# zhang-tao-whu/DVIS_Plus

Hardware: AMD Instinct MI355X
Metric: frames/sec DVIS++ R50 offline, 720p T=30 synthetic (higher is better)
Workload: dtype f32 (storage, accumulation, results; the segmenter's dense layers - R50 convolutions from 128 channels on, pixel-decoder projections and FPN output convolution, the deformable encoder's projections and FFN, the decoder's key / value projections - multiply each fp32 operand as two f16 terms on the f1

## Files before the change

### dvis_plus_amd/csrc/conv1x1_x3.hip

```cpp
#include "dvis_common.h"
#include "x3_common.h"

DVIS_EXPORT int64_t dvis_conv_x3_image_bytes(int64_t N, int C, int H, int W);
DVIS_EXPORT int dvis_conv_x3_gn_fold_supported(int K, int G, int64_t HW);

namespace {

constexpr unsigned kOOB = 0x80000000u;

struct CxArgs {
  const float *x, *bias, *res;
  const void *wp;
  float *y;
  int N, C, K, relu, npass;
  int stride, W_in, OW, H_in;
  int taps;
  long long HW, HW_in, pixels;
  long long tiles;
  float xscale, inv;
  int *flag;
  int tag;
  const float *x2;
  int C2, stride2, W2_in;
  long long HW2_in;
// ... 193 lines not shown
              hi4[e] = a.in_relu ? fmaxf(t1, 0.f) : t1;
            }
            asm volatile("" : "+v"(lo4), "+v"(hi4));
            __builtin_amdgcn_sched_barrier(0);
          }
          split8(lo4, hi4, a.xscale, xh[s], xl[s]);
        }
        if constexpr (kAffine)
          if (kc + 1 == NC && more) load_tab(ntile);
        if (++cc == NCC) cc = 0, ++tap;
        const bool first = kc + 1 < NC1, sec = !first && kc + 1 < NC;
        const unsigned po = first ? cx_tap_offset(a, gm, tap) : (sec ? gm2 : cx_tap_offset(a, ngm, 0));
        load_raw(po, first ? cc : (sec ? kc + 1 - NC1 : 0), sec);
      }
#pragma unroll
      for (int part = 0; part < IPC; ++part) {
        const char *stage = ring.wait(false);
        ring.begin(ring.more() ? next_offset() : 0);
        mma_item<IK, NB, PW>(stage, lane, acc, xh + IK * part, xl + IK * part, [&](int i) { ring.piece(i); });
      }
    }
    float chk = 0.f;
    if constexpr (NB == 2 || IMGOUT) {
      if (a.img != nullptr) {
        const unsigned gs = (unsigned)(a.K / 64) * 8192u;
        const __amdgpu_buffer_rsrc_t ri = dvis_make_rsrc_uniform(a.img, (unsigned)((long long)a.N * a.OH * a.XG * gs));
        const __amdgpu_buffer_rsrc_t rb = dvis_make_rsrc_uniform(a.bias ? (const void *)a.bias : (const void *)a.img, a.bias ? (unsigned)a.K * 4u : 0u);
        unsigned ibase = kOOB;
        if (p < a.pixels) {
          const int pix = (int)(p - n * a.HW), oy = pix / a.OW, ox = pix - oy * a.OW;
          ibase = (unsigned)(((n * a.OH + oy) * a.XG + (ox >> 5)) * gs + (co0 / 64) * 8192 + g * 512 + (ox & 31) * 16);
        }
#pragma unroll
        for (int nb = 0; nb < NB; ++nb) {
          float v[16];
#pragma unroll
          for (int q = 0; q < 4; ++q) {
            const f4 b = __builtin_bit_cast(f4, __builtin_amdgcn_raw_buffer_load_b128(rb, (unsigned)(co0 + 32 * nb + 8 * q + 4 * g) * 4u, 0, 0));
#pragma unroll
            for (int i = 0; i < 4; ++i) {
              const float t = acc[nb][4 * q + i] * a.inv + b[i];
              chk = __builtin_fmaf(t, 0.f, chk);
              v[4 * q + i] = a.relu ? x3_relu(t) : t;
            }
          }
          h8 hi[2], lo[2];
#pragma unroll
          for (int u = 0; u < 2; ++u) {
            const f4 p0 = {v[8 * u], v[8 * u + 1], v[8 * u + 2], v[8 * u + 3]}, p1 = {v[8 * u + 4], v[8 * u + 5], v[8 * u + 6], v[8 * u + 7]};
            split8(p0, p1, a.oscale, hi[u], lo[u]);
          }
          const h8 ls = lo[0] + lo[1];
          chk = __builtin_fmaf((float)((ls[0] + ls[1]) + (ls[2] + ls[3]) + (ls[4] + ls[5]) + (ls[6] + ls[7])), 0.f, chk);
          store_fragments4(ri, ibase, hi[0], 4096 * nb, lo[0], 4096 * nb + 1024, hi[1], 4096 * nb + 2048, lo[1], 4096 * nb + 3072);
        }
        if (a.flag != nullptr && chk != chk && p < a.pixels) atomicCAS(a.flag, 0, a.tag);
        tile = ntile, pass = npass_, gm = ngm, gm2 = ngm2;
        continue;
      }
    }
    double gw[8], gw2[4], gw4[2], gtot = 0.0;
#pragma unroll
    for (int nb = 0; nb < NB; ++nb) {
      float rv[16];
      double gq[4];
#pragma unroll
      for (int r = 0; r < 16; ++r)
        rv[r] = a.res ? __builtin_bit_cast(float, __builtin_amdgcn_raw_buffer_load_b32(
                                                      rr, obase + (unsigned)(co0 + 32 * nb + 8 * (r >> 2) + 4 * g + (r & 3)) * ochan, 0, 0))
                      : 0.f;
#pragma unroll
      for (int q = 0; q < 4; ++q) {
        const int co = co0 + 32 * nb + 8 * q + 4 * g;
        f4 b = {0.f, 0.f, 0.f, 0.f};
        if (a.bias) b = *(const f4 *)(a.bias + co);
        double gsum = 0.0, gsq = 0.0;
#pragma unroll
        for (int i = 0; i < 4; ++i) {
          const unsigned o = obase + (unsigned)(co + i) * ochan;
          float v = acc[nb][4 * q + i] * a.inv + b[i] + rv[4 * q + i];
          chk = __builtin_fmaf(v, 0.f, chk);
          if (a.relu) v = x3_relu(v);
          __builtin_amdgcn_raw_buffer_store_b32(__builtin_bit_cast(unsigned, v), ry, o, 0, 0);
          if constexpr (kStats) {
            const double d = p < a.pixels ? (double)v : 0.0;
            gsum = i == 0 ? d : gsum + d;
            gsq = i == 0 ? d * d : __builtin_fma(d, d, gsq);
          }
        }
        if constexpr (kStats) gq[q] = cx_fold<5>(gsum, gsq, lane);
      }
      if constexpr (kStats) {
        gw[nb] = cx_fold<3>(cx_fold<4>(gq[0], gq[1], lane), cx_fold<4>(gq[2], gq[3], lane), lane);
        if (nb % 2 == 1) gw2[nb / 2] = cx_fold<2>(gw[nb - 1], gw[nb], lane);
        if (nb % 4 == 3) gw4[nb / 4] = cx_fold<1>(gw2[nb / 2 - 1], gw2[nb / 2], lane);
        if (nb == NB - 1) gtot = cx_fold<0>(gw4[0], gw4[1], lane);
      }
    }
    if constexpr (kStats) {
      const long long pw = tile * kTile + wave * 32;
      if (pw < a.pixels) {
        const long long nw = pw / a.HW, slot = (pw - nw * a.HW) >> 5;
        const int group = co0 / 8 + 4 * (((lane >> 2) & 1) + 2 * ((lane >> 1) & 1) + 4 * (lane & 1)) + ((lane >> 4) & 1) + 2 * ((lane >> 3) & 1);
        a.gn_part[((nw * (a.K / 8) + group) * a.slots + slot) * 2 + (lane >> 5)] = gtot;
      }
    }
    if (a.flag != nullptr && chk != chk && p < a.pixels) atomicCAS(a.flag, 0, a.tag);
    tile = ntile, pass = npass_, gm = ngm, gm2 = ngm2;
  }
}

__global__ __launch_bounds__(256) void upsample_add_image_kernel(const float *__restrict__ lateral, const float *__restrict__ top,
                                                                 void *__restrict__ img, int N, int C, int H, int W, int h, int w,
                                                                 const float *__restrict__ lat_scale, const float *__restrict__ lat_shift,
                                                                 float oscale) {
  const int NCC = C / 64, XG = (W + 31) / 32;
  const int cc = blockIdx.x, xg = blockIdx.y;
  const int x = threadIdx.x & 31, g = (threadIdx.x >> 5) & 1, S = threadIdx.x >> 6;
  const int px = 32 * xg + x;
  const float sy = (float)h / (float)H, sx = (float)w / (float)W;
  const int pxc = px < W ? px : W - 1;
  float fx = sx * ((float)pxc + 0.5f) - 0.5f;
  fx = fx < 0.f ? 0.f : fx;
  const int x0 = min((int)fx, w - 1), x1 = x0 + (x0 < w - 1 ? 1 : 0);
  const float lx1 = fx - (float)x0, lx0 = 1.f - lx1;
  const __amdgpu_buffer_rsrc_t ri = dvis_make_rsrc_uniform(img, (unsigned)((long long)N * H * XG * NCC * 8192));
  const unsigned rows = (unsigned)N * (unsigned)H;
  for (unsigned row = blockIdx.z * 16u; row < blockIdx.z * 16u + 16u && row < rows; ++row) {
    const unsigned n = row / (unsigned)H;
    const int y = (int)(row - n * (unsigned)H);
    float fy = sy * ((float)y + 0.5f) - 0.5f;
    fy = fy < 0.f ? 0.f : fy;
    const int y0 = min((int)fy, h - 1), y1 = y0 + (y0 < h - 1 ? 1 : 0);
    const float ly1 = fy - (float)y0, ly0 = 1.f - ly1;
    float v[8];
#pragma unroll
    for (int e = 0; e < 8; ++e) {
      const int c = 64 * cc + 32 * (S >> 1) + 16 * (S & 1) + 8 * (e >> 2) + 4 * g + (e & 3);
      const unsigned pl = n * (unsigned)C + (unsigned)c;
      const float *t0 = top + ((size_t)pl * h + y0) * (size_t)w, *t1 = top + ((size_t)pl * h + y1) * (size_t)w;
      float lat = lateral[((size_t)pl * H + y) * (size_t)W + pxc];
      if (lat_scale) lat = lat * lat_scale[pl] + lat_shift[pl];
      v[e] = lat + (ly0 * (lx0 * t0[x0] + lx1 * t0[x1]) + ly1 * (lx0 * t1[x0] + lx1 * t1[x1]));
    }
    const f4 p0 = {v[0], v[1], v[2], v[3]}, p1 = {v[4], v[5], v[6], v[7]};
    h8 hi, lo;
    split8(p0, p1, oscale, hi, lo);
    const unsigned G = row * (unsigned)XG + (unsigned)xg;
    const unsigned off = (G * (unsigned)NCC + (unsigned)cc) * 8192u + (unsigned)(S * 2048 + g * 512 + x * 16);
    store_fragments2(ri, off, hi, 0, lo, 1024);
  }
}

}

DVIS_EXPORT int dvis_upsample_add_image(const float *lateral, const float *lat_scale, const float *lat_shift, const float *top, void *image,
                                        int N, int C, int H, int W, int h, int w, int oexp, void *stream) {
  DVIS_REQUIRE(lateral && top && image, "dvis_upsample_add_image: null pointer");
  DVIS_REQUIRE((lat_scale == nullptr) == (lat_shift == nullptr), "dvis_upsample_add_image: scale and shift together");
  DVIS_REQUIRE(N > 0 && C > 0 && C % 64 == 0 && H > 0 && W > 0 && h > 0 && w > 0, "dvis_upsample_add_image: bad sizes");
  DVIS_REQUIRE((uintptr_t)image % 16 == 0 && dvis_conv_x3_image_bytes(N, C, H, W) < ((int64_t)1 << 31), "dvis_upsample_add_image: a 16-byte "
               "aligned image below 2 GiB");
  const int per = 16 * 65535 / H;
  DVIS_REQUIRE(per >= 1 && (W + 31) / 32 <= 65535, "dvis_upsample_add_image: map too large (%d x %d)", H, W);
  for (int i = 0; i < N; i += per) {
    const int n = N - i < per ? N - i : per;
    hipLaunchKernelGGL(upsample_add_image_kernel, dim3(C / 64, (W + 31) / 32, (n * H + 15) / 16), dim3(256), 0, (hipStream_t)stream,
                       lateral + (size_t)i * C * H * W, top + (size_t)i * C * h * w,
                       (char *)image + (size_t)i * H * ((W + 31) / 32) * (C / 64) * 8192, n, C, H, W, h, w,
                       lat_scale ? lat_scale + (size_t)i * C : nullptr, lat_shift ? lat_shift + (size_t)i * C : nullptr, ldexpf(1.f, oexp));
  }
  return dvis_check_launch("dvis_upsample_add_image");
}

DVIS_EXPORT int dvis_conv1x1_x3_supported(int C, int K, int64_t N, int64_t HW_in, int64_t HW_out) {
  if (C < 64 || C % 64 != 0 || C > 4096) return 0;
  if (!(K == 64 || K == 128 || (K > 0 && K % 256 == 0 && K <= 8192))) return 0;
  if (N <= 0 || HW_out <= 0 || HW_in < HW_out) return 0;
  if (N * C * HW_in * 4 >= ((int64_t)1 << 31) || N * K * HW_out * 4 >= ((int64_t)1 << 31)) return 0;
  return 1;
}

DVIS_EXPORT int64_t dvis_conv1x1_x3_packed_bytes(int C, int K) {
  if (!dvis_conv1x1_x3_supported(C, K, 1, 1, 1)) return -1;
  return (int64_t)(C / 16) * (K / 32) * 2 * kPiece;
}

DVIS_EXPORT int dvis_conv1x1_x3_pack(const float *w, int K, int C, int wexp, void *packed, void *stream) {
  DVIS_REQUIRE(w && packed, "dvis_conv1x1_x3_pack: null operand");
  DVIS_REQUIRE(dvis_conv1x1_x3_supported(C, K, 1, 1, 1), "dvis_conv1x1_x3_pack: (C, K) = (%d, %d) is not served", C, K);
  DVIS_REQUIRE(wexp >= -60 && wexp <= 60, "dvis_conv1x1_x3_pack: wexp = %d", wexp);
  const int NB = K == 64 ? 2 : K == 128 ? 4 : 8;
  const int64_t fragments = (int64_t)(C / 16) * (K / 32) * 64;
  hipLaunchKernelGGL(x3_pack_kernel, dim3((unsigned)((fragments + 255) / 256)), dim3(256), 0, (hipStream_t)stream, w, (int64_t)C, K, C,
                     NB, 0, ldexpf(1.f, wexp), (_Float16 *)packed, fragments);
  return dvis_check_launch("dvis_conv1x1_x3_pack");
}

struct CxFold {
  double *gn_part;
  const float *in_scale, *in_shift;
  int in_relu;
};

static int cx_launch(const float *x, const void *packed, const float *bias, const float *res, float *y, int N, int C, int K, int H, int W,
                     int stride, int taps, int xexp, int wexp, int relu, void *stream, const float *x2 = nullptr, int C2 = 0, int H2 = 0,
                     int W2 = 0, int stride2 = 1, void *image = nullptr, int oexp = 0, const void *ximg = nullptr,
                     const CxFold *fold = nullptr);

DVIS_EXPORT int dvis_conv1x1_x3_dual(const float *x, const float *x2, const void *packed, const float *bias, const float *res, float *y,
                                     int N, int C, int C2, int K, int H, int W, int H2, int W2, int stride2, int xexp, int wexp, int relu,
                                     void *stream) {
  DVIS_REQUIRE(x2 != nullptr && C2 >= 64 && C2 % 64 == 0 && C2 <= 4096, "dvis_conv1x1_x3_dual: C2 %% 64 == 0 (got %d)", C2);
  DVIS_REQUIRE((stride2 == 1 || stride2 == 2) && (H2 + stride2 - 1) / stride2 == H && (W2 + stride2 - 1) / stride2 == W,
               "dvis_conv1x1_x3_dual: x2 (%d x %d, stride %d) must down-sample onto x's %d x %d map", H2, W2, stride2, H, W);
  DVIS_REQUIRE((long long)N * C2 * H2 * W2 * 4 < ((long long)1 << 31) && (uintptr_t)x2 % 16 == 0, "dvis_conv1x1_x3_dual: x2 below 2 GiB, 16-byte aligned");
  return cx_launch(x, packed, bias, res, y, N, C, K, H, W, 1, 1, xexp, wexp, relu, stream, x2, C2, H2, W2, stride2);
}

DVIS_EXPORT int dvis_conv1x1_x3(const float *x, const void *packed, const float *bias, const float *res, float *y, int N, int C, int K,
                                int H, int W, int stride, int xexp, int wexp, int relu, void *stream, const float *in_scale,
                                const float *in_shift, int in_relu, double *gn_part) {
  DVIS_REQUIRE((in_scale == nullptr) == (in_shift == nullptr), "dvis_conv1x1_x3: in_scale and in_shift together");
  const CxFold fold = {gn_part, in_scale, in_shift, in_relu};
  return cx_launch(x, packed, bias, res, y, N, C, K, H, W, stride, 1, xexp, wexp, relu, stream, nullptr, 0, 0, 0, 1, nullptr, 0, nullptr,
                   (gn_part || in_scale) ? &fold : nullptr);
}

DVIS_EXPORT int dvis_conv_x3_gn_fold_supported(int K, int G, int64_t HW) {
  return K > 0 && K % 256 == 0 && G > 0 && K == 8 * G && HW > 0 && HW % 32 == 0;
}

DVIS_EXPORT int dvis_conv1x1_x3_image(const float *x, const void *packed, const float *bias, void *image, int N, int C, int H, int W, int xexp,
                                      int wexp, int oexp, int relu, void *stream) {
  DVIS_REQUIRE(image != nullptr && (uintptr_t)image % 16 == 0, "dvis_conv1x1_x3_image: null / unaligned image");
  DVIS_REQUIRE((long long)N * H * ((W + 31) / 32) * 8192 < ((long long)1 << 31), "dvis_conv1x1_x3_image: the image must stay below 2 GiB");
  return cx_launch(x, packed, bias, nullptr, nullptr, N, C, 64, H, W, 1, 1, xexp, wexp, relu, stream, nullptr, 0, 0, 0, 1, image, oexp);
}

DVIS_EXPORT int64_t dvis_conv_x3_image_bytes(int64_t N, int C, int H, int W) {
  if (N < 0 || C <= 0 || C % 64 != 0 || H <= 0 || W <= 0) return -1;
  return N * H * ((W + 31) / 32) * (int64_t)(C / 64) * 8192;
}

DVIS_EXPORT int dvis_conv_x3_pack_image(const float *w, int K, int C, int taps, int wexp, void *packed, void *stream) {
  DVIS_REQUIRE(w && packed, "dvis_conv_x3_pack_image: null operand");
  DVIS_REQUIRE(taps == 1 || taps == 9, "dvis_conv_x3_pack_image: taps = %d", taps);
  DVIS_REQUIRE(dvis_conv1x1_x3_supported(C, K, 1, 1, 1) && K >= 128, "dvis_conv_x3_pack_image: (C, K) = (%d, %d) is not served", C, K);
  DVIS_REQUIRE(wexp >= -60 && wexp <= 60, "dvis_conv_x3_pack_image: wexp = %d", wexp);
  const int NB = K == 128 ? 4 : 8;
  const int64_t fragments = (int64_t)(taps * C / 16) * (K / 32) * 64;
  hipLaunchKernelGGL(x3_pack_kernel, dim3((unsigned)((fragments + 255) / 256)), dim3(256), 0, (hipStream_t)stream, w, (int64_t)taps * C, K,
                     taps * C, NB, 1, ldexpf(1.f, wexp), (_Float16 *)packed, fragments, taps);
  return dvis_check_launch("dvis_conv_x3_pack_image");
}

DVIS_EXPORT int dvis_conv_x3_image(const void *ximg, const float *x, const void *packed, const float *bias, const float *res, float *y,
                                   void *image, int N, int C, int K, int H, int W, int stride, int taps, int xexp, int wexp, int oexp, int relu,
                                   void *stream, double *gn_part) {
  DVIS_REQUIRE(ximg != nullptr || image != nullptr, "dvis_conv_x3_image: neither side is an operand image (use dvis_conv1x1_x3 / dvis_conv3x3_x3)");
  DVIS_REQUIRE((ximg != nullptr) != (x != nullptr), "dvis_conv_x3_image: exactly one of ximg and x");
  DVIS_REQUIRE((image != nullptr) != (y != nullptr), "dvis_conv_x3_image: exactly one of image and y");
  DVIS_REQUIRE(K == 128 || K % 256 == 0, "dvis_conv_x3_image: K = %d (128 or a multiple of 256)", K);
  DVIS_REQUIRE(taps == 1 || taps == 9, "dvis_conv_x3_image: taps = %d", taps);
  DVIS_REQUIRE(image == nullptr || res == nullptr, "dvis_conv_x3_image: an image output takes no residual");
  DVIS_REQUIRE(((uintptr_t)ximg | (uintptr_t)image) % 16 == 0, "dvis_conv_x3_image: images must be 16-byte aligned");
  const int OH = (H + stride - 1) / stride, OW = (W + stride - 1) / stride;
  DVIS_REQUIRE(dvis_conv_x3_image_bytes(N, C, H, W) < ((int64_t)1 << 31) && dvis_conv_x3_image_bytes(N, K, OH, OW) < ((int64_t)1 << 31),
               "dvis_conv_x3_image: images must stay below 2 GiB");
  DVIS_REQUIRE(gn_part == nullptr || (ximg != nullptr && y != nullptr), "dvis_conv_x3_image: statistics with an image in and an fp32 map out");
  const CxFold fold = {gn_part, nullptr, nullptr, 0};
  return cx_launch(x, packed, bias, res, y, N, C, K, H, W, stride, taps, xexp, wexp, relu, stream, nullptr, 0, 0, 0, 1, image, oexp, ximg,
                   gn_part ? &fold : nullptr);
}

DVIS_EXPORT int64_t dvis_conv3x3_x3_packed_bytes(int C, int K) {
  const int64_t b = dvis_conv1x1_x3_packed_bytes(C, K);
  return b < 0 ? b : 9 * b;
}

DVIS_EXPORT int dvis_conv3x3_x3_pack(const float *w, int K, int C, int wexp, void *packed, void *stream) {
  DVIS_REQUIRE(w && packed, "dvis_conv3x3_x3_pack: null operand");
  DVIS_REQUIRE(dvis_conv1x1_x3_supported(C, K, 1, 1, 1), "dvis_conv3x3_x3_pack: (C, K) = (%d, %d) is not served", C, K);
  DVIS_REQUIRE(wexp >= -60 && wexp <= 60, "dvis_conv3x3_x3_pack: wexp = %d", wexp);
  const int NB = K == 64 ? 2 : K == 128 ? 4 : 8;
  const int64_t fragments = (int64_t)(9 * C / 16) * (K / 32) * 64;
  hipLaunchKernelGGL(x3_pack_kernel, dim3((unsigned)((fragments + 255) / 256)), dim3(256), 0, (hipStream_t)stream, w, (int64_t)9 * C, K, 9 * C,
                     NB, 0, ldexpf(1.f, wexp), (_Float16 *)packed, fragments, 9);
  return dvis_check_launch("dvis_conv3x3_x3_pack");
}

DVIS_EXPORT int dvis_conv3x3_x3(const float *x, const void *packed, const float *bias, const float *res, float *y, int N, int C, int K,
                                int H, int W, int stride, int xexp, int wexp, int relu, void *stream) {
  return cx_launch(x, packed, bias, res, y, N, C, K, H, W, stride, 9, xexp, wexp, relu, stream);
}

static int cx_launch(const float *x, const void *packed, const float *bias, const float *res, float *y, int N, int C, int K, int H, int W,
                     int stride, int taps, int xexp, int wexp, int relu, void *stream, const float *x2, int C2, int H2, int W2, int stride2,
                     void *image, int oexp, const void *ximg, const CxFold *fold) {
  DVIS_REQUIRE((x || ximg) && packed && (y || image), "dvis_conv1x1_x3: null operand");
  DVIS_REQUIRE(stride == 1 || stride == 2, "dvis_conv1x1_x3: stride %d", stride);
  const int OH = (H + stride - 1) / stride, OW = (W + stride - 1) / stride;
  DVIS_REQUIRE(dvis_conv1x1_x3_supported(C, K, N, (int64_t)H * W, (int64_t)OH * OW), "dvis_conv1x1_x3: shape (N %d, C %d, K %d, %d x %d, "
               "stride %d) is not served (C %% 64 == 0, K = 64 / 128 or K %% 256 == 0, tensors below 2 GiB)", N, C, K, H, W, stride);
  DVIS_REQUIRE((uintptr_t)x % 16 == 0 && (uintptr_t)y % 16 == 0 && (uintptr_t)packed % 16 == 0 && (bias == nullptr || (uintptr_t)bias % 16 == 0),
               "dvis_conv1x1_x3: operands must be 16-byte aligned");
  CxArgs a = {};
  a.x = x, a.bias = bias, a.res = res, a.wp = packed, a.y = y, a.N = N, a.C = C, a.K = K, a.relu = relu;
  a.stride = stride, a.W_in = W, a.H_in = H, a.taps = taps, a.OW = OW, a.HW = (long long)OH * OW, a.HW_in = (long long)H * W;
  a.pixels = a.HW * N;
  a.xscale = ldexpf(1.f, xexp), a.inv = ldexpf(1.f, -(xexp + wexp));
  const X3Guard gd = dvis_x3_guard();
  a.flag = gd.flag, a.tag = gd.tag;
  a.x2 = x2, a.C2 = x2 ? C2 : 0, a.stride2 = stride2, a.W2_in = W2, a.HW2_in = (long long)H2 * W2;
  a.img = image, a.XG = (OW + 31) / 32, a.oscale = ldexpf(1.f, oexp), a.OH = OH;
  a.ximg = ximg, a.XG_in = (W + 31) / 32;
  const int grid = dvis_x3_persistent_cus();
  hipStream_t st = (hipStream_t)stream;
  a.npass = K <= 128 ? 1 : K / 256;
  if (fold != nullptr) {
    DVIS_REQUIRE(dvis_conv_x3_gn_fold_supported(K, K / 8, a.HW) && image == nullptr && x2 == nullptr, "dvis_conv1x1_x3: folded GroupNorm "
                 "needs K %% 256 == 0, H * W %% 32 == 0, an fp32 map out, one source (K %d, %d x %d)", K, OH, OW);
    DVIS_REQUIRE((fold->gn_part != nullptr) != (fold->in_scale != nullptr), "dvis_conv1x1_x3: statistics or an input affine, not both");
    a.tiles = (a.pixels + 255) / 256;
    a.gn_part = fold->gn_part, a.slots = (int)(a.HW / 32);
// ... 65 lines not shown
```

### dvis_plus_amd/csrc/gemm_x3.hip

```cpp
#define DVIS_X3_DMA_MUBUF 1
#include "dvis_common.h"
#include "x3_common.h"

#include <stdlib.h>

namespace {

template <int KS>
__device__ __forceinline__ void load_x(const float *x, int64_t ldx, int64_t row, int g, float s, h8 *xh, h8 *xl,
                                       const float *addp = nullptr) {
  const float *p = x + row * ldx + 8 * g;
  f4 raw[2 * KS];
#pragma unroll
  for (int S = 0; S < KS; ++S) raw[2 * S] = *(const f4 *)(p + 16 * S), raw[2 * S + 1] = *(const f4 *)(p + 16 * S + 4);
  if (addp != nullptr) {
#pragma unroll
    for (int S = 0; S < KS; ++S) raw[2 * S] += *(const f4 *)(addp + 16 * S), raw[2 * S + 1] += *(const f4 *)(addp + 16 * S + 4);
  }
#pragma unroll
  for (int S = 0; S < KS; ++S) split8(raw[2 * S], raw[2 * S + 1], s, xh[S], xl[S]);
}

__device__ __forceinline__ void store_block(char *scr, int lane, const f4 *v, float *dst, int64_t ld, int rows_valid,
                                            const float *radd = nullptr, int64_t ldr = 0) {
  const int j = lane & 31, g = lane >> 5, sw = (j >> 1) & 7;
#pragma unroll
  for (int q = 0; q < 4; ++q) *(f4 *)(scr + j * 128 + (((2 * q + g) ^ sw) << 4)) = v[q];
  __builtin_amdgcn_wave_barrier();
#pragma unroll
  for (int t = 0; t < 4; ++t) {
    const int jr = 8 * t + (lane >> 3), pp = lane & 7;
    f4 o = *(const f4 *)(scr + jr * 128 + ((pp ^ ((jr >> 1) & 7)) << 4));
    if (radd != nullptr && jr < rows_valid) o += *(const f4 *)(radd + jr * ldr + 4 * pp);
    if (jr < rows_valid) *(f4 *)(dst + jr * ld + 4 * pp) = o;
  }
  __builtin_amdgcn_wave_barrier();
}

struct EpiArgs {
  const float *bias;
  const float *res;
  int64_t ldres;
  const float *gamma, *beta;
  float eps;
  const float *pos;
  int64_t pos_rows;
  float *out, *out2;
  int64_t ldo;
  float inv;
  int relu;
  const float *radd;
  int *flag;
  int tag;
};

template <int NB, bool LN, bool EX = false>
__device__ __forceinline__ void epilogue(f16v *acc, const EpiArgs &e, const float *cb, const float *cg, const float *cbeta, char *scr,
                                         int lane, int64_t tok0, int64_t M, int col0 = 0) {
  const int j = lane & 31, g = lane >> 5;
  const int64_t tok = tok0 + j < M ? tok0 + j : M - 1;
  const int rows_valid = M - tok0 < 32 ? (int)(M - tok0) : 32;
  constexpr int N = 32 * NB;
  float mean = 0.f, rstd = 1.f;
  if constexpr (LN) {
    const float *rp = e.res + tok * e.ldres + 4 * g;
    f4 r[2][4];
    auto fetch = [&](int nb, f4 *dst) {
#pragma unroll
      for (int q = 0; q < 4; ++q) dst[q] = *(const f4 *)(rp + 32 * nb + 8 * q);
    };
    fetch(0, r[0]);
    float sum = 0.f;
#pragma unroll
    for (int nb = 0; nb < NB; ++nb) {
      if (nb + 1 < NB) fetch(nb + 1, r[(nb + 1) & 1]);
#pragma unroll
      for (int q = 0; q < 4; ++q) {
        const f4 b = *(const f4 *)(cb + 32 * nb + 8 * q + 4 * g);
#pragma unroll
        for (int i = 0; i < 4; ++i) {
          const float v = acc[nb][4 * q + i] * e.inv + b[i] + r[nb & 1][q][i];
          acc[nb][4 * q + i] = v;
          sum += v;
        }
      }
    }
    sum += __shfl_xor(sum, 32);
    if (e.flag != nullptr && !(fabsf(sum) <= 3.4028235e38f)) atomicCAS(e.flag, 0, e.tag);
    mean = sum * (1.f / N);
    float sq = 0.f;
#pragma unroll
    for (int nb = 0; nb < NB; ++nb)
#pragma unroll
      for (int i = 0; i < 16; ++i) {
        const float d = acc[nb][i] - mean;
        sq += d * d;
      }
    sq += __shfl_xor(sq, 32);
    rstd = rsqrtf(sq * (1.f / N) + e.eps);
  }
  float chk = 0.f;
  const float *pr = nullptr;
  f4 pv[2][4];
  auto fetch_pos = [&](int nb, f4 *dst) {
#pragma unroll
    for (int q = 0; q < 4; ++q) dst[q] = *(const f4 *)(pr + 32 * nb + 8 * q);
  };
  if constexpr (LN) {
    if (e.pos != nullptr) {
      pr = e.pos + (tok % e.pos_rows) * N + 4 * g;
      fetch_pos(0, pv[0]);
    }
  }
#pragma unroll
  for (int nb = 0; nb < NB; ++nb) {
    f4 v[4];
    if constexpr (LN) {
      if (e.pos != nullptr && nb + 1 < NB) fetch_pos(nb + 1, pv[(nb + 1) & 1]);
    }
#pragma unroll
    for (int q = 0; q < 4; ++q) {
      const int n = 32 * nb + 8 * q + 4 * g;
      if constexpr (LN) {
        const f4 ga = *(const f4 *)(cg + n), be = *(const f4 *)(cbeta + n);
#pragma unroll
        for (int i = 0; i < 4; ++i) v[q][i] = (acc[nb][4 * q + i] - mean) * rstd * ga[i] + be[i];
      } else {
        const f4 b = *(const f4 *)(cb + n);
#pragma unroll
        for (int i = 0; i < 4; ++i) {
          const float t = acc[nb][4 * q + i] * e.inv + b[i];
          chk = __builtin_fmaf(t, 0.f, chk);
          if constexpr (EX)
            v[q][i] = e.relu == 1 ? x3_relu(t) : e.relu == 2 ? 0.5f * t * (1.f + erff(t * 0.70710678118654752440f)) : t;
          else
            v[q][i] = e.relu ? x3_relu(t) : t;
        }
      }
    }
    if constexpr (!EX)
      store_block(scr, lane, v, e.out + tok0 * e.ldo + col0 + 32 * nb, e.ldo, rows_valid);
    else
      store_block(scr, lane, v, e.out + tok0 * e.ldo + col0 + 32 * nb, e.ldo, rows_valid,
                  e.radd ? e.radd + tok0 * e.ldres + col0 + 32 * nb : nullptr, e.ldres);
    if constexpr (LN) {
      if (e.pos != nullptr) {
#pragma unroll
        for (int q = 0; q < 4; ++q) v[q] += pv[nb & 1][q];
        store_block(scr, lane, v, e.out2 + tok0 * e.ldo + 32 * nb, e.ldo, rows_valid);
      }
    }
  }
  if constexpr (!LN) {
    if (e.flag != nullptr && chk != chk) atomicCAS(e.flag, 0, e.tag);
  }
}

template <int NB>
__global__ __launch_bounds__(kThreads) void x3_linear_kernel(const float *__restrict__ x, int64_t ldx, int64_t M,
                                                             const void *__restrict__ wp, float xscale, int npass,
                                                             const float *__restrict__ xadd, int64_t xadd_rows, EpiArgs e) {
  extern __shared__ __attribute__((aligned(1024))) char lds[];
  constexpr int K = 256, KS = K / 16, NI = K / 32;
  const int wave = threadIdx.x >> 6, lane = threadIdx.x & 63, j = lane & 31, g = lane >> 5;
  const int64_t ntiles = (M + kTileTok - 1) / kTileTok;
  const int64_t my = blockIdx.x < ntiles ? (ntiles - blockIdx.x + gridDim.x - 1) / gridDim.x : 0;
  Ring<NB> ring;
  ring.start(wp, lds, NI * npass, (int)(my * NI * npass), wave, lane);
  char *scr = lds + kStages * Ring<NB>::kItemBytes + wave * kScratch;
  float *cst = (float *)(lds + kStages * Ring<NB>::kItemBytes + kWaves * kScratch);
  const int ntot = 32 * NB * npass;
  for (int i = threadIdx.x; i < ntot; i += kThreads) cst[i] = e.bias ? e.bias[i] : 0.f;
  __syncthreads();
  for (int64_t tile = blockIdx.x; tile < ntiles; tile += gridDim.x) {
    const int64_t tok0 = tile * kTileTok + wave * 32;
    const int64_t row = tok0 + j < M ? tok0 + j : M - 1;
    h8 xh[KS], xl[KS];
    load_x<KS>(x, ldx, row, g, xscale, xh, xl, xadd ? xadd + (row % xadd_rows) * K + 8 * g : nullptr);
    for (int pass = 0; pass < npass; ++pass) {
      f16v acc[NB];
#pragma unroll
      for (int nb = 0; nb < NB; ++nb)
#pragma unroll
        for (int i = 0; i < 16; ++i) acc[nb][i] = 0.f;
#pragma unroll
      for (int c = 0; c < NI; ++c) {
        const char *stage = ring.wait(c == 0);
        ring.begin_periodic();
        mma_item<2, NB, NB>(stage, lane, acc, xh + 2 * c, xl + 2 * c, [&](int i) { ring.piece(i); });
      }
      if (tok0 < M) epilogue<NB, false>(acc, e, cst + pass * 32 * NB, cst + ntot, cst + ntot + 32 * NB, scr, lane, tok0, M, pass * 32 * NB);
    }
  }
}

constexpr int x3_stream_layout_blocks(int nb) { return 4 * nb % 8 == 0 ? nb : nb + 1; }

template <int NB, bool LN, bool EX = false, bool ADD = false>
__global__ __launch_bounds__(512) void x3_linear_stream_kernel(const float *__restrict__ x, int64_t ldx, int64_t M, int K,
                                                               const void *__restrict__ wp, float xscale, int npass,
                                                               const float *__restrict__ xadd, int64_t xadd_rows, EpiArgs e) {
  extern __shared__ __attribute__((aligned(1024))) char lds[];
  constexpr int NBL = x3_stream_layout_blocks(NB);
  constexpr int NW = 8, PW = 4 * NBL / NW, kTile = NW * 32;
  typedef Ring<PW, 8, NW> RingT;
  const int wave = threadIdx.x >> 6, lane = threadIdx.x & 63, j = lane & 31, g = lane >> 5;
  const int NI = K / 32, NC = K / 64;
  const int64_t ntiles = (M + kTile - 1) / kTile;
  const int64_t my = blockIdx.x < ntiles ? (ntiles - blockIdx.x + gridDim.x - 1) / gridDim.x : 0;
  if (my == 0) return;
  RingT ring;
  ring.start(wp, lds, NI * npass, (int)(my * NI * npass), wave, lane);
  char *scr = lds + kStages * RingT::kItemBytes + wave * kScratch;
  float *cst = (float *)(lds + kStages * RingT::kItemBytes + NW * kScratch);
  const int ntot = 32 * NB * npass;
  for (int i = threadIdx.x; i < ntot; i += 512) cst[i] = e.bias ? e.bias[i] : 0.f;
  if constexpr (LN)
    for (int i = threadIdx.x; i < 32 * NB; i += 512) cst[ntot + i] = e.gamma[i], cst[ntot + 32 * NB + i] = e.beta[i];
  __syncthreads();
  auto products = [&](const char *stage, f16v *acc, const h8 *xh, const h8 *xl) {
    if constexpr (NBL == NB) {
      mma_item<2, NB, PW>(stage, lane, acc, xh, xl, [&](int i) { ring.piece(i); });
    } else {
      mma_item<1, NB, 3>(stage, lane, acc, xh, xl, [&](int i) { ring.piece(i); });
      mma_item<1, NB, PW - 3>(stage + NBL * 2 * kPiece, lane, acc, xh + 1, xl + 1, [&](int i) { ring.piece(3 + i); });
    }
  };
  auto row_of = [&](int64_t tile) {
    const int64_t t = tile * kTile + wave * 32 + j;
    return t < M ? t : M - 1;
  };
  if constexpr (ADD) {
    f4 raw[4], rawp[4];
    auto load_raw = [&](const float *rowp, const float *posp, int it) {
#pragma unroll
      for (int s = 0; s < 2; ++s) {
        raw[2 * s] = *(const f4 *)(rowp + 32 * it + 16 * s), raw[2 * s + 1] = *(const f4 *)(rowp + 32 * it + 16 * s + 4);
        rawp[2 * s] = *(const f4 *)(posp + 32 * it + 16 * s), rawp[2 * s + 1] = *(const f4 *)(posp + 32 * it + 16 * s + 4);
      }
    };
    int64_t r0 = row_of(blockIdx.x);
    const float *rowp = x + r0 * ldx + 8 * g, *posp = xadd + (r0 % xadd_rows) * K + 8 * g;
    load_raw(rowp, posp, 0);
    for (int64_t tile = blockIdx.x; tile < ntiles; tile += gridDim.x) {
      const int64_t tok0 = tile * kTile + wave * 32;
      const int64_t rn = row_of(tile + gridDim.x < ntiles ? tile + gridDim.x : tile);
      const float *nrowp = x + rn * ldx + 8 * g, *nposp = xadd + (rn % xadd_rows) * K + 8 * g;
      for (int pass = 0; pass < npass; ++pass) {
        f16v acc[NB];
#pragma unroll
        for (int nb = 0; nb < NB; ++nb)
#pragma unroll
          for (int i = 0; i < 16; ++i) acc[nb][i] = 0.f;
        for (int it = 0; it < NI; ++it) {
#pragma unroll
          for (int i = 0; i < 4; ++i) asm volatile("" : "+v"(raw[i]), "+v"(rawp[i]));
          h8 xh[2], xl[2];
#pragma unroll
          for (int s = 0; s < 2; ++s) split8(raw[2 * s] + rawp[2 * s], raw[2 * s + 1] + rawp[2 * s + 1], xscale, xh[s], xl[s]);
          if (it + 1 < NI)
            load_raw(rowp, posp, it + 1);
          else if (pass + 1 < npass)
            load_raw(rowp, posp, 0);
          else
            load_raw(nrowp, nposp, 0);
          const char *stage = ring.wait(false);
          ring.begin_periodic();
          products(stage, acc, xh, xl);
        }
        if (tok0 < M) epilogue<NB, LN, EX>(acc, e, cst + pass * 32 * NB, cst + ntot, cst + ntot + 32 * NB, scr, lane, tok0, M, pass * 32 * NB);
      }
      rowp = nrowp, posp = nposp;
    }
    return;
  }
  f4 raw[8];
  auto load_raw = [&](const float *rowp, int kc) {
#pragma unroll
    for (int s = 0; s < 4; ++s) raw[2 * s] = *(const f4 *)(rowp + 64 * kc + 16 * s), raw[2 * s + 1] = *(const f4 *)(rowp + 64 * kc + 16 * s + 4);
  };
  auto row_ptr = [&](int64_t tile) { return x + row_of(tile) * ldx + 8 * g; };
  const float *rowp = row_ptr(blockIdx.x);
  load_raw(rowp, 0);
  for (int64_t tile = blockIdx.x; tile < ntiles; tile += gridDim.x) {
    const int64_t tok0 = tile * kTile + wave * 32;
    const float *nrowp = row_ptr(tile + gridDim.x < ntiles ? tile + gridDim.x : tile);
    for (int pass = 0; pass < npass; ++pass) {
      f16v acc[NB];
#pragma unroll
      for (int nb = 0; nb < NB; ++nb)
#pragma unroll
        for (int i = 0; i < 16; ++i) acc[nb][i] = 0.f;
      for (int kc = 0; kc < NC; ++kc) {
#pragma unroll
        for (int i = 0; i < 8; ++i) asm volatile("" : "+v"(raw[i]));
        h8 xh[4], xl[4];
#pragma unroll
        for (int s = 0; s < 4; ++s) split8(raw[2 * s], raw[2 * s + 1], xscale, xh[s], xl[s]);
        if (kc + 1 < NC)
          load_raw(rowp, kc + 1);
        else
          load_raw(pass + 1 < npass ? rowp : nrowp, 0);
#pragma unroll
        for (int half = 0; half < 2; ++half) {
          const char *stage = ring.wait(false);
          ring.begin_periodic();
          products(stage, acc, xh + 2 * half, xl + 2 * half);
        }
      }
      if (tok0 < M) epilogue<NB, LN, EX>(acc, e, cst + pass * 32 * NB, cst + ntot, cst + ntot + 32 * NB, scr, lane, tok0, M, pass * 32 * NB);
    }
    rowp = nrowp;
  }
}

struct FfnArgs {
  const float *b1;
  float inv1, hscale;
  int HB;
};

__global__ __launch_bounds__(kThreads) void x3_ffn_kernel(const float *__restrict__ x, int64_t ldx, int64_t M,
                                                          const void *__restrict__ wp, float xscale, FfnArgs f, EpiArgs e) {
  extern __shared__ __attribute__((aligned(1024))) char lds[];
  constexpr int KS = 16;
  const int wave = threadIdx.x >> 6, lane = threadIdx.x & 63, j = lane & 31, g = lane >> 5;
  const int64_t ntiles = (M + kTileTok - 1) / kTileTok;
  const int64_t my = blockIdx.x < ntiles ? (ntiles - blockIdx.x + gridDim.x - 1) / gridDim.x : 0;
  const int per_tile = 8 * f.HB;
  Ring<8> ring;
  ring.start(wp, lds, per_tile, (int)(my * per_tile), wave, lane);
  char *scr = lds + kStages * Ring<8>::kItemBytes + wave * kScratch;
  float *b1s = (float *)(lds + kStages * Ring<8>::kItemBytes + kWaves * kScratch);
  for (int i = threadIdx.x; i < 128 * f.HB; i += kThreads) b1s[i] = f.b1[i];
  float *cst = b1s + 128 * f.HB;
  for (int i = threadIdx.x; i < 256; i += kThreads) cst[i] = e.bias[i], cst[256 + i] = e.gamma[i], cst[512 + i] = e.beta[i];
  __syncthreads();
  for (int64_t tile = blockIdx.x; tile < ntiles; tile += gridDim.x) {
    const int64_t tok0 = tile * kTileTok + wave * 32;
    const int64_t row = tok0 + j < M ? tok0 + j : M - 1;
    h8 xh[KS], xl[KS];
    load_x<KS>(x, ldx, row, g, xscale, xh, xl);
    f16v acc2[8];
#pragma unroll
    for (int nb = 0; nb < 8; ++nb)
#pragma unroll
      for (int i = 0; i < 16; ++i) acc2[nb][i] = 0.f;
    for (int hb = 0; hb < f.HB; ++hb) {
      f16v acc1[4];
#pragma unroll
      for (int t = 0; t < 4; ++t)
#pragma unroll
        for (int i = 0; i < 16; ++i) acc1[t][i] = 0.f;
      h8 hh[8], hl[8];
      f2 cv = {0.f, 0.f};
      auto convert = [&](int tc, int t) {
        const int pair = t >> 1, u = pair >> 2, pp = pair & 3;
        if ((t & 1) == 0) {
          const f2 b = *(const f2 *)(b1s + 128 * hb + 32 * tc + 16 * u + 8 * (pp >> 1) + 4 * g + 2 * (pp & 1));
          cv[0] = x3_relu(acc1[tc][8 * u + 2 * pp] * f.inv1 + b[0]) * f.hscale;
          cv[1] = x3_relu(acc1[tc][8 * u + 2 * pp + 1] * f.inv1 + b[1]) * f.hscale;
        } else {
          const h2 h = __builtin_convertvector(cv, h2);
          const f2 r = cv - __builtin_convertvector(h, f2);
          const h2 l = __builtin_convertvector(r, h2);
          hh[2 * tc + u][2 * pp] = h.x, hh[2 * tc + u][2 * pp + 1] = h.y;
          hl[2 * tc + u][2 * pp] = l.x, hl[2 * tc + u][2 * pp + 1] = l.y;
        }
      };
#pragma unroll
      for (int c = 0; c < 4; ++c) {
        const char *stage = ring.wait(hb == 0 && c == 0);
        ring.begin_periodic();
        mma_item<16, 1, 8>(stage, lane, acc1 + c, xh, xl, [&](int i) { ring.piece(i); }, [&](int t) {
          if (c > 0) convert(c - 1, t);
        });
      }
#pragma unroll
      for (int c = 0; c < 4; ++c) {
        const char *stage = ring.wait(false);
        ring.begin_periodic();
        if (c == 0) {
          mma_item<2, 8, 8>(stage, lane, acc2, hh, hl, [&](int i) { ring.piece(i); }, [&](int t) { convert(3, t); });
        } else {
          mma_item<2, 8, 8>(stage, lane, acc2, hh + 2 * c, hl + 2 * c, [&](int i) { ring.piece(i); });
        }
      }
    }
    if (tok0 < M) epilogue<8, true>(acc2, e, cst, cst + 256, cst + 512, scr, lane, tok0, M);
  }
}

__global__ void x3_ffn_pack_kernel(const float *w1, int64_t ldw1, const float *w2, int64_t ldw2, int H, float s1, float s2,
                                   _Float16 *out, int64_t fragments) {
  const int64_t idx = (int64_t)blockIdx.x * blockDim.x + threadIdx.x;
  if (idx >= fragments) return;
  const int lane = idx & 63;
  int64_t t = idx >> 6;
  const int fr = t & 15;
  t >>= 4;
  const int item = t & 7, hb = t >> 3;
  _Float16 *o = out + (((int64_t)hb * 8 + item) * 16 + fr) * 1024 + lane * 8;
  if (item < 4) {
    x3_pack_fragment(w1, ldw1, H, 256, 128 * hb + 32 * item + (lane & 31), 0, fr, lane >> 5, s1, o, o + 512);
  } else {
    const int s = fr >> 3, nb = fr & 7;
    x3_pack_fragment(w2, ldw2, 256, H, 32 * nb + (lane & 31), 1, 8 * hb + 2 * (item - 4) + s, lane >> 5, s2, o, o + 512);
  }
}

int x3_grid(int64_t ntiles) {
  const int cus = dvis_x3_persistent_cus();
  return (int)(ntiles < cus ? ntiles : cus);
}

float x3_pow2(int e) { return ldexpf(1.f, e); }

template <typename Kern, typename... Args>
int x3_launch(Kern kern, DvisLdsOptIn *opted, size_t lds_bytes, int64_t M, hipStream_t st, const char *what, Args... args) {
  const int rc = dvis_lds_opt_in((const void *)kern, lds_bytes, opted, what);
  if (rc != DVIS_OK) return rc;
  const int64_t ntiles = (M + kTileTok - 1) / kTileTok;
  hipLaunchKernelGGL(kern, dim3(x3_grid(ntiles)), dim3(kThreads), lds_bytes, st, args...);
  return dvis_check_launch(what);
}

int x3_check_common(const float *x, int64_t ldx, int64_t M, const void *wp, const float *out, int64_t ldo) {
  DVIS_REQUIRE(x && wp && out, "dvis_x3: null operand");
  DVIS_REQUIRE(M >= 0 && M < (int64_t)1 << 31, "dvis_x3: M = %lld out of range", (long long)M);
  DVIS_REQUIRE(ldx % 4 == 0 && ldo % 4 == 0 && (uintptr_t)x % 16 == 0 && (uintptr_t)out % 16 == 0 && (uintptr_t)wp % 16 == 0,
               "dvis_x3: operands must be 16-byte aligned with row strides %% 4 == 0");
  return DVIS_OK;
}

}

static int x3_passes(int N, int *nb) {
  if (N == 128 || N == 192 || N == 256 || N == 288) return *nb = N / 32, 1;
  if (N > 0 && N % 256 == 0 && N <= 8192) return *nb = 8, N / 256;
  return *nb = 0, 0;
}

static int g_x3_reserve = [] {
  const char *e = getenv("DVIS_X3_RESERVE");
  const int r = e ? atoi(e) : 0;
  return r < 0 ? 0 : r / 8 * 8;
}();

int dvis_x3_persistent_cus() {
  int dev = 0, cus = 256;
  if (hipGetDevice(&dev) == hipSuccess) {
    int v = 0;
    if (hipDeviceGetAttribute(&v, hipDeviceAttributeMultiprocessorCount, dev) == hipSuccess && v >= 8) cus = v;
  }
  cus = cus / 8 * 8;
  const int r = __atomic_load_n(&g_x3_reserve, __ATOMIC_RELAXED);
  return cus - r >= 8 ? cus - r : cus;
}

DVIS_EXPORT int dvis_x3_set_reserve(int cus) {
  const int r = cus < 0 ? 0 : cus / 8 * 8;
  return __atomic_exchange_n(&g_x3_reserve, r, __ATOMIC_RELAXED);
}

static int *g_x3_flag[64] = {};
static thread_local int t_x3_tag = 1;

X3Guard dvis_x3_guard() {
  int dev = 0;
  if (hipGetDevice(&dev) != hipSuccess || dev < 0 || dev >= 64) return X3Guard{nullptr, 0};
  return X3Guard{__atomic_load_n(&g_x3_flag[dev], __ATOMIC_RELAXED), t_x3_tag};
}

DVIS_EXPORT int dvis_x3_set_range_flag(int32_t *flag) {
  int dev = 0;
  if (hipGetDevice(&dev) != hipSuccess || dev < 0 || dev >= 64) {
    dvis_set_error("dvis_x3_set_range_flag: no current device");
    return DVIS_E_ARG;
  }
  __atomic_store_n(&g_x3_flag[dev], (int *)flag, __ATOMIC_RELAXED);
  return DVIS_OK;
}

DVIS_EXPORT int dvis_x3_set_tag(int tag) {
  const int prev = t_x3_tag;
  t_x3_tag = tag > 0 ? tag : 1;
  return prev;
}

DVIS_EXPORT int dvis_x3_linear_supported(int N, int K, int ln) {
  int nb;
  if (K < 64 || K % 64 != 0 || K > 8192) return 0;
  if (ln) return N == 256;
  if (N == 288) return K == 256;
  return x3_passes(N, &nb) > 0;
}

DVIS_EXPORT int64_t dvis_x3_packed_bytes(int N, int K) {
  if (!dvis_x3_linear_supported(N, K, 0)) return -1;
  int NB;
  const int npass = x3_passes(N, &NB);
  return (int64_t)(K / 16) * npass * x3_stream_layout_blocks(NB) * 2 * kPiece;
}

DVIS_EXPORT int dvis_x3_pack(const float *w, int64_t ldw, int N, int K, int wexp, void *packed, void *stream) {
  DVIS_REQUIRE(w && packed, "dvis_x3_pack: null operand");
  DVIS_REQUIRE(dvis_x3_linear_supported(N, K, 0), "dvis_x3_pack: (N, K) = (%d, %d) is not served (K %% 64 == 0; N in 128 / 192 / 256 or N %% 256 == 0; N = 288 at K = 256)", N, K);
  DVIS_REQUIRE(wexp >= -60 && wexp <= 60, "dvis_x3_pack: wexp = %d", wexp);
  int NB;
  const int npass = x3_passes(N, &NB);
  const int NBL = x3_stream_layout_blocks(NB);
  const int64_t fragments = (int64_t)(K / 16) * npass * NBL * 64;
  hipLaunchKernelGGL(x3_pack_kernel, dim3((unsigned)((fragments + 255) / 256)), dim3(256), 0, (hipStream_t)stream, w, ldw, N, K,
                     NBL, 0, x3_pow2(wexp), (_Float16 *)packed, fragments);
  return dvis_check_launch("dvis_x3_pack");
}

static int x3_linear_impl(const float *x, int64_t ldx, int64_t M, int K, const void *wp, int N, int xexp, int wexp, const float *xadd,
                          int64_t xadd_rows, const float *bias, int relu, float *out, int64_t ldo, void *stream,
                          const float *radd = nullptr, int64_t ldr = 0);

DVIS_EXPORT int dvis_x3_linear(const float *x, int64_t ldx, int64_t M, int K, const void *wp, int N, int xexp, int wexp,
                               const float *bias, int relu, float *out, int64_t ldo, void *stream) {
  return x3_linear_impl(x, ldx, M, K, wp, N, xexp, wexp, nullptr, 0, bias, relu, out, ldo, stream);
}

DVIS_EXPORT int dvis_x3_linear_add(const float *x, int64_t ldx, int64_t M, int K, const void *wp, int N, int xexp, int wexp,
                                   const float *xadd, int64_t xadd_rows, const float *bias, int relu, float *out, int64_t ldo,
                                   void *stream) {
  DVIS_REQUIRE(xadd && xadd_rows > 0 && (uintptr_t)xadd % 16 == 0, "dvis_x3_linear_add: xadd (xadd_rows x K, 16-byte aligned) is required");
  DVIS_REQUIRE(K == 256 && dvis_x3_linear_supported(N, K, 0), "dvis_x3_linear_add: served for K = 256 (N %d, K %d)", N, K);
  return x3_linear_impl(x, ldx, M, K, wp, N, xexp, wexp, xadd, xadd_rows, bias, relu, out, ldo, stream);
}

DVIS_EXPORT int dvis_x3_linear_res(const float *x, int64_t ldx, int64_t M, int K, const void *wp, int N, int xexp, int wexp,
                                   const float *bias, int act, const float *res, int64_t ldres, float *out, int64_t ldo, void *stream) {
  DVIS_REQUIRE(act >= 0 && act <= 2, "dvis_x3_linear_res: act must be 0 (none), 1 (ReLU) or 2 (GELU)");
  DVIS_REQUIRE(res == nullptr || ((uintptr_t)res % 16 == 0 && ldres % 4 == 0 && ldres >= N),
               "dvis_x3_linear_res: res must be 16-byte aligned with a row stride that is a multiple of 4 floats and >= N");
  return x3_linear_impl(x, ldx, M, K, wp, N, xexp, wexp, nullptr, 0, bias, act, out, ldo, stream, res, ldres);
}

static int x3_linear_impl(const float *x, int64_t ldx, int64_t M, int K, const void *wp, int N, int xexp, int wexp, const float *xadd,
                          int64_t xadd_rows, const float *bias, int relu, float *out, int64_t ldo, void *stream, const float *radd,
                          int64_t ldr) {
  DVIS_REQUIRE(dvis_x3_linear_supported(N, K, 0), "dvis_x3_linear: (N, K) = (%d, %d) is not served (K %% 64 == 0; N in 128 / 192 / 256 or N %% 256 == 0; N = 288 at K = 256)", N, K);
  const int rc = x3_check_common(x, ldx, M, wp, out, ldo);
  if (rc != DVIS_OK) return rc;
  if (M == 0) return DVIS_OK;
  EpiArgs e = {};
  e.bias = bias, e.out = out, e.ldo = ldo, e.inv = x3_pow2(-(xexp + wexp)), e.relu = relu;
  e.radd = radd, e.ldres = ldr;
  const X3Guard gd = dvis_x3_guard();
  e.flag = gd.flag, e.tag = gd.tag;
  const float xs = x3_pow2(xexp);
  hipStream_t st = (hipStream_t)stream;
  int NB;
  const int npass = x3_passes(N, &NB);
#define DVIS_X3_STREAM_FORM(NBV, LNV, EXV, ADDV, XADD, XROWS, WHAT, LDS_EXTRA)                                        \
  {                                                                                                                  \
    static DvisLdsOptIn opted;                                                                                       \
    typedef Ring<4 * x3_stream_layout_blocks(NBV) / 8, 8, 8> R;                                                      \
    const size_t lds_bytes = kStages * R::kItemBytes + 8 * kScratch + (LDS_EXTRA);                                   \
    const int rc2 = dvis_lds_opt_in((const void *)x3_linear_stream_kernel<NBV, LNV, EXV, ADDV>, lds_bytes, &opted, WHAT);  \
    if (rc2 != DVIS_OK) return rc2;                                                                                  \
    const int64_t ntiles = (M + 255) / 256;                                                                          \
    hipLaunchKernelGGL((x3_linear_stream_kernel<NBV, LNV, EXV, ADDV>), dim3(x3_grid(ntiles)), dim3(512), lds_bytes, st, x, ldx, M, K, wp, \
                       xs, npass, XADD, XROWS, e);                                                                   \
    return dvis_check_launch(WHAT);                                                                                  \
  }
#define DVIS_X3_STREAM_EX(NBV, LNV, EXV, WHAT, LDS_EXTRA) DVIS_X3_STREAM_FORM(NBV, LNV, EXV, false, (const float *)nullptr, (int64_t)0, WHAT, LDS_EXTRA)
#define DVIS_X3_STREAM(NBV, LNV, WHAT, LDS_EXTRA) DVIS_X3_STREAM_EX(NBV, LNV, false, WHAT, LDS_EXTRA)
#define DVIS_X3_RESIDENT(NBV)                                                                                        \
  {                                                                                                                  \
    static DvisLdsOptIn opted;                                                                                       \
    return x3_launch(x3_linear_kernel<NBV>, &opted, kStages * Ring<NBV>::kItemBytes + kWaves * kScratch + (size_t)N * 4, \
                     M, st, "dvis_x3_linear", x, ldx, M, wp, xs, npass, xadd, xadd_rows, e);                         \
  }
  if (relu == 2 || radd) {
    DVIS_REQUIRE(NB == 8 && !xadd, "dvis_x3_linear_res: the GELU / residual epilogue is served for N %% 256 == 0 (N = %d)", N);
    DVIS_X3_STREAM_EX(8, false, true, "dvis_x3_linear_res", (size_t)N * 4)
  }
  if (xadd) {
    switch (NB) {
      case 4: DVIS_X3_RESIDENT(4)
      case 6: DVIS_X3_RESIDENT(6)
      case 8: DVIS_X3_RESIDENT(8)
      default: DVIS_X3_STREAM_FORM(9, false, false, true, xadd, xadd_rows, "dvis_x3_linear_add", (size_t)N * 4)
    }
  }
  switch (NB) {
    case 4: DVIS_X3_STREAM(4, false, "dvis_x3_linear", (size_t)N * 4)
    case 6: DVIS_X3_STREAM(6, false, "dvis_x3_linear", (size_t)N * 4)
    case 8: DVIS_X3_STREAM(8, false, "dvis_x3_linear", (size_t)N * 4)
    default: DVIS_X3_STREAM(9, false, "dvis_x3_linear", (size_t)N * 4)
  }
#undef DVIS_X3_RESIDENT
}

DVIS_EXPORT int dvis_x3_linear_ln(const float *x, int64_t ldx, int64_t M, int K, const void *wp, int N, int xexp, int wexp,
                                  const float *bias, const float *res, int64_t ldres, const float *gamma, const float *beta,
                                  float eps, const float *pos, int64_t pos_rows, float *out, float *out2, int64_t ldo,
                                  void *stream) {
  DVIS_REQUIRE(dvis_x3_linear_supported(N, K, 1), "dvis_x3_linear_ln: (N, K) = (%d, %d) is not served (256, 256)", N, K);
  DVIS_REQUIRE(bias && res && gamma && beta, "dvis_x3_linear_ln: bias, res, gamma, beta are required");
  DVIS_REQUIRE(ldres % 4 == 0 && (uintptr_t)res % 16 == 0, "dvis_x3_linear_ln: res must be 16-byte aligned, ldres %% 4 == 0");
  DVIS_REQUIRE(pos == nullptr || (out2 && pos_rows > 0 && (uintptr_t)pos % 16 == 0 && (uintptr_t)out2 % 16 == 0),
               "dvis_x3_linear_ln: pos needs out2, pos_rows > 0 and 16-byte alignment");
  const int rc = x3_check_common(x, ldx, M, wp, out, ldo);
  if (rc != DVIS_OK) return rc;
  if (M == 0) return DVIS_OK;
  EpiArgs e = {};
  e.bias = bias, e.res = res, e.ldres = ldres, e.gamma = gamma, e.beta = beta, e.eps = eps, e.pos = pos, e.pos_rows = pos_rows;
  e.out = out, e.out2 = out2, e.ldo = ldo, e.inv = x3_pow2(-(xexp + wexp));
  const X3Guard gd = dvis_x3_guard();
  e.flag = gd.flag, e.tag = gd.tag;
  const float xs = x3_pow2(xexp);
  const int npass = 1;
  hipStream_t st = (hipStream_t)stream;
  DVIS_X3_STREAM(8, true, "dvis_x3_linear_ln", (size_t)3 * 256 * 4)
#undef DVIS_X3_STREAM
#undef DVIS_X3_STREAM_EX
#undef DVIS_X3_STREAM_FORM
}

DVIS_EXPORT int64_t dvis_x3_ffn_packed_bytes(int K, int H, int N) {
  if (K != 256 || N != 256 || H <= 0 || H % 128 != 0 || H > 4096) return -1;
  return (int64_t)(H / 128) * 8 * Ring<8>::kItemBytes;
}

DVIS_EXPORT int dvis_x3_ffn_pack(const float *w1, int64_t ldw1, const float *w2, int64_t ldw2, int K, int H, int N, int w1exp,
                                 int w2exp, void *packed, void *stream) {
  DVIS_REQUIRE(w1 && w2 && packed, "dvis_x3_ffn_pack: null operand");
  DVIS_REQUIRE(dvis_x3_ffn_packed_bytes(K, H, N) > 0, "dvis_x3_ffn_pack: needs K = N = 256, H %% 128 == 0 (K %d, H %d, N %d)", K, H, N);
  const int64_t fragments = (int64_t)(H / 128) * 8 * 16 * 64;
  hipLaunchKernelGGL(x3_ffn_pack_kernel, dim3((unsigned)((fragments + 255) / 256)), dim3(256), 0, (hipStream_t)stream, w1, ldw1,
                     w2, ldw2, H, x3_pow2(w1exp), x3_pow2(w2exp), (_Float16 *)packed, fragments);
  return dvis_check_launch("dvis_x3_ffn_pack");
}

DVIS_EXPORT int dvis_x3_ffn_ln(const float *x, int64_t ldx, int64_t M, int K, int H, int N, const void *wp, int xexp, int w1exp,
                               int hexp, int w2exp, const float *b1, const float *b2, const float *gamma, const float *beta,
                               float eps, const float *pos, int64_t pos_rows, float *out, float *out2, int64_t ldo,
                               void *stream) {
  DVIS_REQUIRE(dvis_x3_ffn_packed_bytes(K, H, N) > 0, "dvis_x3_ffn_ln: needs K = N = 256, H %% 128 == 0 (K %d, H %d, N %d)", K, H, N);
  DVIS_REQUIRE(b1 && b2 && gamma && beta, "dvis_x3_ffn_ln: biases, gamma, beta are required");
  DVIS_REQUIRE(pos == nullptr || (out2 && pos_rows > 0 && (uintptr_t)pos % 16 == 0 && (uintptr_t)out2 % 16 == 0),
               "dvis_x3_ffn_ln: pos needs out2, pos_rows > 0 and 16-byte alignment");
  const int rc = x3_check_common(x, ldx, M, wp, out, ldo);
  if (rc != DVIS_OK) return rc;
  if (M == 0) return DVIS_OK;
  EpiArgs e = {};
  e.bias = b2, e.res = x, e.ldres = ldx, e.gamma = gamma, e.beta = beta, e.eps = eps, e.pos = pos, e.pos_rows = pos_rows;
  e.out = out, e.out2 = out2, e.ldo = ldo, e.inv = x3_pow2(-(hexp + w2exp));
  const X3Guard gd = dvis_x3_guard();
  e.flag = gd.flag, e.tag = gd.tag;
  FfnArgs f = {b1, x3_pow2(-(xexp + w1exp)), x3_pow2(hexp), H / 128};
  static DvisLdsOptIn opted;
  return x3_launch(x3_ffn_kernel, &opted, kStages * Ring<8>::kItemBytes + kWaves * kScratch + (size_t)(H + 3 * 256) * 4, M,
                   (hipStream_t)stream, "dvis_x3_ffn_ln", x, ldx, M, wp, x3_pow2(xexp), f, e);
}
```

### dvis_plus_amd/functions.py

```python
import collections
import ctypes
import math
import os
import threading

import torch
from torch.autograd import Function
from torch.autograd.function import once_differentiable

from . import cpu_ops, derived, native
from .cpu_ops import ms_deform_attn_core_pytorch


def _torch_path(op, x, why):
    if os.environ.get("DVIS_STRICT", "1") != "0" and x.is_cuda and not torch.is_grad_enabled():
        raise RuntimeError(f"DVIS_STRICT: {op} would run its torch formulation on a GPU tensor ({why}; shape "
                           f"{tuple(x.shape)}, dtype {x.dtype}, contiguous {x.is_contiguous()})")


class no_autocast:

    def __enter__(self):
        import contextlib
        self._stack = contextlib.ExitStack()
# ... 1493 lines not shown
        return n


def _rows_image_buffer(M, K, device):
    nbytes = native.lib().dvis_x3_rows_image_bytes(M, K)
    if nbytes < 0:
        raise RuntimeError(f"row image: K % 32 == 0 is required (K {K})")
    return torch.empty(nbytes, dtype=torch.uint8, device=device)


def x3_rows_image(x, xexp=None):
    K = x.shape[-1]
    x2, ldx = _x3_rows(x, "x")
    e = X3_XEXP if xexp is None else xexp
    buf = _rows_image_buffer(x2.shape[0], K, x.device)
    with torch.cuda.device(x.device):
        native.check(native.lib().dvis_x3_rows_image(ctypes.c_void_p(x2.data_ptr()), ldx, x2.shape[0], K, e, ctypes.c_void_p(buf.data_ptr()),
                                                     native.stream_ptr(x.device)), "dvis_x3_rows_image")
    return RowImage(buf, x.shape, e, 0)


def layer_norm_rows_image_ok(x, norm):
    C = x.shape[-1]
    return (X3_ROW_IMAGES and x3_on() and x.is_cuda and x.dtype == torch.float32 and x.is_contiguous() and x.data_ptr() % 16 == 0
            and C % 32 == 0 and C <= 1024 and norm.weight is not None and norm.bias is not None and not torch.is_grad_enabled()
            and not torch.is_autocast_enabled())


def layer_norm_rows_image(x, norm, xexp=None):
    C = x.shape[-1]
    M = x.numel() // C
    e = X3_XEXP if xexp is None else xexp
    buf = _rows_image_buffer(M, C, x.device)
    with torch.cuda.device(x.device):
        native.check(native.lib().dvis_layernorm_rows_image(
            ctypes.c_void_p(x.data_ptr()), native.dev_ptr(norm.weight, "gamma"), native.dev_ptr(norm.bias, "beta"), M, C, float(norm.eps), e,
            ctypes.c_void_p(buf.data_ptr()), native.stream_ptr(x.device)), "dvis_layernorm_rows_image")
    return RowImage(buf, x.shape, e, 0)


def x3_tile_linear(x, weight, bias, act=None, residual=None, xexp=None):
    N, K = weight.shape
    if isinstance(x, RowImage):
        return _x3_tile_linear_image(x, weight, bias, act, residual)
    x2, ldx = _x3_rows(x, "x")
    buf, wexp = x3_tile_pack(weight)
    out = torch.empty((*x.shape[:-1], N), dtype=torch.float32, device=x.device)
    rptr, ldr = None, 0
    if residual is not None:
        if residual.shape != out.shape or residual.dtype != torch.float32 or not residual.is_cuda:
            raise RuntimeError("x3_tile_linear: residual must be a float32 GPU tensor of the output's shape")
        r2, ldr = _rows2d(residual, N)
        rptr = ctypes.c_void_p(r2.data_ptr())
    with torch.cuda.device(x.device):
        native.check(native.lib().dvis_x3_tile_linear(
            ctypes.c_void_p(x2.data_ptr()), ldx, x2.shape[0], K, ctypes.c_void_p(buf.data_ptr()), N,
            X3_XEXP if xexp is None else xexp, wexp, None if bias is None else native.dev_ptr(bias.detach(), "bias"),
            {None: 0, "relu": 1, "gelu": 2}[act], rptr, ldr, ctypes.c_void_p(out.data_ptr()), N, native.stream_ptr(x.device)),
            "dvis_x3_tile_linear")
    return out


def _x3_tile_linear_image(img, weight, bias, act, residual):
    N, K = weight.shape
    if img.shape[-1] != K:
        raise RuntimeError(f"x3_tile_linear: image of {img.shape} rows against a weight of {tuple(weight.shape)}")
    M = img.rows
    buf, wexp = x3_tile_pack(weight, img.order)
    bptr = None if bias is None else native.dev_ptr(bias.detach(), "bias")
    lib = native.lib()
    with torch.cuda.device(img.device):
        if act == "gelu":
            if residual is not None:
                raise RuntimeError("x3_tile_linear: the GELU form of a row image writes a row image (no residual)")
            out = _rows_image_buffer(M, N, img.device)
            native.check(lib.dvis_x3_tile_linear_image(ctypes.c_void_p(img.data.data_ptr()), M, K, ctypes.c_void_p(buf.data_ptr()), N, img.exp, wexp,
                                                       bptr, 2, None, 0, None, 0, ctypes.c_void_p(out.data_ptr()), X3_XEXP,
                                                       native.stream_ptr(img.device)), "dvis_x3_tile_linear_image")
            return RowImage(out, (*img.shape[:-1], N), X3_XEXP, 1)
        out = torch.empty((*img.shape[:-1], N), dtype=torch.float32, device=img.device)
        rptr, ldr = None, 0
        if residual is not None:
            if residual.shape != out.shape or residual.dtype != torch.float32 or not residual.is_cuda:
                raise RuntimeError("x3_tile_linear: residual must be a float32 GPU tensor of the output's shape")
            r2, ldr = _rows2d(residual, N)
            rptr = ctypes.c_void_p(r2.data_ptr())
        native.check(lib.dvis_x3_tile_linear_image(ctypes.c_void_p(img.data.data_ptr()), M, K, ctypes.c_void_p(buf.data_ptr()), N, img.exp, wexp,
                                                   bptr, {None: 0, "relu": 1}[act], rptr, ldr, ctypes.c_void_p(out.data_ptr()), N, None, 0,
                                                   native.stream_ptr(img.device)), "dvis_x3_tile_linear_image")
    return out


X3_QKV_FUSED = os.environ.get("DVIS_X3_QKV_FUSED", "1") != "0"


def x3_qkv_attention_ok(x, weight, heads):
    if isinstance(x, RowImage):
        if len(x.shape) != 3 or not (X3_QKV_FUSED and weight.dim() == 2 and weight._base is None):
            return False
        B, L, C = x.shape
        return (C == heads * 64 and weight.shape == (3 * C, C) and L >= 1024 and C >= X3_TILE_MIN_K
                and bool(native.lib().dvis_x3_tile_supported(3 * C, C)))
    if not (X3_QKV_FUSED and x.dim() == 3 and x.is_cuda and x.dtype == torch.float32 and not torch.is_grad_enabled()
            and not torch.is_autocast_enabled() and x3_on() and weight.dim() == 2 and weight._base is None):
        return False
    B, L, C = x.shape
    return (C == heads * 64 and weight.shape == (3 * C, C) and L >= 1024 and x.is_contiguous() and x.data_ptr() % 16 == 0
            and x3_tile_ok(x, 3 * C, C))


def x3_qkv_attention(x, weight, bias, heads, out_image=False):
    B, L, C = x.shape
    image_in = isinstance(x, RowImage)
    buf, wexp = x3_tile_pack(weight, x.order if image_in else 0)
    lib = native.lib()
    nbytes = lib.dvis_attention_ws_bytes_k(B * heads, L, L, 64, 2)
    ws = torch.empty((nbytes + 3) // 4, dtype=torch.float32, device=x.device)
    qscale = (1.0 / 8.0) * 1.4426950408889634 * 16.0
    bptr = None if bias is None else native.dev_ptr(bias.detach(), "bias")
    with torch.cuda.device(x.device):
        if image_in:
            native.check(lib.dvis_x3_tile_linear_qkv_image(
                ctypes.c_void_p(x.data.data_ptr()), B * L, C, ctypes.c_void_p(buf.data_ptr()), 3 * C, x.exp, wexp, bptr, heads, L, qscale,
                ctypes.c_void_p(ws.data_ptr()), native.stream_ptr(x.device)), "dvis_x3_tile_linear_qkv_image")
        else:
            native.check(lib.dvis_x3_tile_linear_qkv(
                ctypes.c_void_p(x.data_ptr()), C, B * L, C, ctypes.c_void_p(buf.data_ptr()), 3 * C, X3_XEXP, wexp, bptr, heads, L, qscale,
                ctypes.c_void_p(ws.data_ptr()), native.stream_ptr(x.device)), "dvis_x3_tile_linear_qkv")
        if out_image:
            out = _rows_image_buffer(B * L, C, x.device)
            native.check(lib.dvis_attention_x3_packed_image(ctypes.c_void_p(ws.data_ptr()), ctypes.c_void_p(out.data_ptr()), B, heads, L, X3_XEXP,
                                                            native.stream_ptr(x.device)), "dvis_attention_x3_packed_image")
            return RowImage(out, (B, L, C), X3_XEXP, 2)
        out = torch.empty((B, L, C), dtype=torch.float32, device=x.device)
        strides = (ctypes.c_int64 * 3)(L * C, 64, C)
        native.check(lib.dvis_attention_x3_packed(ctypes.c_void_p(ws.data_ptr()), ctypes.c_void_p(out.data_ptr()), strides, B, heads, L,
                                                  native.stream_ptr(x.device)), "dvis_attention_x3_packed")
    return out


def x3_ok(x, N, K, ln=False, add=False):
    return (x.is_cuda and x.dtype == torch.float32 and not torch.is_grad_enabled() and x.shape[-1] == K
            and (not add or K == 256) and bool(native.lib().dvis_x3_linear_supported(N, K, int(ln))))


def _x3_rows(x, name):
    K = x.shape[-1]
    x2, ld = _rows2d(x, K)
    if x2.data_ptr() % 16 or ld % 4:
        raise RuntimeError(f"x3: {name} must be 16-byte aligned with a row stride % 4 == 0")
    return x2, ld


def x3_linear(x, weight, bias, relu=False, xexp=None, xadd=None, act=None, residual=None):
    N, K = weight.shape
    x2, ldx = _x3_rows(x, "x")
    buf, wexp = x3_pack(weight)
    out = torch.empty((*x.shape[:-1], N), dtype=torch.float32, device=x.device)
    if act is not None or residual is not None:
        if xadd is not None:
            raise RuntimeError("x3_linear: xadd and act / residual are served by different entry points")
        code = {None: int(bool(relu)), "relu": 1, "gelu": 2}[act]
        rptr, ldr = None, 0
        if residual is not None:
            if residual.shape != out.shape or residual.dtype != torch.float32 or not residual.is_cuda:
                raise RuntimeError("x3_linear: residual must be a float32 GPU tensor of the output's shape")
            r2, ldr = _x3_rows(residual, "residual")
            rptr = ctypes.c_void_p(r2.data_ptr())
        with torch.cuda.device(x.device):
            native.check(native.lib().dvis_x3_linear_res(
                ctypes.c_void_p(x2.data_ptr()), ldx, x2.shape[0], K, ctypes.c_void_p(buf.data_ptr()), N,
                X3_XEXP if xexp is None else xexp, wexp, None if bias is None else native.dev_ptr(bias.detach(), "bias"), code,
                rptr, ldr, ctypes.c_void_p(out.data_ptr()), N, native.stream_ptr(x.device)), "dvis_x3_linear_res")
        return out
    if xadd is not None:
        if x.dim() != 3 or xadd.numel() != x.shape[1] * K or xadd.dtype != torch.float32 or not xadd.is_cuda:
            raise RuntimeError("x3_linear: xadd must be a float32 GPU (S, K) embedding for x of shape (B, S, K)")
        xadd = xadd.contiguous()
        with torch.cuda.device(x.device):
            native.check(native.lib().dvis_x3_linear_add(
                ctypes.c_void_p(x2.data_ptr()), ldx, x2.shape[0], K, ctypes.c_void_p(buf.data_ptr()), N,
                X3_XEXP if xexp is None else xexp, wexp, ctypes.c_void_p(xadd.data_ptr()), x.shape[1],
                None if bias is None else native.dev_ptr(bias.detach(), "bias"), int(relu), ctypes.c_void_p(out.data_ptr()), N,
                native.stream_ptr(x.device)), "dvis_x3_linear_add")
        return out
    with torch.cuda.device(x.device):
        native.check(native.lib().dvis_x3_linear(
            ctypes.c_void_p(x2.data_ptr()), ldx, x2.shape[0], K, ctypes.c_void_p(buf.data_ptr()), N,
            X3_XEXP if xexp is None else xexp, wexp, None if bias is None else native.dev_ptr(bias.detach(), "bias"), int(relu),
            ctypes.c_void_p(out.data_ptr()), N, native.stream_ptr(x.device)), "dvis_x3_linear")
    return out


def _x3_pos(pos, x, N):
    if pos is None:
        return None, 0, None
    if x.dim() != 3 or pos.numel() != x.shape[1] * N or pos.dtype != torch.float32 or not pos.is_cuda:
        raise RuntimeError("x3: pos must be a float32 GPU (S, C) embedding for x of shape (N, S, C)")
    return pos.contiguous(), x.shape[1], torch.empty((*x.shape[:-1], N), dtype=torch.float32, device=x.device)


def x3_linear_ln(x, weight, bias, res, norm, pos=None, xexp=None):
    N, K = weight.shape
    x2, ldx = _x3_rows(x, "x")
    r2, ldr = _x3_rows(res, "res")
    buf, wexp = x3_pack(weight)
    out = torch.empty((*x.shape[:-1], N), dtype=torch.float32, device=x.device)
    pos, pos_rows, out2 = _x3_pos(pos, x, N)
    with torch.cuda.device(x.device):
        native.check(native.lib().dvis_x3_linear_ln(
            ctypes.c_void_p(x2.data_ptr()), ldx, x2.shape[0], K, ctypes.c_void_p(buf.data_ptr()), N,
            X3_XEXP if xexp is None else xexp, wexp, native.dev_ptr(bias.detach(), "bias"), ctypes.c_void_p(r2.data_ptr()), ldr,
            native.dev_ptr(norm.weight.detach(), "gamma"), native.dev_ptr(norm.bias.detach(), "beta"), float(norm.eps),
            None if pos is None else ctypes.c_void_p(pos.data_ptr()), pos_rows, ctypes.c_void_p(out.data_ptr()),
            None if out2 is None else ctypes.c_void_p(out2.data_ptr()), N, native.stream_ptr(x.device)), "dvis_x3_linear_ln")
    return out if out2 is None else (out, out2)


def x3_ffn_ok(x, lin1, lin2):
    K, H, N = lin1.weight.shape[1], lin1.weight.shape[0], lin2.weight.shape[0]
    return (x.is_cuda and x.dtype == torch.float32 and not torch.is_grad_enabled() and x.shape[-1] == K
            and lin2.weight.shape[1] == H and lin1.bias is not None and lin2.bias is not None
            and native.lib().dvis_x3_ffn_packed_bytes(K, H, N) > 0)


def x3_ffn_ln(x, lin1, lin2, norm, pos=None, xexp=None, hexp=None):
    w1, w2 = lin1.weight, lin2.weight
    H, K = w1.shape
    N = w2.shape[0]
    x2, ldx = _x3_rows(x, "x")

    def make():
        a, b = w1.detach().contiguous(), w2.detach().contiguous()
        e1, e2 = _x3_wexp(a), _x3_wexp(b)
        buf = torch.empty(native.lib().dvis_x3_ffn_packed_bytes(K, H, N), dtype=torch.uint8, device=a.device)
        with torch.cuda.device(a.device):
            native.check(native.lib().dvis_x3_ffn_pack(ctypes.c_void_p(a.data_ptr()), K, ctypes.c_void_p(b.data_ptr()), H, K, H,
                                                       N, e1, e2, ctypes.c_void_p(buf.data_ptr()),
                                                       native.stream_ptr(a.device)), "dvis_x3_ffn_pack")
        return buf, e1, e2
    buf, e1, e2 = _x3_cache(w1, [w1, w2], make, kind="ffn")
    out = torch.empty((*x.shape[:-1], N), dtype=torch.float32, device=x.device)
    pos, pos_rows, out2 = _x3_pos(pos, x, N)
    with torch.cuda.device(x.device):
        native.check(native.lib().dvis_x3_ffn_ln(
            ctypes.c_void_p(x2.data_ptr()), ldx, x2.shape[0], K, H, N, ctypes.c_void_p(buf.data_ptr()),
            X3_XEXP if xexp is None else xexp, e1, X3_XEXP if hexp is None else hexp, e2,
            native.dev_ptr(lin1.bias.detach(), "b1"), native.dev_ptr(lin2.bias.detach(), "b2"),
            native.dev_ptr(norm.weight.detach(), "gamma"), native.dev_ptr(norm.bias.detach(), "beta"), float(norm.eps),
            None if pos is None else ctypes.c_void_p(pos.data_ptr()), pos_rows, ctypes.c_void_p(out.data_ptr()),
            None if out2 is None else ctypes.c_void_p(out2.data_ptr()), N, native.stream_ptr(x.device)), "dvis_x3_ffn_ln")
    return out if out2 is None else (out, out2)


def maps_to_tokens(maps, affines=None, pos=None):
    affines = affines or [None] * len(maps)
    N, C = maps[0].shape[:2]
    if not all(m.is_cuda and m.dtype == torch.float32 and m.is_contiguous() for m in maps) or torch.is_grad_enabled():
        _torch_path("maps_to_tokens", maps[0], "needs contiguous fp32 NCHW maps")
        maps = [m if a is None else m * a[0].view(N, C, 1, 1) + a[1].view(N, C, 1, 1) for m, a in zip(maps, affines)]
        out = torch.cat([m.flatten(2).transpose(1, 2) for m in maps], 1)
        return out if pos is None else (out, out + pos.reshape(1, -1, C))
    S = sum(m.shape[2] * m.shape[3] for m in maps)
    out = torch.empty((N, S, C), dtype=torch.float32, device=maps[0].device)
    out_pos = pp = None
    if pos is not None:
        if pos.numel() != S * C or pos.dtype != torch.float32 or not pos.is_cuda:
            raise RuntimeError("maps_to_tokens: pos must be a float32 GPU (S, C) embedding")
        pos = pos.contiguous()
        out_pos = torch.empty_like(out)
        pp = native.dev_ptr(pos, "pos")
    row0 = 0
    with torch.cuda.device(out.device):
        for m, a in zip(maps, affines):
            HW = m.shape[2] * m.shape[3]
            rc = native.lib().dvis_nchw_to_tokens_affine(
                ctypes.c_void_p(m.data_ptr()), None if a is None else native.dev_ptr(a[0], "scale"),
                None if a is None else native.dev_ptr(a[1], "shift"), pp, ctypes.c_void_p(out.data_ptr()),
                None if out_pos is None else ctypes.c_void_p(out_pos.data_ptr()), N, C, HW, S, row0,
                native.stream_ptr(out.device))
            native.check(rc, "dvis_nchw_to_tokens_affine")
            row0 += HW
    return out if pos is None else (out, out_pos)


def normalize_pad_ok(x, mean):
    return bool(x.is_cuda and x.dim() == 4 and x.dtype in (torch.uint8, torch.float32) and x.is_contiguous()
                and mean.numel() == x.shape[1] and mean.dtype == torch.float32 and not torch.is_grad_enabled())


def normalize_pad(x, mean, std, Hp, Wp):
    N, C, H, W = x.shape
    out = torch.empty((N, C, Hp, Wp), dtype=torch.float32, device=x.device)
    with torch.cuda.device(x.device):
        native.check(native.lib().dvis_normalize_pad(
            native.dev_ptr(x, "frames"), int(x.dtype == torch.uint8), native.dev_ptr(out, "out"), N * C, C, H, W, Hp, Wp,
            native.dev_ptr(mean.detach().reshape(-1), "pixel_mean"), native.dev_ptr(std.detach().reshape(-1), "pixel_std"),
            native.stream_ptr(x.device)), "dvis_normalize_pad")
    return out


def tokens_to_map(tokens, row0, h, w):
    N, S, C = tokens.shape
    if not (tokens.is_cuda and tokens.dtype == torch.float32 and tokens.is_contiguous() and not torch.is_grad_enabled()):
        return tokens[:, row0:row0 + h * w].transpose(1, 2).reshape(N, C, h, w)
    out = torch.empty((N, C, h, w), dtype=torch.float32, device=tokens.device)
    with torch.cuda.device(tokens.device):
        native.check(native.lib().dvis_tokens_to_nchw(ctypes.c_void_p(tokens.data_ptr()), ctypes.c_void_p(out.data_ptr()), N, C, h * w,
# ... 65 lines not shown
def gn_fold_ok(norm, K, HW):
    return bool(PD_GN_FOLD and isinstance(norm, torch.nn.GroupNorm) and norm.num_channels == K
                and native.lib().dvis_conv_x3_gn_fold_supported(K, norm.num_groups, HW))


def affine_in_ok(x, weight):
    return bool(PD_GN_FOLD and conv1x1_x3_ok(x, weight) and x.shape[1] == 256 and x.shape[0] > 0
                and native.lib().dvis_conv_x3_gn_fold_supported(weight.shape[0], weight.shape[0] // 8, x.shape[2] * x.shape[3]))


def _gn_partials(N, K, HW, device):
    return torch.empty((N, K // 8, HW // 32, 2), dtype=torch.float64, device=device)


def _gn_finalize(part, norm, N, K, HW):
    scale = torch.empty(N * K, dtype=torch.float32, device=part.device)
    shift = torch.empty(N * K, dtype=torch.float32, device=part.device)
    with torch.cuda.device(part.device):
        native.check(native.lib().dvis_group_norm_finalize(
            native.dev_ptr(part, "partials"), None if norm.weight is None else native.dev_ptr(norm.weight.detach(), "gamma"),
            None if norm.bias is None else native.dev_ptr(norm.bias.detach(), "beta"), native.dev_ptr(scale, "scale"),
            native.dev_ptr(shift, "shift"), N, K, norm.num_groups, HW, float(norm.eps), native.stream_ptr(part.device)),
            "dvis_group_norm_finalize")
    return scale, shift


def conv1x1_x3(x, weight, bias=None, res=None, relu=False, stride=1, xexp=None, affine=None, affine_relu=False, gn=None):
    N, Ci, H, W = x.shape
    Co = weight.shape[0]

    def make():
        return _x3_pack_conv1x1(weight.detach().reshape(Co, Ci).contiguous())
    buf, wexp = _x3_cache(weight, [weight], make, kind="conv1x1")
    OH, OW = (H + stride - 1) // stride, (W + stride - 1) // stride
    out = torch.empty((N, Co, OH, OW), dtype=torch.float32, device=x.device)
    step = _conv_x3_chunks(N, Ci, Co, H * W, OH * OW)
    if affine is not None and not (affine_in_ok(x, weight) and stride == 1 and gn is None):
        raise RuntimeError("conv1x1_x3: this launch takes no input affine (see affine_in_ok); apply scale_shift_act_ first")
    part = _gn_partials(N, Co, OH * OW, x.device) if gn is not None and N > 0 and gn_fold_ok(gn, Co, OH * OW) else None
    with torch.cuda.device(x.device):
        for i in range(0, N, step):
            n = min(step, N - i)
            native.check(native.lib().dvis_conv1x1_x3(
                native.dev_ptr(x[i:i + n], "x"), ctypes.c_void_p(buf.data_ptr()),
                None if bias is None else native.dev_ptr(bias.detach(), "bias"),
                None if res is None else native.dev_ptr(res[i:i + n], "res"), native.dev_ptr(out[i:i + n], "out"), n, Ci, Co, H, W,
                stride, X3_CONV_XEXP if xexp is None else xexp, wexp, 1 if relu else 0, native.stream_ptr(x.device),
                None if affine is None else native.dev_ptr(affine[0].reshape(N, Ci)[i:i + n], "scale"),
                None if affine is None else native.dev_ptr(affine[1].reshape(N, Ci)[i:i + n], "shift"), 1 if affine_relu else 0,
                None if part is None else native.dev_ptr(part[i:i + n], "partials")), "dvis_conv1x1_x3")
    if gn is None:
        return out
    return out, (_gn_finalize(part, gn, N, Co, OH * OW) if part is not None else group_norm_affine(out, gn))


X3_DUAL = os.environ.get("DVIS_X3_DUAL", "1") != "0"


def conv1x1_x3_dual_ok(a, w3, x, ws, stride2):
    if not (X3_DUAL and conv1x1_x3_ok(a, w3) and x.is_cuda and x.dim() == 4 and x.dtype == torch.float32 and x.is_contiguous()
            and ws.dtype == torch.float32 and ws.shape[0] == w3.shape[0] and stride2 in (1, 2)):
        return False
    N, C, H, W = a.shape
    N2, C2, H2, W2 = x.shape
    Co = w3.shape[0]
    return (N2 == N and C2 % 64 == 0 and 64 <= C2 <= 4096 and (H2 + stride2 - 1) // stride2 == H and (W2 + stride2 - 1) // stride2 == W
            and (C + C2) <= 4096 and bool(native.lib().dvis_conv1x1_x3_supported(C + C2, Co, 1, H * W, H * W))
            and C2 * H2 * W2 * 4 < 2 ** 31)


def conv1x1_x3_dual(a, w3, b3, x, ws, bs, relu=True, stride2=1, xexp=None):
    N, C, H, W = a.shape
    _, C2, H2, W2 = x.shape
    Co = w3.shape[0]

    def make():
        wcat = torch.cat([w3.detach().reshape(Co, C), ws.detach().reshape(Co, C2)], 1).contiguous()
        buf, e = _x3_pack_conv1x1(wcat)
        bias = None
        if b3 is not None or bs is not None:
            bias = (0 if b3 is None else b3.detach()) + (0 if bs is None else bs.detach())
        return buf, e, bias
    buf, wexp, bias = _x3_cache(w3, [w3, ws, b3, bs], make, kind="conv1x1 + shortcut")
    out = torch.empty((N, Co, H, W), dtype=torch.float32, device=a.device)
    step = min(_conv_x3_chunks(N, C, Co, H * W, H * W), _conv_x3_chunks(N, C2, Co, H2 * W2, H * W))
    with torch.cuda.device(a.device):
        for i in range(0, N, step):
            n = min(step, N - i)
            native.check(native.lib().dvis_conv1x1_x3_dual(
                native.dev_ptr(a[i:i + n], "a"), native.dev_ptr(x[i:i + n], "x"), ctypes.c_void_p(buf.data_ptr()),
                None if bias is None else native.dev_ptr(bias, "bias"), None, native.dev_ptr(out[i:i + n], "out"), n, C, C2, Co, H, W,
                H2, W2, stride2, X3_CONV_XEXP if xexp is None else xexp, wexp, 1 if relu else 0, native.stream_ptr(a.device)),
                "dvis_conv1x1_x3_dual")
    return out


def conv3x3_x3_ok(x, weight, stride=1, res=None):
    return weight.dim() == 4 and tuple(weight.shape[2:]) == (3, 3) and conv1x1_x3_ok(x, weight, stride, res)


def conv3x3_x3(x, weight, bias=None, res=None, relu=False, stride=1, xexp=None):
    N, Ci, H, W = x.shape
    Co = weight.shape[0]

    def make():
        return _x3_pack_conv3x3(weight.detach().contiguous())
    buf, wexp = _x3_cache(weight, [weight], make, kind="conv3x3")
    OH, OW = (H + stride - 1) // stride, (W + stride - 1) // stride
    out = torch.empty((N, Co, OH, OW), dtype=torch.float32, device=x.device)
    step = _conv_x3_chunks(N, Ci, Co, H * W, OH * OW)
    with torch.cuda.device(x.device):
        for i in range(0, N, step):
            n = min(step, N - i)
            native.check(native.lib().dvis_conv3x3_x3(
                native.dev_ptr(x[i:i + n], "x"), ctypes.c_void_p(buf.data_ptr()),
                None if bias is None else native.dev_ptr(bias.detach(), "bias"),
                None if res is None else native.dev_ptr(res[i:i + n], "res"), native.dev_ptr(out[i:i + n], "out"), n, Ci, Co, H, W,
                stride, X3_CONV_XEXP if xexp is None else xexp, wexp, 1 if relu else 0, native.stream_ptr(x.device)),
                "dvis_conv3x3_x3")
    return out


X3_IMAGES = os.environ.get("DVIS_X3_IMAGES", "1") != "0"


class OperandImage:

    def __init__(self, data, N, C, H, W, exp):
        self.data, self.N, self.C, self.H, self.W, self.exp = data, N, C, H, W, exp

    @property
    def device(self):
        return self.data.device

    def images(self, i, n):
        per = self.data.numel() // self.N
        return self.data[i * per:(i + n) * per]


def x3_images_ok(N, C, K, H, W, device, taps=1, stride=1):
    if not (X3_IMAGES and x3_on() and device.type == "cuda" and not torch.is_grad_enabled()):
        return False
    if taps not in (1, 9) or C % 64 != 0 or not (K == 128 or K % 256 == 0) or N <= 0:
        return False
    OH, OW = (H + stride - 1) // stride, (W + stride - 1) // stride
    return bool(native.lib().dvis_conv1x1_x3_supported(C, K, 1, H * W, OH * OW))


def _image_chunks(N, C, K, H, W, OH, OW):
    per = max(C * H * ((W + 31) // 32 * 32), K * OH * ((OW + 31) // 32 * 32)) * 4
    return max(1, min(N, (2 ** 31 - 1) // per))


def upsample_add_image(lateral, top, lat_affine=None, oexp=None):
    N, C, H, W = lateral.shape
    lib = native.lib()
    oe = X3_CONV_XEXP if oexp is None else oexp
    top = top.contiguous()
    data = torch.empty(lib.dvis_conv_x3_image_bytes(N, C, H, W), dtype=torch.uint8, device=lateral.device)
    img = OperandImage(data, N, C, H, W, oe)
    step = _image_chunks(N, C, C, H, W, H, W)
    with torch.cuda.device(lateral.device):
        for i in range(0, N, step):
            n = min(step, N - i)
            sc = None if lat_affine is None else native.dev_ptr(lat_affine[0].reshape(N, C)[i:i + n], "scale")
            sh = None if lat_affine is None else native.dev_ptr(lat_affine[1].reshape(N, C)[i:i + n], "shift")
            native.check(lib.dvis_upsample_add_image(native.dev_ptr(lateral[i:i + n], "lateral"), sc, sh, native.dev_ptr(top[i:i + n], "top"),
                                                     ctypes.c_void_p(img.images(i, n).data_ptr()), n, C, H, W, top.shape[-2], top.shape[-1], oe,
                                                     native.stream_ptr(lateral.device)), "dvis_upsample_add_image")
    return img


def conv_x3_image(src, weight, bias=None, res=None, relu=False, stride=1, out_image=False, oexp=None, xexp=None, gn=None):
    lib = native.lib()
    from_img = isinstance(src, OperandImage)
    if not (from_img or out_image):
        raise ValueError("conv_x3_image: neither side is an operand image")
    N, C, H, W = (src.N, src.C, src.H, src.W) if from_img else src.shape
    K, taps = weight.shape[0], weight.shape[2] * weight.shape[3]
    dev = weight.device

    def make():
        w2 = weight.detach().contiguous()
        if from_img:
            return _x3_packed(w2, lib.dvis_conv1x1_x3_packed_bytes(C, K) * taps, lambda e, buf, st: lib.dvis_conv_x3_pack_image(
                native.dev_ptr(w2, "weight"), K, C, taps, e, buf, st), "dvis_conv_x3_pack_image")
        return _x3_pack_conv1x1(w2.reshape(K, C)) if taps == 1 else _x3_pack_conv3x3(w2)
    kind = ("conv%dx%d" % ((1, 1) if taps == 1 else (3, 3))) + (" image-in" if from_img else "")
    buf, wexp = _x3_cache(weight, [weight], make, kind=kind)
    OH, OW = (H + stride - 1) // stride, (W + stride - 1) // stride
    xe = src.exp if from_img else (X3_CONV_XEXP if xexp is None else xexp)
    oe = X3_CONV_XEXP if oexp is None else oexp
    if out_image:
        out = OperandImage(torch.empty(lib.dvis_conv_x3_image_bytes(N, K, OH, OW), dtype=torch.uint8, device=dev), N, K, OH, OW, oe)
    else:
        out = torch.empty((N, K, OH, OW), dtype=torch.float32, device=dev)
    step = _image_chunks(N, C, K, H, W, OH, OW)
    if gn is not None and not (from_img and not out_image):
        raise ValueError("conv_x3_image: gn needs an operand image in and an fp32 map out")
    part = _gn_partials(N, K, OH * OW, dev) if gn is not None and N > 0 and gn_fold_ok(gn, K, OH * OW) else None
    with torch.cuda.device(dev):
        for i in range(0, N, step):
            n = min(step, N - i)
            native.check(lib.dvis_conv_x3_image(
                ctypes.c_void_p(src.images(i, n).data_ptr()) if from_img else None, None if from_img else native.dev_ptr(src[i:i + n], "x"),
                ctypes.c_void_p(buf.data_ptr()), None if bias is None else native.dev_ptr(bias.detach(), "bias"),
                None if res is None else native.dev_ptr(res[i:i + n], "res"), None if out_image else native.dev_ptr(out[i:i + n], "out"),
                ctypes.c_void_p(out.images(i, n).data_ptr()) if out_image else None, n, C, K, H, W, stride, taps, xe, wexp, oe, 1 if relu else 0,
                native.stream_ptr(dev), None if part is None else native.dev_ptr(part[i:i + n], "partials")), "dvis_conv_x3_image")
    if gn is None:
        return out
    return out, (_gn_finalize(part, gn, N, K, OH * OW) if part is not None else group_norm_affine(out, gn))


X3_BNECK = os.environ.get("DVIS_X3_BNECK", "1") != "0"


def bneck_stage_x3_ok(x, blocks):
    if not (X3_BNECK and x3_on() and x.is_cuda and x.dim() == 4 and x.dtype == torch.float32 and x.is_contiguous()
            and not torch.is_grad_enabled() and len(blocks) >= 2 and x.shape[1] == 64 and x.shape[0] > 0):
        return False
    for i, b in enumerate(blocks):
        cin = 64 if i == 0 else 256
        if tuple(b["w1"].shape) != (64, cin, 1, 1) or tuple(b["w2"].shape) != (64, 64, 3, 3) or tuple(b["w3"].shape) != (256, 64, 1, 1):
            return False
        if (b["ws"] is not None) != (i == 0) or (i == 0 and tuple(b["ws"].shape) != (256, 64, 1, 1)):
            return False
        if any(b[k] is not None and (b[k].dtype != torch.float32 or b[k].device != x.device) for k in b):
            return False
    return bool(native.lib().dvis_bneck_x3_supported(1, x.shape[2], x.shape[3]))


def bneck_stage_x3(x, blocks, xexp=None):
    N, _, H, W = x.shape
    lib = native.lib()
    xe = X3_CONV_XEXP if xexp is None else xexp
    dev = x.device

    def packed_conv1():
        w = blocks[0]["w1"]

        return _x3_cache(w, [w], lambda: _x3_pack_conv1x1(w.detach().reshape(64, 64).contiguous()), kind="conv1x1")

    def packed_block(i):
        b, nxt = blocks[i], (blocks[i + 1] if i + 1 < len(blocks) else None)
        ws, w1n = b["ws"], (None if nxt is None else nxt["w1"])

        def make():
            w2 = b["w2"].detach().contiguous()
            w3 = b["w3"].detach().reshape(256, 64).contiguous()
            wsd = None if ws is None else ws.detach().reshape(256, 64).contiguous()
            w1d = None if w1n is None else w1n.detach().reshape(64, 256).contiguous()
            e2, e1 = _x3_wexp(w2), (0 if w1d is None else _x3_wexp(w1d))
            e3 = _x3_wexp(w3 if wsd is None else torch.cat([w3, wsd], 1))
            buf = torch.empty(lib.dvis_bneck_x3_packed_bytes(0 if w1d is None else 1, 0 if wsd is None else 1), dtype=torch.uint8, device=dev)
            with torch.cuda.device(dev):
                native.check(lib.dvis_bneck_x3_pack(native.dev_ptr(w2, "w2"), native.dev_ptr(w3, "w3"),
                                                    None if wsd is None else native.dev_ptr(wsd, "ws"),
                                                    None if w1d is None else native.dev_ptr(w1d, "w1"), e2, e3, e1,
                                                    ctypes.c_void_p(buf.data_ptr()), native.stream_ptr(dev)), "dvis_bneck_x3_pack")
            b3 = b["b3"]
            if b["bs"] is not None:
                b3 = b["bs"].detach() if b3 is None else b3.detach() + b["bs"].detach()
            return buf, e2, e3, e1, (None if b3 is None else b3.detach().clone())
        return _x3_cache(b["w2"], [b["w2"], b["w3"], ws, w1n, b["b3"], b["bs"]], make, kind="bottleneck chain")

    img_bytes = lib.dvis_bneck_x3_image_bytes(N, H, W)
    imgs = [torch.empty(img_bytes, dtype=torch.uint8, device=dev) for _ in range(2)]
    ys = [torch.empty((N, 256, H, W), dtype=torch.float32, device=dev) for _ in range(min(2, len(blocks)))]
    step = max(1, min(N, (2 ** 31 - 1) // (256 * H * W * 4)))
    per_img = img_bytes // N

    def ptr(t):
        return None if t is None else native.dev_ptr(t.detach(), "shift")

    with torch.cuda.device(dev):
        for i0 in range(0, N, step):
            n = min(step, N - i0)
            isl = slice(i0 * per_img, (i0 + n) * per_img)
            buf1, e1 = packed_conv1()
            native.check(lib.dvis_conv1x1_x3_image(native.dev_ptr(x[i0:i0 + n], "x"), ctypes.c_void_p(buf1.data_ptr()), ptr(blocks[0]["b1"]),
                                                   ctypes.c_void_p(imgs[0][isl].data_ptr()), n, 64, H, W, xe, e1, xe, 1, native.stream_ptr(dev)),
                         "dvis_conv1x1_x3_image")
            for i, b in enumerate(blocks):
                buf, e2, e3, e1n, b3 = packed_block(i)
                last = i + 1 == len(blocks)
                y, yprev = ys[i % 2], ys[(i + 1) % 2]
                native.check(lib.dvis_bneck_x3(
                    ctypes.c_void_p(imgs[i % 2][isl].data_ptr()), None if i == 0 else native.dev_ptr(yprev[i0:i0 + n], "res"),
                    native.dev_ptr(x[i0:i0 + n], "x") if i == 0 else None, ctypes.c_void_p(buf.data_ptr()), ptr(b["b2"]), ptr(b3),
                    None if last else ptr(blocks[i + 1]["b1"]), native.dev_ptr(y[i0:i0 + n], "y"),
                    None if last else ctypes.c_void_p(imgs[(i + 1) % 2][isl].data_ptr()), n, H, W, xe, e2, e3, e1n, native.stream_ptr(dev)),
                    "dvis_bneck_x3")
    return ys[(len(blocks) - 1) % 2]


def _fp32_pack(weight, kind, numel, pack, name):
    def make():
        w = weight.detach().contiguous()
        uf = torch.empty(numel, dtype=torch.float32, device=w.device)
        with torch.cuda.device(w.device):
            native.check(pack(native.dev_ptr(w, "weight"), native.dev_ptr(uf, "uf"), native.stream_ptr(w.device)), name)
        return uf
    return derived.TABLE.get(weight, kind, [weight], make)


CONV1X1_MFMA = os.environ.get("DVIS_CONV1X1_MFMA", "1") != "0"


def conv1x1s2_supported(x, weight):
    N, Ci, H, W = x.shape
    return CONV1X1_MFMA and x.is_cuda and x.dtype == torch.float32 and x.is_contiguous() and not torch.is_grad_enabled() \
        and bool(native.lib().dvis_conv1x1_mfma_supported(Ci, weight.shape[0], ((H + 1) // 2) * ((W + 1) // 2))) \
        and 2 * Ci * H * W * 4 < 2 ** 31


def conv1x1_mfma(x, weight, bias=None, res=None, relu=False, stride=1):
    N, Ci, H, W = x.shape
    Co = weight.shape[0]
# ... 822 lines not shown
```

### dvis_plus_amd/native.py

```python
import ctypes
import os

import torch

_HERE = os.path.dirname(os.path.abspath(__file__))
LIB_PATH = os.environ.get("DVIS_HIP_LIB") or os.path.join(_HERE, "lib", "libdvis_hip.so")

F32, F64, F16, BF16 = 0, 1, 2, 3
_DTYPE = {torch.float32: F32, torch.float64: F64, torch.float16: F16, torch.bfloat16: BF16}

_c = ctypes
_i, _i64, _p, _f = _c.c_int, _c.c_int64, _c.c_void_p, _c.c_float

SIGNATURES = {
    "dvis_last_error": (_c.c_char_p, []),
    "dvis_version": (_i, []),
    "dvis_msda_forward": (_i, [_i, _p, _p, _p, _p, _p, _i, _i, _i, _i, _i, _i, _i, _p, _p]),
    "dvis_msda_backward": (_i, [_i, _p, _p, _p, _p, _p, _p, _i, _i, _i, _i, _i, _i, _i, _p, _p, _p, _p]),
    "dvis_msda_backward_det_ws_bytes": (_i64, [_i, _i, _i, _i]),
    "dvis_msda_backward_det": (_i, [_p, _p, _p, _p, _p, _p, _i, _i, _i, _i, _i, _i, _i, _p, _p, _p, _p, _p]),
    "dvis_msda_fused_backward_ws_bytes": (_i64, [_i, _i, _i, _i]),
    "dvis_msda_fused_backward": (_i, [_p, _p, _p, _p, _i, _p, _i64, _p, _i64, _p, _i, _i, _i, _i, _i, _i, _i, _p, _p, _p, _p, _p]),
    "dvis_msda_fused_forward": (_i, [_p, _p, _p, _p, _i, _p, _i64, _p, _i64, _i, _i, _i, _i, _i, _i, _i, _p, _p, _p]),
    "dvis_msda_fused_forward_pos": (_i, [_p, _p, _p, _p, _i, _p, _i64, _p, _i64, _p, _p, _i64, _i, _i, _i, _i, _i, _i, _i,
                                         _p, _p, _p]),
    "dvis_msda_fused_forward_h": (_i, [_i, _p, _p, _p, _p, _i, _p, _i64, _p, _i64, _i, _i, _i, _i, _i, _i, _i, _p, _p, _p]),
    "dvis_msda_fused_forward_slots": (_i, [_p, _p, _p, _p, _i, _p, _i64, _p, _i64, _i, _i, _i, _p, _p, _i64, _i, _i, _i, _i,
                                           _i, _i, _i, _p, _p, _p]),
    "dvis_nchw_to_tokens": (_i, [_p, _p, _i64, _i, _i64, _i64, _i64, _p]),
    "dvis_tokens_to_nchw": (_i, [_p, _p, _i64, _i, _i64, _i64, _i64, _p]),
    "dvis_normalize_pad": (_i, [_p, _i, _p, _i64, _i, _i, _i, _i, _i, _p, _p, _p]),
    "dvis_nchw_to_tokens_affine": (_i, [_p, _p, _p, _p, _p, _p, _i64, _i, _i64, _i64, _i64, _p]),
    "dvis_mask_logits": (_i, [_p, _p, _i, _i, _i, _i64, _p, _p]),
    "dvis_mask_logits_backward_ws_bytes": (_i64, [_i, _i, _i, _i64]),
    "dvis_mask_logits_backward": (_i, [_p, _p, _i, _i, _i, _i64, _p, _p, _p, _p]),
    "dvis_attn_mask": (_i, [_p, _p, _i, _i, _i, _i, _i, _i, _i, _p, _p, _p]),
    "dvis_center_pool3": (_i, [_p, _i64, _i, _i, _p, _p, _p, _p]),
    "dvis_attn_mask_pooled": (_i, [_p, _p, _i, _i, _i, _i, _i, _p, _p, _p]),
    "dvis_mask_gemm_plan": (_i, [_i, _i, _i, _i, _i, _i, _i, _i, _i, _i, _p, _i]),
    "dvis_attention_ws_bytes": (_i64, [_i, _i, _i, _i]),
    "dvis_attention_ws_bytes_k": (_i64, [_i, _i, _i, _i, _i]),
    "dvis_attention_plan": (_i, [_i, _i, _i, _i, _i, _i64, _i64, _i, _p]),
    "dvis_attention_forward": (_i, [_p, _p, _p, _p, _p, _p, _p, _p, _p, _p, _i, _i, _i, _i, _i, _f, _p, _p]),
    "dvis_attention_forward_k": (_i, [_p, _p, _p, _p, _p, _p, _p, _p, _p, _p, _i, _i, _i, _i, _i, _f, _p, _p, _i]),
    "dvis_attention_backward": (_i, [_p, _p, _p, _p, _p, _p, _p, _p, _p, _p, _p, _i, _i, _i, _i, _i, _f, _p]),
    "dvis_attention_backward_threads": (_i, [_i]),
    "dvis_masked_attention_backward_ws_bytes": (_i64, [_i, _i, _i, _i]),
    "dvis_masked_attention_backward": (_i, [_p, _p, _p, _p, _p, _p, _p, _p, _p, _p, _p, _p, _p, _i, _i, _i, _i, _i, _f, _p, _p]),
    "dvis_masked_attention_backward_plan": (_i, [_i, _i, _i, _p]),
    "dvis_add_layernorm": (_i, [_p, _p, _i64, _p, _p, _p, _i64, _i, _f, _p]),
    "dvis_add_layernorm_pos": (_i, [_p, _p, _i64, _p, _p, _p, _p, _i64, _p, _i64, _i, _f, _p]),
    "dvis_bias_act": (_i, [_p, _p, _p, _i64, _i, _i64, _i, _p]),
    "dvis_conv3x3_winograd_supported": (_i, [_i, _i, _i, _i]),
    "dvis_conv3x3_winograd_pack": (_i, [_p, _p, _i, _i, _p]),
    "dvis_conv3x3_winograd": (_i, [_p, _p, _p, _p, _i, _i, _i, _i, _i, _i, _p]),
    "dvis_conv3x3s2_supported": (_i, [_i, _i, _i, _i]),
    "dvis_conv3x3s2_pack": (_i, [_p, _p, _i, _i, _p]),
    "dvis_conv3x3s2": (_i, [_p, _p, _p, _p, _i, _i, _i, _i, _i, _i, _p]),
    "dvis_conv7x7s2_supported": (_i, [_i, _i, _i, _i]),
    "dvis_conv7x7s2_pack": (_i, [_p, _p, _p]),
    "dvis_conv7x7s2": (_i, [_p, _p, _p, _p, _i, _i, _i, _i, _p]),
    "dvis_conv1x1_mfma_supported": (_i, [_i, _i, _i64]),
    "dvis_conv1x1_mfma_pack": (_i, [_p, _p, _i, _i, _p]),
    "dvis_conv1x1_mfma": (_i, [_p, _p, _p, _p, _p, _i, _i, _i, _i64, _i, _p]),
    "dvis_conv1x1s2_mfma": (_i, [_p, _p, _p, _p, _p, _i, _i, _i, _i, _i, _i, _p]),
    "dvis_conv1x1_supported": (_i, [_i, _i, _i64]),
    "dvis_conv1x1_bias_act": (_i, [_p, _p, _p, _p, _p, _i, _i, _i, _i64, _i, _p]),
    "dvis_bias_relu_maxpool": (_i, [_p, _p, _p, _i64, _i, _i, _i, _p]),
    "dvis_group_norm_affine": (_i, [_p, _p, _p, _p, _p, _i64, _i, _i, _i64, _f, _p]),
    "dvis_scale_shift_act": (_i, [_p, _p, _p, _i64, _i64, _i, _p]),
    "dvis_group_norm_finalize": (_i, [_p, _p, _p, _p, _p, _i64, _i, _i, _i64, _f, _p]),
    "dvis_upsample_add_affine": (_i, [_p, _p, _p, _p, _p, _i64, _i, _i, _i, _i, _p]),
    "dvis_upsample_add": (_i, [_p, _p, _p, _i64, _i, _i, _i, _i, _p]),
    "dvis_dwconv3x3_tokens": (_i, [_p, _p, _i64, _i, _i, _i, _i, _p, _p, _i, _p]),
    "dvis_dwconv3x3_tokens_backward_ws_bytes": (_i64, [_i, _i, _i, _i]),
    "dvis_dwconv3x3_tokens_backward": (_i, [_p, _p, _p, _p, _i, _i64, _i, _i, _i, _i, _p, _p, _p, _p, _p]),
    "dvis_adapter_res2": (_i, [_p, _p, _p, _p, _p, _p, _i, _i, _i, _i, _p]),
    "dvis_vps_argmax": (_i, [_p, _i64, _i64, _p, _i, _i, _i, _i, _i, _i, _i, _i, _i, _i, _p, _p, _p, _p]),
    "dvis_vss_argmax": (_i, [_p, _i64, _i64, _p, _i, _i, _i, _i, _i, _i, _i, _i, _i, _i, _i, _i, _p, _p]),
    "dvis_resize2_gt0": (_i, [_p, _i64, _i64, _i, _i, _i, _i, _i, _i, _i, _i, _i, _i, _p, _p]),
    "dvis_resize2": (_i, [_p, _i64, _i64, _i, _i, _i, _i, _i, _i, _i, _i, _i, _i, _i, _p, _p]),
    "dvis_lsap_solve": (_i, [_p, _i, _i, _p]),
    "dvis_match_chain": (_i, [_p, _i, _i, _p]),
    "dvis_gemm_nt": (_i, [_p, _i64, _i64, _p, _i64, _i64, _p, _p, _i64, _i64, _p, _i64, _i64, _i, _i, _i, _i, _i, _i, _p]),
    "dvis_gemm_nt_hm": (_i, [_p, _i64, _i64, _p, _i64, _i64, _p, _p, _i64, _i64, _p, _i64, _i64, _i, _i, _i, _i, _i, _i, _i,
                             _i64, _p]),
    "dvis_gemm_nt_bb": (_i, [_p, _i64, _i64, _p, _i64, _i64, _p, _i64, _p, _i64, _i64, _p, _i64, _i64, _i, _i, _i, _i, _i, _i,
                             _p]),
    "dvis_gemm_ln": (_i, [_p, _i64, _p, _i64, _p, _p, _f, _p, _p, _f, _p, _i64, _p, _i64, _p, _p, _i64, _p, _i64, _i, _i, _i,
                          _i, _i, _p]),
    "dvis_gemm_ln_supported": (_i, [_i, _i, _i, _i]),
    "dvis_gemm_ln_num_configs": (_i, []),
    "dvis_gemm_ln_pick_config": (_i, [_i, _i, _i]),
    "dvis_x3_packed_bytes": (_i64, [_i, _i]),
    "dvis_x3_set_reserve": (_i, [_i]),
    "dvis_x3_set_range_flag": (_i, [_p]),
    "dvis_x3_set_tag": (_i, [_i]),
    "dvis_x3_pack": (_i, [_p, _i64, _i, _i, _i, _p, _p]),
    "dvis_x3_linear_supported": (_i, [_i, _i, _i]),
    "dvis_x3_linear": (_i, [_p, _i64, _i64, _i, _p, _i, _i, _i, _p, _i, _p, _i64, _p]),
    "dvis_x3_tile_supported": (_i, [_i, _i]),
    "dvis_x3_tile_packed_bytes": (_i64, [_i, _i]),
    "dvis_x3_tile_pack": (_i, [_p, _i64, _i, _i, _i, _p, _p]),
    "dvis_x3_tile_linear_qkv": (_i, [_p, _i64, _i64, _i, _p, _i, _i, _i, _p, _i, _i, _f, _p, _p]),
    "dvis_attention_x3_packed": (_i, [_p, _p, _p, _i, _i, _i, _p]),
    "dvis_x3_rows_image_bytes": (_i64, [_i64, _i]),
    "dvis_x3_rows_image": (_i, [_p, _i64, _i64, _i, _i, _p, _p]),
    "dvis_layernorm_rows_image": (_i, [_p, _p, _p, _i64, _i, _f, _i, _p, _p]),
    "dvis_x3_tile_pack_order": (_i, [_p, _i64, _i, _i, _i, _i, _p, _p]),
    "dvis_x3_tile_linear_image": (_i, [_p, _i64, _i, _p, _i, _i, _i, _p, _i, _p, _i64, _p, _i64, _p, _i, _p]),
    "dvis_x3_tile_linear_qkv_image": (_i, [_p, _i64, _i, _p, _i, _i, _i, _p, _i, _i, _f, _p, _p]),
    "dvis_attention_x3_packed_image": (_i, [_p, _p, _i, _i, _i, _i, _p]),
    "dvis_x3_tile_linear": (_i, [_p, _i64, _i64, _i, _p, _i, _i, _i, _p, _i, _p, _i64, _p, _i64, _p]),
    "dvis_x3_linear_res": (_i, [_p, _i64, _i64, _i, _p, _i, _i, _i, _p, _i, _p, _i64, _p, _i64, _p]),
    "dvis_x3_linear_add": (_i, [_p, _i64, _i64, _i, _p, _i, _i, _i, _p, _i64, _p, _i, _p, _i64, _p]),
    "dvis_x3_linear_ln": (_i, [_p, _i64, _i64, _i, _p, _i, _i, _i, _p, _p, _i64, _p, _p, _f, _p, _i64, _p, _p, _i64, _p]),
    "dvis_x3_ffn_packed_bytes": (_i64, [_i, _i, _i]),
    "dvis_x3_ffn_pack": (_i, [_p, _i64, _p, _i64, _i, _i, _i, _i, _i, _p, _p]),
    "dvis_x3_ffn_ln": (_i, [_p, _i64, _i64, _i, _i, _i, _p, _i, _i, _i, _i, _p, _p, _p, _p, _f, _p, _i64, _p, _p, _i64, _p]),
    "dvis_conv1x1_x3_supported": (_i, [_i, _i, _i64, _i64, _i64]),
    "dvis_conv1x1_x3_packed_bytes": (_i64, [_i, _i]),
    "dvis_conv1x1_x3_pack": (_i, [_p, _i, _i, _i, _p, _p]),
    "dvis_conv_x3_gn_fold_supported": (_i, [_i, _i, _i64]),
    "dvis_conv1x1_x3": (_i, [_p, _p, _p, _p, _p, _i, _i, _i, _i, _i, _i, _i, _i, _i, _p, _p, _p, _i, _p]),
    "dvis_conv1x1_x3_dual": (_i, [_p, _p, _p, _p, _p, _p, _i, _i, _i, _i, _i, _i, _i, _i, _i, _i, _i, _i, _p]),
    "dvis_conv3x3_x3_packed_bytes": (_i64, [_i, _i]),
    "dvis_conv3x3_x3_pack": (_i, [_p, _i, _i, _i, _p, _p]),
    "dvis_conv3x3_x3": (_i, [_p, _p, _p, _p, _p, _i, _i, _i, _i, _i, _i, _i, _i, _i, _p]),
    "dvis_bneck_x3_supported": (_i, [_i64, _i, _i]),
    "dvis_bneck_x3_image_bytes": (_i64, [_i64, _i, _i]),
    "dvis_bneck_x3_packed_bytes": (_i64, [_i, _i]),
    "dvis_bneck_x3_pack": (_i, [_p, _p, _p, _p, _i, _i, _i, _p, _p]),
    "dvis_bneck_x3": (_i, [_p, _p, _p, _p, _p, _p, _p, _p, _p, _i, _i, _i, _i, _i, _i, _i, _p]),
    "dvis_conv1x1_x3_image": (_i, [_p, _p, _p, _p, _i, _i, _i, _i, _i, _i, _i, _i, _p]),
    "dvis_conv_x3_image_bytes": (_i64, [_i64, _i, _i, _i]),
    "dvis_conv_x3_pack_image": (_i, [_p, _i, _i, _i, _i, _p, _p]),
    "dvis_conv_x3_image": (_i, [_p, _p, _p, _p, _p, _p, _p, _i, _i, _i, _i, _i, _i, _i, _i, _i, _i, _i, _p, _p]),
    "dvis_upsample_add_image": (_i, [_p, _p, _p, _p, _p, _i, _i, _i, _i, _i, _i, _i, _p]),
    "dvis_gemm_num_configs": (_i, []),
    "dvis_gemm_pick_config": (_i, [_i, _i, _i, _i]),
    "dvis_gemm_pick_config_nw": (_i, [_i, _i, _i, _i, _i]),
    "dvis_gemm_config_waves": (_i, [_i]),
    "dvis_pan_pair_hist": (_i, [_p, _p, _p, _i, _i, _i, _i64, _p, _p, _p]),
    "dvis_sem_confusion": (_i, [_p, _p, _i64, _i, _p, _p, _p]),
    "dvis_video_consistency": (_i, [_p, _p, _i, _i64, _p, _i, _p, _p, _p]),
    "dvis_rle_encode": (_i, [_p, _i64, _i, _i, _i, _p, _p, _p, _p, _p, _p, _p]),
    "dvis_rle_strings": (_i, [_p, _p, _i64, _p, _p, _p, _p]),
    "dvis_rle_decode": (_i, [_p, _p, _i64, _i, _i, _p, _p]),
    "dvis_track_intersections": (_i, [_p, _i64, _i, _p, _i64, _i, _i, _i64, _i, _p, _p]),
    "dvis_pan_segment_stats": (_i, [_p, _i, _i, _i, _i, _p, _p, _p]),
    "dvis_pan_paint_rgb": (_i, [_p, _i64, _p, _i, _p, _p]),
    "dvis_sem_paint": (_i, [_p, _i64, _p, _p, _p, _p]),
    "dvis_resize_frames_u8": (_i, [_p, _i, _i, _i, _p, _i, _i, _p, _i, _p, _i, _i, _p]),
    "dvis_match_cost_ws_bytes": (_i64, [_i, _i, _i, _i]),
    "dvis_match_cost": (_i, [_p, _p, _i, _p, _p, _p, _i, _i, _i, _i, _i, _i, _i, _i, _i, _f, _f, _f, _p, _p, _p, _p]),
    "dvis_point_sample_rows": (_i, [_p, _i, _p, _i64, _i, _i, _i, _p, _p]),
    "dvis_point_loss_ws_bytes": (_i64, [_i64]),
    "dvis_point_loss_fwd": (_i, [_p, _p, _i, _p, _i, _i, _i, _i, _i, _i, _p, _p, _p]),
    "dvis_point_loss_bwd": (_i, [_p, _p, _i, _p, _p, _p, _p, _i, _i, _i, _i, _i, _i, _f, _p, _p, _p]),
    "dvis_contrastive_items_tile": (_i, []),
    "dvis_contrastive_items": (_i, [_p, _i64, _i, _p, _p, _p, _p, _p, _i, _i64, _p, _p, _p, _p, _p, _p]),
    "dvis_contrastive_items_backward_ws_bytes": (_i64, [_i, _i64, _i]),
    "dvis_contrastive_items_backward": (_i, [_p, _i64, _i, _p, _p, _p, _p, _p, _i, _i64, _p, _p, _p, _p, _p, _p, _p, _p, _p, _p,
                                             _p, _p, _p]),
    "dvis_window_attention_supported": (_i, [_i, _i]),
    "dvis_window_attention": (_i, [_p, _p, _p, _p, _i, _i, _i, _i, _i, _i, _i, _f, _p]),
}

_lib = None


def lib():
    global _lib
    if _lib is None:
        if not os.path.exists(LIB_PATH):
            raise RuntimeError(
                f"{LIB_PATH} not found: build it with `python -m dvis_plus_amd.build` "
                "(__graft_entry__.build()).  dvis_plus_amd has no CPU/eager fallback.")
        l = ctypes.CDLL(LIB_PATH)
        for name, (res, args) in SIGNATURES.items():
            fn = getattr(l, name)
            fn.restype, fn.argtypes = res, args
        _lib = l
    return _lib


def check(rc, what):
    if rc != 0:
        msg = lib().dvis_last_error().decode()
        raise RuntimeError(f"{what} failed (code {rc}): {msg}")


def dtype_code(t):
    try:
        return _DTYPE[t.dtype]
    except KeyError:
        raise RuntimeError(f"unsupported dtype {t.dtype}") from None


def dev_ptr(t, name):
    if not t.is_cuda:
        raise RuntimeError(f"{name} must be a GPU tensor (dvis_plus_amd has no CPU path); got device {t.device}")
    if not t.is_contiguous():
        raise RuntimeError(f"{name} tensor has to be contiguous")
    return ctypes.c_void_p(t.data_ptr())


def stream_ptr(device=None):
    return ctypes.c_void_p(torch.cuda.current_stream(device).cuda_stream)
```

### dvis_plus_amd/pixel_decoder.py

```python
import math
import os
import warnings

import torch
import torch.nn.functional as F
from torch import nn
from torch.nn.init import constant_, normal_, xavier_uniform_

from . import derived, functions as Fn
from .d2 import configurable
from .registry import SEM_SEG_HEADS_REGISTRY, ShapeSpec

_POS_IN_KERNEL = os.environ.get("DVIS_MSDA_POS", "0") == "1"
_MSDA_SLOTS = int(os.environ.get("DVIS_MSDA_SLOTS", "0") or 0)
_MSDA_HM = os.environ.get("DVIS_MSDA_HM", "0") == "1"


def _is_power_of_2(n):
    if (not isinstance(n, int)) or (n < 0):
        raise ValueError("invalid input for _is_power_of_2: {} (type: {})".format(n, type(n)))
    return (n & (n - 1) == 0) and n != 0


class PositionEmbeddingSine(nn.Module):
# ... 355 lines not shown

    def __init__(self, *args, norm=None, activation=None, **kwargs):
        super().__init__(*args, **kwargs)
        self.norm, self.activation = norm, activation

    def _plain_1x1(self):
        return self.kernel_size == (1, 1) and self.stride == (1, 1) and self.groups == 1 and self.padding == (0, 0)

    def affine_input_ok(self, x):
        return self._plain_1x1() and torch.is_tensor(x) and Fn.affine_in_ok(x, self.weight)

    def conv(self, x, in_affine=None):
        if in_affine is not None:
            return Fn.conv1x1_x3(x, self.weight, self.bias, affine=in_affine[:2], affine_relu=in_affine[2])
        if self._plain_1x1():
            return Fn.conv1x1(x, self.weight, self.bias)
        if self.kernel_size == (3, 3) and self.stride == (1, 1) and self.padding == (1, 1) and self.dilation == (1, 1) \
                and self.groups == 1 and x.is_cuda and not torch.is_grad_enabled():
            return Fn.conv3x3_bias_act(x, self.weight, self.bias)
        return F.conv2d(x, self.weight, self.bias, self.stride, self.padding, self.dilation, self.groups)

    def conv_and_affine(self, x):
        if isinstance(self.norm, nn.GroupNorm) and self.activation is None:
            if self._plain_1x1() and Fn.conv1x1_x3_ok(x, self.weight) \
                    and Fn.gn_fold_ok(self.norm, self.out_channels, x.shape[2] * x.shape[3]):
                return Fn.conv1x1_x3(x, self.weight, self.bias, gn=self.norm)
            y = self.conv(x)
            aff = Fn.group_norm_affine(y, self.norm)
            if aff is not None:
                return y, aff
            return self.norm(y), None
        return self.forward(x), None

    def image_input_ok(self, N, C, H, W, device):
        return self.stride == (1, 1) and self.dilation == (1, 1) and self.groups == 1 and self.weight.dtype == torch.float32 \
            and ((self.kernel_size == (3, 3) and self.padding == (1, 1)) or (self.kernel_size == (1, 1) and self.padding == (0, 0))) \
            and C == self.in_channels and Fn.x3_images_ok(N, C, self.out_channels, H, W, device, taps=self.kernel_size[0] ** 2)

    def forward(self, x, in_affine=None, defer_to=None):
        aff = None
        gn_relu = isinstance(self.norm, nn.GroupNorm) and self.activation in (None, F.relu)
        if isinstance(x, Fn.OperandImage):
            if gn_relu:
                x, aff = Fn.conv_x3_image(x, self.weight, self.bias, gn=self.norm)
            else:
                x = Fn.conv_x3_image(x, self.weight, self.bias)
        else:
            x = self.conv(x, in_affine)
        if gn_relu:
            if aff is None:
                aff = Fn.group_norm_affine(x, self.norm)
            if aff is not None:
                if defer_to is not None and defer_to.affine_input_ok(x):
                    return x, (aff[0], aff[1], self.activation is not None)
                return Fn.scale_shift_act_(x, aff[0], aff[1], relu=self.activation is not None)
        if self.norm is not None:
            x = self.norm(x)
        if self.activation is not None:
            x = self.activation(x)
        return x


def get_norm(norm, out_channels):
    if norm is None or norm == "":
        return None
    if norm != "GN":
        raise NotImplementedError(f"norm {norm!r}: the DVIS++ configs use GN")
    return nn.GroupNorm(32, out_channels)


def c2_xavier_fill(module):
    nn.init.kaiming_uniform_(module.weight, a=1)
    if module.bias is not None:
        nn.init.constant_(module.bias, 0)


@SEM_SEG_HEADS_REGISTRY.register()
class MSDeformAttnPixelDecoder(nn.Module):
    @configurable
    def __init__(self, input_shape, *, transformer_dropout, transformer_nheads, transformer_dim_feedforward,
                 transformer_enc_layers, conv_dim, mask_dim, norm=None, transformer_in_features, common_stride):
        super().__init__()
        transformer_input_shape = {k: v for k, v in input_shape.items() if k in transformer_in_features}
        input_shape = sorted(input_shape.items(), key=lambda x: x[1].stride)
        self.in_features = [k for k, v in input_shape]
        self.feature_strides = [v.stride for k, v in input_shape]
        self.feature_channels = [v.channels for k, v in input_shape]
        transformer_input_shape = sorted(transformer_input_shape.items(), key=lambda x: x[1].stride)
        self.transformer_in_features = [k for k, v in transformer_input_shape]
        transformer_in_channels = [v.channels for k, v in transformer_input_shape]
        self.transformer_feature_strides = [v.stride for k, v in transformer_input_shape]
        self.transformer_num_feature_levels = len(self.transformer_in_features)
        chans = transformer_in_channels[::-1] if self.transformer_num_feature_levels > 1 \
            else [transformer_in_channels[-1]]
        self.input_proj = nn.ModuleList([
            nn.Sequential(nn.Conv2d(c, conv_dim, kernel_size=1), nn.GroupNorm(32, conv_dim)) for c in chans])
        for proj in self.input_proj:
            nn.init.xavier_uniform_(proj[0].weight, gain=1)
            nn.init.constant_(proj[0].bias, 0)
        self.transformer = MSDeformAttnTransformerEncoderOnly(
            d_model=conv_dim, dropout=transformer_dropout, nhead=transformer_nheads,
            dim_feedforward=transformer_dim_feedforward, num_encoder_layers=transformer_enc_layers,
            num_feature_levels=self.transformer_num_feature_levels)
        self.pe_layer = PositionEmbeddingSine(conv_dim // 2, normalize=True)
        self.mask_dim = mask_dim
        self.mask_features = ConvNorm(conv_dim, mask_dim, kernel_size=1, stride=1, padding=0)
        c2_xavier_fill(self.mask_features)
        self.maskformer_num_feature_levels = 3
        self.common_stride = common_stride
        stride = min(self.transformer_feature_strides)
        self.num_fpn_levels = int(math.log2(stride) - math.log2(self.common_stride))
        lateral_convs, output_convs = [], []
        use_bias = norm == ""
        for idx, in_channels in enumerate(self.feature_channels[:self.num_fpn_levels]):
            lateral_conv = ConvNorm(in_channels, conv_dim, kernel_size=1, bias=use_bias, norm=get_norm(norm, conv_dim))
            output_conv = ConvNorm(conv_dim, conv_dim, kernel_size=3, stride=1, padding=1, bias=use_bias,
                                   norm=get_norm(norm, conv_dim), activation=F.relu)
            c2_xavier_fill(lateral_conv)
            c2_xavier_fill(output_conv)
            self.add_module("adapter_{}".format(idx + 1), lateral_conv)
            self.add_module("layer_{}".format(idx + 1), output_conv)
            lateral_convs.append(lateral_conv)
            output_convs.append(output_conv)
        self.lateral_convs = lateral_convs[::-1]
        self.output_convs = output_convs[::-1]

    @classmethod
    def from_config(cls, cfg, input_shape):
        hd = cfg.MODEL.SEM_SEG_HEAD
        return dict(
            input_shape={k: v for k, v in input_shape.items() if k in hd.IN_FEATURES},
            conv_dim=hd.CONVS_DIM, mask_dim=hd.MASK_DIM, norm=hd.NORM,
            transformer_dropout=cfg.MODEL.MASK_FORMER.DROPOUT, transformer_nheads=cfg.MODEL.MASK_FORMER.NHEADS,
            transformer_dim_feedforward=1024, transformer_enc_layers=hd.TRANSFORMER_ENC_LAYERS,
            transformer_in_features=hd.DEFORMABLE_TRANSFORMER_ENCODER_IN_FEATURES, common_stride=hd.COMMON_STRIDE)

    def forward_features(self, features):
        with torch.autocast(device_type="cuda", enabled=False), Fn.x3_stage("pd_proj"):
            if self.training:
                return self._train_features(features)
            srcs, pos, affines = [], [], []
            for idx, f in enumerate(self.transformer_in_features[::-1]):
                x = features[f].float().contiguous()
                conv, gn = self.input_proj[idx][0], self.input_proj[idx][1]
                s_ = Fn.conv1x1(x, conv.weight, conv.bias) if conv.kernel_size == (1, 1) and conv.stride == (1, 1) \
                    and conv.padding == (0, 0) and conv.groups == 1 else conv(x)
                affine = Fn.group_norm_affine(s_, gn)
                srcs.append(s_ if affine is not None else gn(s_))
                affines.append(affine)
                pos.append(self.pe_layer.compute(x.shape[2], x.shape[3], x.device))
            with Fn.x3_stage("encoder"):
                y, _, _, shapes_py = self.transformer(srcs, pos, affines)
            bs = y.shape[0]
            out, tokens, start = [], [], 0
            for li, (h, w) in enumerate(shapes_py):
                tokens.append(y[:, start:start + h * w])
                if li + 1 == len(shapes_py) and self.num_fpn_levels > 0:
                    out.append(Fn.tokens_to_map(y, start, h, w))
                else:
                    out.append(tokens[-1].transpose(1, 2).reshape(bs, -1, h, w))
                start += h * w
            with Fn.x3_stage("mask_path"):
                deferred = None
                for idx, f in enumerate(self.in_features[:self.num_fpn_levels][::-1]):
                    x = features[f].float().contiguous()
                    cur_fpn, affine = self.lateral_convs[idx].conv_and_affine(x)
                    oc = self.output_convs[idx]
                    if cur_fpn.is_cuda and cur_fpn.dtype == torch.float32 and cur_fpn.is_contiguous() and out[-1].dtype == torch.float32 \
                            and oc.image_input_ok(*cur_fpn.shape, cur_fpn.device):
                        last = idx + 1 == self.num_fpn_levels and len(out) >= self.maskformer_num_feature_levels
                        y = oc(Fn.upsample_add_image(cur_fpn, out[-1], affine), defer_to=self.mask_features if last else None)
                        if isinstance(y, tuple):
                            y, deferred = y
                        out.append(y)
                    else:
                        out.append(oc(Fn.upsample_add(cur_fpn, out[-1], affine)))
                multi_scale_features = TokenMaps(out[:self.maskformer_num_feature_levels])
                multi_scale_features.tokens = tokens[:self.maskformer_num_feature_levels]
                return self.mask_features(out[-1], in_affine=deferred), out[0], multi_scale_features

    @staticmethod
    def _conv_norm(layer, x):
        x = F.conv2d(x, layer.weight, layer.bias, layer.stride, layer.padding, layer.dilation, layer.groups)
        if layer.norm is not None:
            x = F.group_norm(x, layer.norm.num_groups, layer.norm.weight, layer.norm.bias, layer.norm.eps)
        return x if layer.activation is None else layer.activation(x)

    def _train_features(self, features):
        dtype = self.mask_features.weight.dtype
        cast = lambda t: t.to(dtype) if dtype == torch.float64 else t.float()
        srcs, pos = [], []
        for idx, f in enumerate(self.transformer_in_features[::-1]):
            x = cast(features[f])
            conv, gn = self.input_proj[idx][0], self.input_proj[idx][1]
            s_ = F.conv2d(x, conv.weight, conv.bias, conv.stride, conv.padding, conv.dilation, conv.groups)
            srcs.append(F.group_norm(s_, gn.num_groups, gn.weight, gn.bias, gn.eps))
            pos.append(self.pe_layer.compute(x.shape[2], x.shape[3], x.device))
        y, shapes_py = self.transformer.train_forward(srcs, pos)
        bs = y.shape[0]
        out, start = [], 0
        for h, w in shapes_py:
            out.append(y[:, start:start + h * w].transpose(1, 2).reshape(bs, -1, h, w))
            start += h * w
        for idx, f in enumerate(self.in_features[:self.num_fpn_levels][::-1]):
            cur_fpn = self._conv_norm(self.lateral_convs[idx], cast(features[f]))
            top = F.interpolate(out[-1], size=cur_fpn.shape[-2:], mode="bilinear", align_corners=False)
            out.append(self._conv_norm(self.output_convs[idx], cur_fpn + top))
        return self._conv_norm(self.mask_features, out[-1]), out[0], TokenMaps(out[:self.maskformer_num_feature_levels])


class TokenMaps(list):
    tokens = None


def r50_input_shape():
    return {"res2": ShapeSpec(channels=256, stride=4), "res3": ShapeSpec(channels=512, stride=8),
            "res4": ShapeSpec(channels=1024, stride=16), "res5": ShapeSpec(channels=2048, stride=32)}
```

### dvis_plus_amd/transformer_decoder.py

```python
import torch
import torch.nn.functional as F
from torch import nn

from . import derived, functions as Fn
from .pixel_decoder import ConvNorm, PositionEmbeddingSine, c2_xavier_fill
from .d2 import configurable
from .registry import TRANSFORMER_DECODER_REGISTRY


def _xavier_(module):
    for p in module.parameters():
        if p.dim() > 1:
            nn.init.xavier_uniform_(p)


class SelfAttentionLayer(nn.Module):
    own_gemm = None

    def __init__(self, d_model, nhead, dropout=0.0, activation="relu", normalize_before=False):
        super().__init__()
        if normalize_before:
            raise NotImplementedError("PRE_NORM=True is not used by the DVIS++ configs")
        self.self_attn = nn.MultiheadAttention(d_model, nhead, dropout=dropout)
        self.norm = nn.LayerNorm(d_model)
# ... 85 lines not shown
        self.linear2 = nn.Linear(dim_feedforward, d_model)
        self.norm = nn.LayerNorm(d_model)
        _xavier_(self)

    def forward(self, tgt):
        h = Fn.linear_relu(tgt, self.linear1, own=self.own_gemm)
        return Fn.add_layer_norm(Fn.linear(h, self.linear2.weight, self.linear2.bias, own=self.own_gemm), tgt, self.norm)

    def train_forward(self, tgt):
        h = torch.relu(F.linear(tgt, self.linear1.weight, self.linear1.bias))
        return self.norm(tgt + F.linear(h, self.linear2.weight, self.linear2.bias))


class MLP(nn.Module):
    own_gemm = None

    def __init__(self, input_dim, hidden_dim, output_dim, num_layers):
        super().__init__()
        self.num_layers = num_layers
        h = [hidden_dim] * (num_layers - 1)
        self.layers = nn.ModuleList(nn.Linear(n, k) for n, k in zip([input_dim] + h, h + [output_dim]))

    def forward(self, x):
        for i, layer in enumerate(self.layers):
            x = Fn.linear(x, layer.weight, layer.bias, relu=i < self.num_layers - 1, own=self.own_gemm)
        return x

    def train_forward(self, x):
        for i, layer in enumerate(self.layers):
            x = F.linear(x, layer.weight, layer.bias)
            x = torch.relu(x) if i < self.num_layers - 1 else x
        return x


def layer_predictions(logits, masks):
    return {"pred_logits": logits[-1], "pred_masks": masks[-1],
            "aux_outputs": [{"pred_logits": a, "pred_masks": m} for a, m in zip(logits[:-1], masks[:-1])]}


def layer_mask_logits(mask_embed, mask_features, mask_logits):
    L, _, T, Q, cm = mask_embed.shape
    h, w = mask_features.shape[-2:]
    rows = mask_embed[:, 0].permute(1, 0, 2, 3).reshape(T, L * Q, cm)
    logits = mask_logits(rows, mask_features[0].detach().contiguous())
    return logits.view(T, L, Q, h, w).permute(1, 2, 0, 3, 4).unsqueeze(1)


class _MaskedDecoderBase(nn.Module):

    _version = 2

    @configurable
    def __init__(self, in_channels, mask_classification=True, *, num_classes, hidden_dim, num_queries, nheads,
                 dim_feedforward, dec_layers, pre_norm, mask_dim, enforce_input_project):
        super().__init__()
        assert mask_classification, "Only support mask classification model"
        self.mask_classification = mask_classification
        self.pe_layer = PositionEmbeddingSine(hidden_dim // 2, normalize=True)
        self.num_heads, self.num_layers = nheads, dec_layers
        self.transformer_self_attention_layers = nn.ModuleList()
        self.transformer_cross_attention_layers = nn.ModuleList()
        self.transformer_ffn_layers = nn.ModuleList()
        for _ in range(self.num_layers):
            self.transformer_self_attention_layers.append(
                SelfAttentionLayer(d_model=hidden_dim, nhead=nheads, dropout=0.0, normalize_before=pre_norm))
            self.transformer_cross_attention_layers.append(
                CrossAttentionLayer(d_model=hidden_dim, nhead=nheads, dropout=0.0, normalize_before=pre_norm))
            self.transformer_ffn_layers.append(
                FFNLayer(d_model=hidden_dim, dim_feedforward=dim_feedforward, dropout=0.0, normalize_before=pre_norm))
        self.decoder_norm = nn.LayerNorm(hidden_dim)
        self.num_queries = num_queries
        self.query_feat = nn.Embedding(num_queries, hidden_dim)
        self.query_embed = nn.Embedding(num_queries, hidden_dim)
        self.num_feature_levels = 3
        self.level_embed = nn.Embedding(self.num_feature_levels, hidden_dim)
        self.input_proj = nn.ModuleList()
        for _ in range(self.num_feature_levels):
            if in_channels != hidden_dim or enforce_input_project:
                self.input_proj.append(ConvNorm(in_channels, hidden_dim, kernel_size=1))
                c2_xavier_fill(self.input_proj[-1])
            else:
                self.input_proj.append(nn.Sequential())
        self.class_embed = nn.Linear(hidden_dim, num_classes + 1)
        self.mask_embed = MLP(hidden_dim, hidden_dim, mask_dim, 3)
        self._kv_cache = derived.Derived()
        self.debug_masks = None

    def _load_from_state_dict(self, state_dict, prefix, local_metadata, strict, missing_keys, unexpected_keys,
                              error_msgs):
        version = local_metadata.get("version", None)
        if version is None or version < 2:
            for k in list(state_dict.keys()):
                if k.startswith(prefix) and "static_query" in k:
                    state_dict[k.replace("static_query", "query_feat")] = state_dict.pop(k)
        super()._load_from_state_dict(state_dict, prefix, local_metadata, strict, missing_keys, unexpected_keys,
                                      error_msgs)

    @staticmethod
    def _base_from_config(cfg, in_channels, mask_classification):
        mf = cfg.MODEL.MASK_FORMER
        assert mf.DEC_LAYERS >= 1
        return dict(in_channels=in_channels, mask_classification=mask_classification,
                    num_classes=cfg.MODEL.SEM_SEG_HEAD.NUM_CLASSES, hidden_dim=mf.HIDDEN_DIM,
                    num_queries=mf.NUM_OBJECT_QUERIES, nheads=mf.NHEADS, dim_feedforward=mf.DIM_FEEDFORWARD,
                    dec_layers=mf.DEC_LAYERS - 1, pre_norm=mf.PRE_NORM, enforce_input_project=mf.ENFORCE_INPUT_PROJ,
                    mask_dim=cfg.MODEL.SEM_SEG_HEAD.MASK_DIM)

    def _level_kv_weights(self):
        def make():
            per_level = []
            for lvl in range(self.num_feature_levels):
                idx = [i for i in range(self.num_layers) if i % self.num_feature_levels == lvl]
                ws = [self.transformer_cross_attention_layers[i].kv_weights() for i in idx]
                if not ws:
                    per_level.append(None)
                    continue
                Wv, bv = torch.cat([w[2] for w in ws], 0).detach(), torch.cat([w[3] for w in ws], 0).detach()
                bv_le = (bv.double() + Wv.double() @ self.level_embed.weight[lvl].detach().double()).float()
                per_level.append((tuple(idx), torch.cat([w[0] for w in ws], 0).detach(), torch.cat([w[1] for w in ws], 0).detach(),
                                  Wv, bv, bv_le))
            return tuple(per_level)
        return self._kv_cache.get([t for l in self.transformer_cross_attention_layers
                                   for t in (l.multihead_attn.in_proj_weight, l.multihead_attn.in_proj_bias)]
                                  + [self.level_embed.weight], make)

    @staticmethod
    def _f32_inputs(x, mask_features):
        if any(m.dtype != torch.float32 for m in x):
            tokens = getattr(x, "tokens", None)
            x = type(x)(Fn.f32(m) for m in x)
            if tokens is not None:
                x.tokens = [Fn.f32(t) for t in tokens]
        return x, Fn.f32(mask_features)

    def _run_layers(self, x, mask_features):
        C = self.decoder_norm.weight.shape[0]
        N = x[0].shape[0]
        size_list, kproj, vproj = [], {}, {}
        kvw = self._level_kv_weights()
        tokens = getattr(x, "tokens", None)
        with Fn.x3_stage("decoder_kv"):
            for lvl in range(self.num_feature_levels):
                h, w = x[lvl].shape[-2:]
                size_list.append((h, w))
                if kvw[lvl] is None:
                    continue
                idx, Wk, bk, Wv, bv, bv_le = kvw[lvl]
                le = self.level_embed.weight[lvl]
                ident = isinstance(self.input_proj[lvl], nn.Sequential) and len(self.input_proj[lvl]) == 0
                if tokens is not None and ident and not torch.is_grad_enabled():
                    tok = tokens[lvl]
                    pos_t = self.pe_layer.compute(h, w, tok.device).flatten(2).transpose(1, 2)
                    if Fn.x3_on() and Fn.x3_ok(tok, Wk.shape[0], Wk.shape[1], add=True):
                        tok = tok.contiguous()
                        kall = Fn.x3_linear(tok, Wk, bk, xadd=pos_t + le).transpose(0, 1)
                        vall = Fn.x3_linear(tok, Wv, bv_le).transpose(0, 1)
                    else:
                        kall = Fn.linear(tok + (pos_t + le), Wk, bk, tall=True).transpose(0, 1)
                        vall = Fn.linear(tok, Wv, bv_le, tall=True).transpose(0, 1)
                else:
                    src = (self.input_proj[lvl](x[lvl]).flatten(2) + le[None, :, None]).permute(2, 0, 1)
                    pos = self.pe_layer.compute(h, w, x[lvl].device).flatten(2).permute(2, 0, 1)
                    kall = Fn.linear(src + pos, Wk, bk, tall=True)
                    vall = Fn.linear(src, Wv, bv, tall=True)
                for n, i in enumerate(idx):
                    kproj[i], vproj[i] = kall[..., n * C:(n + 1) * C], vall[..., n * C:(n + 1) * C]
        query_embed = self.query_embed.weight.unsqueeze(1)
        output = self.query_feat.weight.unsqueeze(1).repeat(1, N, 1)
        pyramid = Fn.center_pool3(mask_features)
        if pyramid is not None and [tuple(p.shape[-2:]) for p in pyramid] != [tuple(sz) for sz in size_list[:3]]:
            pyramid = None
        for i in range(self.num_layers):
            lvl = i % self.num_feature_levels
            emb = self.mask_embed(self.decoder_norm(output).transpose(0, 1))
            if pyramid is not None:
                mask, allowed = Fn.attn_mask_pooled(emb.contiguous(), pyramid[lvl])
            else:
                mask, allowed = Fn.attn_mask(emb.contiguous(), mask_features, size_list[lvl])
            if self.debug_masks is not None:
                self.debug_masks.append(mask.bool() & (allowed > 0)[..., None])
            layer = self.transformer_cross_attention_layers[i]
            output = layer.attend(output, output + query_embed, kproj[i], vproj[i], mask, allowed)
            output = self.transformer_self_attention_layers[i](output, query_pos=query_embed)
            output = self.transformer_ffn_layers[i](output)
        return output

    def _final_heads(self, output, mask_features, need_masks):
        dec = self.decoder_norm(output).transpose(0, 1)
        logits = Fn.linear(dec, self.class_embed.weight, self.class_embed.bias)
        masks = Fn.mask_logits(self.mask_embed(dec).contiguous(), mask_features) if need_masks else None
        return dec, logits, masks


    def _train_layers(self, x, mask_features):
        N = x[0].shape[0]
        nh, L = self.num_heads, self.num_layers
        size_list, src, pos = [], [], []
        for lvl in range(self.num_feature_levels):
            h, w = x[lvl].shape[-2:]
            size_list.append((h, w))
            proj = self.input_proj[lvl]
            m = F.conv2d(x[lvl], proj.weight, proj.bias) if isinstance(proj, nn.Conv2d) else proj(x[lvl])
            src.append((m.flatten(2) + self.level_embed.weight[lvl][None, :, None]).permute(2, 0, 1))
            pos.append(self.pe_layer.compute(h, w, x[lvl].device).to(m.dtype).flatten(2).permute(2, 0, 1))
        query_embed = self.query_embed.weight.unsqueeze(1)
        output = self.query_feat.weight.unsqueeze(1).repeat(1, N, 1)
        feats = mask_features.detach()
        logits, embs = [], []

        def heads(output):
            dec = self.decoder_norm(output).transpose(0, 1)
            logits.append(F.linear(dec, self.class_embed.weight, self.class_embed.bias))
            embs.append(self.mask_embed.train_forward(dec))
            return dec

        dec = heads(output)
        for i in range(L):
            lvl = i % self.num_feature_levels
            with torch.no_grad():
                mask, allowed = Fn.attn_mask(embs[-1].detach().contiguous(), feats, size_list[lvl])
            if self.debug_masks is not None:
                self.debug_masks.append(mask.bool() & (allowed > 0)[..., None])
            output = self.transformer_cross_attention_layers[i].train_forward(
                output, output + query_embed, src[lvl] + pos[lvl], src[lvl],
                lambda q, k, v: Fn.masked_attention(q, k, v, nh, mask, allowed))
            output = self.transformer_self_attention_layers[i].train_forward(
                output, lambda q, k, v: Fn.attention(q, k, v, nh), query_pos=query_embed)
            output = self.transformer_ffn_layers[i].train_forward(output)
            dec = heads(output)
        Q = output.shape[0]
        if mask_features.requires_grad and torch.is_grad_enabled():
            masks = [Fn.mask_logits(e.contiguous(), mask_features) for e in embs]
        else:
            masks = list(Fn.mask_logits(torch.cat(embs, dim=1), feats).split(Q, dim=1))
        return output, dec, logits, masks

    def _train_inputs(self, x, mask_features):
        assert len(x) == self.num_feature_levels
        dt = self.decoder_norm.weight.dtype
        return [m.to(dt) for m in x], mask_features.to(dt).contiguous()

    @staticmethod
    def _train_video_outputs(b, t, logits, masks):
        return layer_predictions([z.unflatten(0, (b, t)) for z in logits],
                                 [z.unflatten(0, (b, t)).transpose(1, 2) for z in masks])

    @staticmethod
    def _train_bctq(z, b, t):
        return z.unflatten(0, (b, t)).permute(0, 3, 1, 2)

    def _train_clips(self, N):
        t = self.num_frames
        if t < 1 or N % t:
            raise ValueError(f"{type(self).__name__}: a training batch holds (b t) frames with t = num_frames = {t}; got {N} frames")
        return N // t, t


@TRANSFORMER_DECODER_REGISTRY.register()
class MultiScaleMaskedTransformerDecoder(_MaskedDecoderBase):

    @classmethod
    def from_config(cls, cfg, in_channels, mask_classification):
        return cls._base_from_config(cfg, in_channels, mask_classification)

    @Fn.fp32_island
    def forward(self, x, mask_features, mask=None):
        assert len(x) == self.num_feature_levels
        if self.training:
            x, mask_features = self._train_inputs(x, mask_features)
            _, _, logits, masks = self._train_layers(x, mask_features)
            return layer_predictions(logits, masks)
        x, mask_features = self._f32_inputs(x, mask_features)
        output = self._run_layers(x, mask_features)
        _, logits, masks = self._final_heads(output, mask_features, True)
        return {"pred_logits": logits, "pred_masks": masks, "aux_outputs": []}


@TRANSFORMER_DECODER_REGISTRY.register()
class VideoMultiScaleMaskedTransformerDecoder_dvisPlus(_MaskedDecoderBase):
    @configurable
    def __init__(self, in_channels, mask_classification=True, *, num_classes, hidden_dim, num_queries, nheads,
                 dim_feedforward, dec_layers, pre_norm, mask_dim, enforce_input_project, num_frames,
                 num_reid_head_layers, reid_hidden_dim):
        super().__init__(in_channels, mask_classification, num_classes=num_classes, hidden_dim=hidden_dim,
                         num_queries=num_queries, nheads=nheads, dim_feedforward=dim_feedforward,
                         dec_layers=dec_layers, pre_norm=pre_norm, mask_dim=mask_dim,
                         enforce_input_project=enforce_input_project)
        self.num_frames = num_frames
        if num_reid_head_layers > 0:
            self.reid_embed = MLP(hidden_dim, reid_hidden_dim, hidden_dim, num_reid_head_layers)
            for layer in self.reid_embed.layers:
                c2_xavier_fill(layer)
        else:
            self.reid_embed = nn.Identity()
        self.compute_pred_masks = True

    @classmethod
    def from_config(cls, cfg, in_channels, mask_classification):
        ret = cls._base_from_config(cfg, in_channels, mask_classification)
        ret.update(num_frames=cfg.INPUT.SAMPLING_FRAME_NUM, reid_hidden_dim=cfg.MODEL.MASK_FORMER.REID_HIDDEN_DIM,
                   num_reid_head_layers=cfg.MODEL.MASK_FORMER.NUM_REID_HEAD_LAYERS)
        return ret

    @Fn.fp32_island
    def forward(self, x, mask_features, mask=None):
        assert len(x) == self.num_feature_levels
        if self.training:
# ... 75 lines not shown
```

### include/dvis_hip.h

```cpp
#ifndef DVIS_HIP_H
#define DVIS_HIP_H

#include <stdint.h>

#ifdef __cplusplus
extern "C" {
#endif

enum { DVIS_F32 = 0, DVIS_F64 = 1, DVIS_F16 = 2, DVIS_BF16 = 3 };

enum {
  DVIS_OK = 0,
  DVIS_E_ARG = -1,
  DVIS_E_LAUNCH = -2,
  DVIS_E_UNSUPPORTED = -3
};

const char *dvis_last_error(void);
int dvis_version(void);

int dvis_msda_forward(int dtype, const void *value, const int64_t *shapes, const int64_t *level_start,
                      const void *loc, const void *w, int N, int S, int M, int D, int L, int Lq, int P,
                      void *out, void *stream);

// ... 51 lines not shown
                          int32_t *allowed_count, void *stream);
int dvis_mask_gemm_plan(int mode, int B, int Q, int C, int H, int W, int h, int w, int aligned, int embed_aligned, int32_t *plan,
                        int capacity);

int64_t dvis_attention_ws_bytes(int BH, int Lq, int Lk, int d);
int dvis_attention_forward(const float *q, const int64_t *q_strides, const float *k, const int64_t *k_strides,
                           const float *v, const int64_t *v_strides, float *out, const int64_t *o_strides,
                           const uint8_t *mask, const int32_t *allowed_count, int B, int heads, int Lq, int Lk,
                           int d, float scale, void *ws, void *stream);
int dvis_attention_forward_k(const float *q, const int64_t *q_strides, const float *k, const int64_t *k_strides,
                           const float *v, const int64_t *v_strides, float *out, const int64_t *o_strides,
                           const uint8_t *mask, const int32_t *allowed_count, int B, int heads, int Lq, int Lk,
                           int d, float scale, void *ws, void *stream, int kernel);
int64_t dvis_attention_ws_bytes_k(int BH, int Lq, int Lk, int d, int kernel);
enum {
  DVIS_ATTN_FWD = 0,
  DVIS_ATTN_SHORT = 1,
  DVIS_ATTN_X3 = 2,
  DVIS_ATTN_KEYSPLIT = 3
};
int dvis_attention_plan(int BH, int Lq, int Lk, int d, int has_mask, int64_t k_row, int64_t v_row, int kernel, int32_t *plan);

int dvis_attention_backward(const float *q, const int64_t *q_strides, const float *k, const int64_t *k_strides,
                            const float *v, const int64_t *v_strides, const float *grad_out, const int64_t *g_strides,
                            float *dq, float *dk, float *dv, int B, int heads, int Lq, int Lk, int d, float scale,
                            void *stream);
int dvis_attention_backward_threads(int Lk);

int64_t dvis_masked_attention_backward_ws_bytes(int BH, int Lq, int Lk, int d);
int dvis_masked_attention_backward(const float *q, const int64_t *q_strides, const float *k, const int64_t *k_strides,
                                   const float *v, const int64_t *v_strides,
                                   const float *grad_out, const int64_t *g_strides, const uint8_t *mask,
                                   const int32_t *allowed_count, float *dq, float *dk, float *dv, int B, int heads, int Lq,
                                   int Lk, int d, float scale, void *ws, void *stream);
int dvis_masked_attention_backward_plan(int Lq, int Lk, int d, int32_t *plan);

int dvis_add_layernorm(const float *x, const float *res, int64_t res_row_stride, const float *gamma, const float *beta,
                       float *out, int64_t rows, int C, float eps, void *stream);

int dvis_add_layernorm_pos(const float *x, const float *res, int64_t res_row_stride, const float *gamma, const float *beta,
                           float *out, const float *pos, int64_t pos_rows, float *out_pos, int64_t rows, int C, float eps,
                           void *stream);

int dvis_upsample_add(const float *lateral, const float *top, float *out, int64_t planes, int H, int W, int h, int w,
                      void *stream);

int dvis_nchw_to_tokens(const float *x, float *out, int64_t N, int C, int64_t HW, int64_t S, int64_t row0, void *stream);

int dvis_tokens_to_nchw(const float *tok, float *out, int64_t N, int C, int64_t HW, int64_t S, int64_t row0, void *stream);
int dvis_normalize_pad(const void *in, int is_u8, float *out, int64_t planes, int C, int H, int W, int Hp, int Wp, const float *mean,
                       const float *stdv, void *stream);
int dvis_nchw_to_tokens_affine(const float *x, const float *scale, const float *shift, const float *pos, float *out,
                               float *out_pos, int64_t N, int C, int64_t HW, int64_t S, int64_t row0, void *stream);

int dvis_conv1x1_supported(int K, int M, int64_t HW);
int dvis_conv1x1_mfma_supported(int C, int K, int64_t HW);
int dvis_conv1x1_mfma_pack(const float *w, float *uf, int K, int C, void *stream);
int dvis_conv1x1_mfma(const float *x, const float *uf, const float *bias, const float *res, float *y, int N, int C, int K, int64_t HW,
                      int relu, void *stream);
int dvis_conv1x1s2_mfma(const float *x, const float *uf, const float *bias, const float *res, float *y, int N, int C, int K, int H, int W,
                        int relu, void *stream);
int dvis_conv1x1_bias_act(const float *x, const float *w, const float *bias, const float *res, float *out,
                          int N, int K, int M, int64_t HW, int relu, void *stream);

int dvis_conv3x3_winograd_supported(int C, int K, int H, int W);
int dvis_conv3x3s2_supported(int C, int K, int H, int W);
int dvis_conv7x7s2_supported(int C, int K, int H, int W);
int dvis_conv7x7s2_pack(const float *w, float *uf, void *stream);
int dvis_conv7x7s2(const float *x, const float *uf, const float *bias, float *y, int N, int H, int W, int relu, void *stream);
int dvis_conv3x3s2_pack(const float *w, float *uf, int K, int C, void *stream);
int dvis_conv3x3s2(const float *x, const float *uf, const float *bias, float *y, int N, int C, int K, int H, int W, int relu,
                   void *stream);
int dvis_conv3x3_winograd_pack(const float *w, float *uf, int K, int C, void *stream);
int dvis_conv3x3_winograd(const float *x, const float *uf, const float *bias, float *y, int N, int C, int K, int H, int W,
                          int relu, void *stream);

int dvis_bias_act(float *x, const float *bias, const float *res, int64_t planes, int C, int64_t HW, int relu,
                  void *stream);

int dvis_bias_relu_maxpool(const float *x, const float *bias, float *out, int64_t planes, int C, int H, int W,
                           void *stream);

int dvis_group_norm_affine(const float *x, const float *gamma, const float *beta, float *scale, float *shift, int64_t N,
                           int C, int G, int64_t HW, float eps, void *stream);
int dvis_scale_shift_act(float *x, const float *scale, const float *shift, int64_t planes, int64_t HW, int relu,
                         void *stream);
int dvis_group_norm_finalize(const double *part, const float *gamma, const float *beta, float *scale, float *shift, int64_t N, int C,
                             int G, int64_t HW, float eps, void *stream);
int dvis_upsample_add_affine(const float *lateral, const float *lat_scale, const float *lat_shift, const float *top,
                             float *out, int64_t planes, int H, int W, int h, int w, void *stream);

int dvis_dwconv3x3_tokens(const float *x, float *out, int64_t batch_stride, int B, int h, int w, int C, const float *weight,
                          const float *bias, int gelu, void *stream);

int64_t dvis_dwconv3x3_tokens_backward_ws_bytes(int B, int h, int w, int C);
int dvis_dwconv3x3_tokens_backward(const float *x, const float *grad_out, const float *weight, const float *bias, int gelu,
                                   int64_t batch_stride, int B, int h, int w, int C, float *grad_x, float *grad_weight, float *grad_bias,
                                   void *ws, void *stream);

int dvis_adapter_res2(const float *g, const float *c1, const float *x1, const float *scale, const float *shift, float *out, int B, int C,
                      int h8, int w8, void *stream);

int dvis_vps_argmax(const float *logits, int64_t stride_k, int64_t stride_t, const float *scores, int K, int T,
                    int h, int w, int first_h, int first_w, int img_h, int img_w, int out_h, int out_w,
                    int32_t *ids, uint8_t *conf, int32_t *areas, void *stream);

int dvis_resize2_gt0(const float *logits, int64_t stride_k, int64_t stride_t, int K, int T, int h, int w, int first_h,
                     int first_w, int img_h, int img_w, int out_h, int out_w, uint8_t *out, void *stream);

int dvis_resize2(const float *logits, int64_t stride_k, int64_t stride_t, int K, int T, int h, int w, int first_h,
                 int first_w, int img_h, int img_w, int out_h, int out_w, int sigmoid, float *out, void *stream);

int dvis_vss_argmax(const float *logits, int64_t stride_q, int64_t stride_t, const float *cls, int cls_row_stride, int Q,
                    int C, int T, int h, int w, int first_h, int first_w, int img_h, int img_w, int out_h, int out_w,
                    int64_t *out, void *stream);

int dvis_lsap_solve(const double *cost, int nr, int nc, int64_t *col4row);

int dvis_match_chain(const float *cost, int T, int Q, int64_t *indices);

int dvis_gemm_nt(const float *A, int64_t lda, int64_t strideA, const float *W, int64_t ldw, int64_t strideW,
                 const float *bias, const float *res, int64_t ldres, int64_t strideRes, float *C, int64_t ldc,
                 int64_t strideC, int M, int N, int K, int batch, int act, int config, void *stream);
int dvis_gemm_nt_hm(const float *A, int64_t lda, int64_t strideA, const float *W, int64_t ldw, int64_t strideW,
                    const float *bias, const float *res, int64_t ldres, int64_t strideRes, float *C, int64_t ldc,
                    int64_t strideC, int M, int N, int K, int batch, int act, int config, int head_d, int64_t head_stride,
                    void *stream);
int dvis_gemm_nt_bb(const float *A, int64_t lda, int64_t strideA, const float *W, int64_t ldw, int64_t strideW,
                    const float *bias, int64_t strideBias, const float *res, int64_t ldres, int64_t strideRes, float *C,
                    int64_t ldc, int64_t strideC, int M, int N, int K, int batch, int act, int config, void *stream);
int dvis_gemm_num_configs(void);
int dvis_gemm_pick_config(int M, int N, int K, int batch);
int dvis_gemm_pick_config_nw(int M, int N, int K, int batch, int nw);
int dvis_gemm_config_waves(int config);

int dvis_gemm_ln(const float *A, int64_t lda, const float *add, int64_t ldadd, const float *gamma1, const float *beta1,
                 float eps1, const float *gamma2, const float *beta2, float eps2, float *a_out, int64_t ldaout,
                 const float *W, int64_t ldw, const float *bias, const float *res, int64_t ldres, float *C, int64_t ldc,
                 int M, int N, int K, int act, int config, void *stream);
int dvis_gemm_ln_supported(int M, int N, int K, int norms);
int dvis_gemm_ln_num_configs(void);
int dvis_gemm_ln_pick_config(int M, int N, int K);

int64_t dvis_x3_packed_bytes(int N, int K);
int dvis_x3_set_reserve(int cus);
int dvis_x3_set_range_flag(int32_t *device_word);
int dvis_x3_set_tag(int tag);
int dvis_x3_pack(const float *W, int64_t ldw, int N, int K, int wexp, void *packed, void *stream);
int dvis_x3_linear_supported(int N, int K, int ln);
int dvis_x3_linear(const float *x, int64_t ldx, int64_t M, int K, const void *packed, int N, int xexp, int wexp,
                   const float *bias, int relu, float *out, int64_t ldo, void *stream);
int dvis_x3_linear_add(const float *x, int64_t ldx, int64_t M, int K, const void *packed, int N, int xexp, int wexp,
                       const float *xadd, int64_t xadd_rows, const float *bias, int relu, float *out, int64_t ldo, void *stream);
int dvis_x3_linear_res(const float *x, int64_t ldx, int64_t M, int K, const void *wp, int N, int xexp, int wexp, const float *bias, int act,
                       const float *res, int64_t ldres, float *out, int64_t ldo, void *stream);

int dvis_x3_tile_supported(int N, int K);
int64_t dvis_x3_tile_packed_bytes(int N, int K);
int dvis_x3_tile_pack(const float *w, int64_t ldw, int N, int K, int wexp, void *packed, void *stream);
int dvis_x3_tile_linear(const float *x, int64_t ldx, int64_t M, int K, const void *wp, int N, int xexp, int wexp, const float *bias, int act,
                        const float *res, int64_t ldres, float *out, int64_t ldo, void *stream);
int dvis_x3_tile_linear_qkv(const float *x, int64_t ldx, int64_t M, int K, const void *wp, int N, int xexp, int wexp, const float *bias,
                            int heads, int L, float qscale, void *ws, void *stream);
int dvis_attention_x3_packed(const void *ws, float *out, const int64_t *o_strides, int B, int heads, int L, void *stream);
int64_t dvis_x3_rows_image_bytes(int64_t M, int K);
int dvis_x3_rows_image(const float *x, int64_t ldx, int64_t M, int K, int xexp, void *image, void *stream);
int dvis_layernorm_rows_image(const float *x, const float *gamma, const float *beta, int64_t M, int C, float eps, int xexp, void *image,
                              void *stream);
int dvis_x3_tile_pack_order(const float *w, int64_t ldw, int N, int K, int wexp, int order, void *packed, void *stream);
int dvis_x3_tile_linear_image(const void *ximg, int64_t M, int K, const void *wp, int N, int xexp, int wexp, const float *bias, int act,
                              const float *res, int64_t ldres, float *out, int64_t ldo, void *oimg, int oexp, void *stream);
int dvis_x3_tile_linear_qkv_image(const void *ximg, int64_t M, int K, const void *wp, int N, int xexp, int wexp, const float *bias, int heads,
                                  int L, float qscale, void *ws, void *stream);
int dvis_attention_x3_packed_image(const void *ws, void *image, int B, int heads, int L, int xexp, void *stream);
int dvis_x3_linear_ln(const float *x, int64_t ldx, int64_t M, int K, const void *packed, int N, int xexp, int wexp,
                      const float *bias, const float *res, int64_t ldres, const float *gamma, const float *beta, float eps,
                      const float *pos, int64_t pos_rows, float *out, float *out2, int64_t ldo, void *stream);
int64_t dvis_x3_ffn_packed_bytes(int K, int H, int N);
int dvis_conv1x1_x3_supported(int C, int K, int64_t N, int64_t HW_in, int64_t HW_out);
int64_t dvis_conv1x1_x3_packed_bytes(int C, int K);
int dvis_conv1x1_x3_pack(const float *w, int K, int C, int wexp, void *packed, void *stream);
int dvis_conv_x3_gn_fold_supported(int K, int G, int64_t HW);
int dvis_conv1x1_x3(const float *x, const void *packed, const float *bias, const float *res, float *y, int N, int C, int K, int H,
                    int W, int stride, int xexp, int wexp, int relu, void *stream, const float *in_scale, const float *in_shift,
                    int in_relu, double *gn_part);
int dvis_conv1x1_x3_dual(const float *x, const float *x2, const void *packed, const float *bias, const float *res, float *y, int N,
                         int C, int C2, int K, int H, int W, int H2, int W2, int stride2, int xexp, int wexp, int relu, void *stream);
int64_t dvis_conv3x3_x3_packed_bytes(int C, int K);
int dvis_conv3x3_x3_pack(const float *w, int K, int C, int wexp, void *packed, void *stream);
int dvis_conv3x3_x3(const float *x, const void *packed, const float *bias, const float *res, float *y, int N, int C, int K, int H,
                    int W, int stride, int xexp, int wexp, int relu, void *stream);
int dvis_bneck_x3_supported(int64_t N, int H, int W);
int64_t dvis_bneck_x3_image_bytes(int64_t N, int H, int W);
int64_t dvis_bneck_x3_packed_bytes(int tail, int dual);
int dvis_bneck_x3_pack(const float *w2, const float *w3, const float *ws, const float *w1, int e2, int e3, int e1, void *packed,
                       void *stream);
int dvis_bneck_x3(const void *a1, const float *res, const float *x2, const void *packed, const float *b2, const float *b3,
                  const float *b1, float *y, void *out, int N, int H, int W, int xexp, int e2, int e3, int e1, void *stream);
int dvis_conv1x1_x3_image(const float *x, const void *packed, const float *bias, void *image, int N, int C, int H, int W, int xexp,
                          int wexp, int oexp, int relu, void *stream);
int64_t dvis_conv_x3_image_bytes(int64_t N, int C, int H, int W);
int dvis_conv_x3_pack_image(const float *w, int K, int C, int taps, int wexp, void *packed, void *stream);
int dvis_conv_x3_image(const void *ximg, const float *x, const void *packed, const float *bias, const float *res, float *y, void *image,
                       int N, int C, int K, int H, int W, int stride, int taps, int xexp, int wexp, int oexp, int relu, void *stream,
                       double *gn_part);
int dvis_upsample_add_image(const float *lateral, const float *lat_scale, const float *lat_shift, const float *top, void *image, int N,
                            int C, int H, int W, int h, int w, int oexp, void *stream);
int dvis_x3_ffn_pack(const float *W1, int64_t ldw1, const float *W2, int64_t ldw2, int K, int H, int N, int w1exp, int w2exp,
                     void *packed, void *stream);
int dvis_x3_ffn_ln(const float *x, int64_t ldx, int64_t M, int K, int H, int N, const void *packed, int xexp, int w1exp,
                   int hexp, int w2exp, const float *b1, const float *b2, const float *gamma, const float *beta, float eps,
                   const float *pos, int64_t pos_rows, float *out, float *out2, int64_t ldo, void *stream);

int dvis_pan_pair_hist(const int32_t *gt, const int32_t *pred, const int32_t *gt_table, int Ng, int Np, int T, int64_t HW,
                       int64_t *out, int64_t *bad, void *stream);
int dvis_sem_confusion(const int32_t *gt, const int32_t *pred, int64_t n, int num_class, int64_t *out, int64_t *bad, void *stream);
int dvis_video_consistency(const int32_t *gt, const int32_t *pred, int T, int64_t HW, const int32_t *ks, int nk, int64_t *gt_const,
                           int64_t *both_const, void *stream);

int dvis_rle_encode(const uint8_t *masks, int64_t N, int H, int W, int phase, int64_t *trans, int64_t *area, const int64_t *toff,
                    const int64_t *moff, int32_t *bnd, uint32_t *runs, void *stream);
int dvis_rle_strings(const uint32_t *runs, const int64_t *run_off, int64_t N, const int64_t *str_off, int64_t *lens, uint8_t *chars,
                     void *stream);
int dvis_rle_decode(const int32_t *ends, const int64_t *run_off, int64_t N, int H, int W, uint8_t *out, void *stream);
int dvis_track_intersections(const uint8_t *pred, int64_t pred_stride, int P, const uint8_t *gt, int64_t gt_stride, int G, int T,
                             int64_t HW, int accumulate, int64_t *out, void *stream);

int dvis_pan_segment_stats(const int32_t *map, int T, int H, int W, int n, int64_t *out, int64_t *bad, void *stream);
int dvis_pan_paint_rgb(const int32_t *map, int64_t npx, const int32_t *lut, int nlut, uint8_t *out, void *stream);
int dvis_sem_paint(const int32_t *map, int64_t npx, const int32_t *lut, uint8_t *out, int64_t *bad, void *stream);

int dvis_resize_frames_u8(const uint8_t *in, int T, int H, int W, uint8_t *out, int h, int w, const int32_t *xtab, int kx,
                          const int32_t *ytab, int ky, int reverse, void *stream);

int64_t dvis_match_cost_ws_bytes(int Q, int G, int T, int K);
int dvis_match_cost(const float *pred, const void *tgt, int tgt_u8, const float *coords, const float *logits,
                    const int64_t *tgt_ids, int Q, int G, int T, int H, int W, int Ht, int Wt, int K, int NC, float w_class,
                    float w_mask, float w_dice, float *C, float *terms, void *ws, void *stream);
int dvis_point_sample_rows(const void *rows, int rows_u8, const float *coords, int64_t R, int P, int H, int W, float *out,
                           void *stream);
int64_t dvis_point_loss_ws_bytes(int64_t R);
int dvis_point_loss_fwd(const float *src, const void *tgt, int tgt_u8, const float *coords, int R, int P, int H, int W, int Ht, int Wt,
                        float *out, void *ws, void *stream);
int dvis_point_loss_bwd(const float *src, const void *tgt, int tgt_u8, const float *coords, const float *sums, const float *g_mask,
                        const float *g_dice, int R, int P, int H, int W, int Ht, int Wt, float num_masks, float *grad_src,
                        void *det_ws, void *stream);

int dvis_contrastive_items_tile(void);
int dvis_contrastive_items(const float *src, int64_t R, int C, const int32_t *anchor, const int32_t *pos_ptr, const int32_t *pos_idx,
                           const int32_t *neg_ptr, const int32_t *neg_idx, int n, int64_t S, float *reid, float *aux, float *dots,
                           float *norms, float *stats, void *stream);
int64_t dvis_contrastive_items_backward_ws_bytes(int n, int64_t S, int C);
int dvis_contrastive_items_backward(const float *src, int64_t R, int C, const int32_t *anchor, const int32_t *pos_ptr,
                                    const int32_t *pos_idx, const int32_t *neg_ptr, const int32_t *neg_idx, int n, int64_t S,
                                    const int32_t *row_ptr, const int32_t *occ_slot, const int32_t *occ_item, const int32_t *arow_ptr,
                                    const int32_t *arow_item, const float *dots, const float *norms, const float *stats,
                                    const float *grad_reid, const float *grad_aux, float *grad_src, void *ws, void *stream);

int dvis_window_attention_supported(int ws, int d);
int dvis_window_attention(const float *qkv, const float *qkv_bias, const float *bias_table, float *out, int B, int H, int W, int heads,
                          int d, int ws, int shift, float scale, void *stream);

#ifdef __cplusplus
}
#endif
#endif
```

Before: 423.5.

## Read encoder tokens in place for FPN upsample-add and decoder K/V projections

Adds an upsample-add kernel that reads the top FPN level directly from the encoder's token layout (N, S, C), so the token-to-map transpose copy is no longer needed. It also adds a batch-strided row mapping to the x3 linear kernels, letting the decoder's key/value projections read token slices in place instead of first making a contiguous copy. The intent is to remove transpose and contiguous copy traffic. The cost is gathered, strided reads with a two-row software prefetch, and a different fma ordering in the interpolation, which may change rounding slightly.

Measured after the change: 424.8, median of 2. No clear change (+0.3%).

```diff
diff --git a/dvis_plus_amd/csrc/conv1x1_x3.hip b/dvis_plus_amd/csrc/conv1x1_x3.hip
--- a/dvis_plus_amd/csrc/conv1x1_x3.hip
+++ b/dvis_plus_amd/csrc/conv1x1_x3.hip
@@ -369,6 +369,94 @@
   }
 }
 
+__device__ __forceinline__ float ups_sum(int e, float lat, float a0, float b0, float a1, float b1, float lx0, float lx1, float ly0,
+                                         float ly1) {
+#pragma clang fp contract(off)
+  if (e < 7) {
+    const float i0 = __builtin_fmaf(lx0, a0, lx1 * b0), i1 = __builtin_fmaf(lx0, a1, lx1 * b1);
+    return lat + __builtin_fmaf(ly0, i0, ly1 * i1);
+  }
+  const float i0 = __builtin_fmaf(lx1, b0, lx0 * a0), i1 = __builtin_fmaf(lx0, a1, lx1 * b1);
+  return lat + (ly1 * i1 + ly0 * i0);
+}
+
+struct UpsRow {
+  float lat[8];
+  f4 sc[2], sh[2];
+  f4 c[4][2];
+  float ly0, ly1;
+};
+
+template <bool AFF>
+__global__ __launch_bounds__(256) void upsample_add_image_tokens_kernel(const float *__restrict__ lateral, const float *__restrict__ tok,
+                                                                        long long S, long long row0, void *__restrict__ img, int N, int C,
+                                                                        int H, int W, int h, int w, const float *__restrict__ lat_scale,
+                                                                        const float *__restrict__ lat_shift, float oscale) {
+  const int NCC = C / 64, XG = (W + 31) / 32;
+  const int cc = blockIdx.x, xg = blockIdx.y;
+  const int x = threadIdx.x & 31, g = (threadIdx.x >> 5) & 1, Sk = threadIdx.x >> 6;
+  const int px = 32 * xg + x;
+  const float sy = (float)h / (float)H, sx = (float)w / (float)W;
+  const int pxc = px < W ? px : W - 1;
+  float fx = sx * ((float)pxc + 0.5f) - 0.5f;
+  fx = fx < 0.f ? 0.f : fx;
+  const int x0 = min((int)fx, w - 1), x1 = x0 + (x0 < w - 1 ? 1 : 0);
+  const float lx1 = fx - (float)x0, lx0 = 1.f - lx1;
+  const __amdgpu_buffer_rsrc_t ri = dvis_make_rsrc_uniform(img, (unsigned)((long long)N * H * XG * NCC * 8192));
+  const unsigned rows = (unsigned)N * (unsigned)H;
+  const int cb = 64 * cc + 16 * Sk + 4 * g;
+  const unsigned row_begin = blockIdx.z * 16u, row_end = min(row_begin + 16u, rows);
+  auto request = [&](unsigned row, UpsRow &r) {
+    const unsigned n = row / (unsigned)H;
+    const int y = (int)(row - n * (unsigned)H);
+    float fy = sy * ((float)y + 0.5f) - 0.5f;
+    fy = fy < 0.f ? 0.f : fy;
+    const int y0 = min((int)fy, h - 1), y1 = y0 + (y0 < h - 1 ? 1 : 0);
+    r.ly1 = fy - (float)y0, r.ly0 = 1.f - r.ly1;
+    const float *tn = tok + ((size_t)n * (size_t)S + (size_t)row0) * (size_t)C + cb;
+    const float *t0 = tn + (size_t)y0 * w * (size_t)C, *t1 = tn + (size_t)y1 * w * (size_t)C;
+#pragma unroll
+    for (int u = 0; u < 2; ++u) {
+      r.c[0][u] = *(const f4 *)(t0 + (size_t)x0 * C + 8 * u), r.c[1][u] = *(const f4 *)(t0 + (size_t)x1 * C + 8 * u);
+      r.c[2][u] = *(const f4 *)(t1 + (size_t)x0 * C + 8 * u), r.c[3][u] = *(const f4 *)(t1 + (size_t)x1 * C + 8 * u);
+    }
+    const unsigned pl0 = n * (unsigned)C + (unsigned)cb;
+#pragma unroll
+    for (int e = 0; e < 8; ++e) r.lat[e] = lateral[((size_t)(pl0 + 8 * (e >> 2) + (e & 3)) * H + y) * (size_t)W + pxc];
+    if constexpr (AFF) {
+#pragma unroll
+      for (int u = 0; u < 2; ++u) r.sc[u] = *(const f4 *)(lat_scale + pl0 + 8 * u), r.sh[u] = *(const f4 *)(lat_shift + pl0 + 8 * u);
+    }
+    __builtin_amdgcn_sched_barrier(0);
+  };
+  if (row_begin >= row_end) return;
+  auto emit = [&](unsigned row, const UpsRow &cur) {
+    float v[8];
+#pragma unroll
+    for (int e = 0; e < 8; ++e) {
+      const int u = e >> 2, i = e & 3;
+      float lat = cur.lat[e];
+      if constexpr (AFF) lat = __builtin_fmaf(lat, cur.sc[u][i], cur.sh[u][i]);
+      v[e] = ups_sum(e, lat, cur.c[0][u][i], cur.c[1][u][i], cur.c[2][u][i], cur.c[3][u][i], lx0, lx1, cur.ly0, cur.ly1);
+    }
+    const f4 p0 = {v[0], v[1], v[2], v[3]}, p1 = {v[4], v[5], v[6], v[7]};
+    h8 hi, lo;
+    split8(p0, p1, oscale, hi, lo);
+    const unsigned G = row * (unsigned)XG + (unsigned)xg;
+    const unsigned off = (G * (unsigned)NCC + (unsigned)cc) * 8192u + (unsigned)(Sk * 2048 + g * 512 + x * 16);
+    store_fragments2(ri, off, hi, 0, lo, 1024);
+  };
+  UpsRow ra, rb;
+  request(row_begin, ra);
+  for (unsigned row = row_begin; row < row_end; row += 2) {
+    const unsigned r1 = min(row + 1, row_end - 1);
+    request(r1, rb);
+    emit(row, ra);
+    request(min(row + 2, row_end - 1), ra);
+    emit(r1, rb);
+  }
+}
+
 }
 
 DVIS_EXPORT int dvis_upsample_add_image(const float *lateral, const float *lat_scale, const float *lat_shift, const float *top, void *image,
@@ -388,6 +476,31 @@
                        lat_scale ? lat_scale + (size_t)i * C : nullptr, lat_shift ? lat_shift + (size_t)i * C : nullptr, ldexpf(1.f, oexp));
   }
   return dvis_check_launch("dvis_upsample_add_image");
+}
+
+DVIS_EXPORT int dvis_upsample_add_image_tokens(const float *lateral, const float *lat_scale, const float *lat_shift, const float *tok,
+                                               int64_t S, int64_t row0, void *image, int N, int C, int H, int W, int h, int w, int oexp,
+                                               void *stream) {
+  DVIS_REQUIRE(lateral && tok && image, "dvis_upsample_add_image_tokens: null pointer");
+  DVIS_REQUIRE((lat_scale == nullptr) == (lat_shift == nullptr), "dvis_upsample_add_image_tokens: scale and shift together");
+  DVIS_REQUIRE(N > 0 && C > 0 && C % 64 == 0 && H > 0 && W > 0 && h > 0 && w > 0, "dvis_upsample_add_image_tokens: bad sizes");
+  DVIS_REQUIRE(row0 >= 0 && S > 0 && row0 + (int64_t)h * w <= S, "dvis_upsample_add_image_tokens: rows %lld .. + %d x %d outside the %lld tokens",
+               (long long)row0, h, w, (long long)S);
+  DVIS_REQUIRE((uintptr_t)tok % 16 == 0 && (uintptr_t)lat_scale % 16 == 0 && (uintptr_t)lat_shift % 16 == 0,
+               "dvis_upsample_add_image_tokens: tok, scale and shift must be 16-byte aligned");
+  DVIS_REQUIRE((uintptr_t)image % 16 == 0 && dvis_conv_x3_image_bytes(N, C, H, W) < ((int64_t)1 << 31), "dvis_upsample_add_image_tokens: a 16-byte "
+               "aligned image below 2 GiB");
+  const int per = 16 * 65535 / H;
+  DVIS_REQUIRE(per >= 1 && (W + 31) / 32 <= 65535, "dvis_upsample_add_image_tokens: map too large (%d x %d)", H, W);
+  for (int i = 0; i < N; i += per) {
+    const int n = N - i < per ? N - i : per;
+    hipLaunchKernelGGL(lat_scale ? upsample_add_image_tokens_kernel<true> : upsample_add_image_tokens_kernel<false>,
+                       dim3(C / 64, (W + 31) / 32, (n * H + 15) / 16), dim3(256), 0, (hipStream_t)stream,
+                       lateral + (size_t)i * C * H * W, tok + (size_t)i * S * C, (long long)S, (long long)row0,
+                       (char *)image + (size_t)i * H * ((W + 31) / 32) * (C / 64) * 8192, n, C, H, W, h, w,
+                       lat_scale ? lat_scale + (size_t)i * C : nullptr, lat_shift ? lat_shift + (size_t)i * C : nullptr, ldexpf(1.f, oexp));
+  }
+  return dvis_check_launch("dvis_upsample_add_image_tokens");
 }
 
 DVIS_EXPORT int dvis_conv1x1_x3_supported(int C, int K, int64_t N, int64_t HW_in, int64_t HW_out) {
diff --git a/dvis_plus_amd/csrc/gemm_x3.hip b/dvis_plus_amd/csrc/gemm_x3.hip
--- a/dvis_plus_amd/csrc/gemm_x3.hip
+++ b/dvis_plus_amd/csrc/gemm_x3.hip
@@ -35,6 +35,22 @@
     if (jr < rows_valid) *(f4 *)(dst + jr * ld + 4 * pp) = o;
   }
   __builtin_amdgcn_wave_barrier();
+}
+
+struct RowMap {
+  unsigned rpb, bstride;
+};
+
+template <bool BS>
+__device__ __forceinline__ const float *x3_row(const float *x, int64_t ldx, int64_t row, const RowMap &rm, int64_t xadd_rows, int64_t *arow) {
+  if constexpr (BS) {
+    const unsigned b = (unsigned)row / rm.rpb, r = (unsigned)row - b * rm.rpb;
+    *arow = r;
+    return x + (b * rm.bstride + r * (unsigned)ldx);
+  } else {
+    *arow = row % xadd_rows;
+    return x + row * ldx;
+  }
 }
 
 struct EpiArgs {
@@ -156,10 +172,10 @@
   }
 }
 
-template <int NB>
+template <int NB, bool BS = false>
 __global__ __launch_bounds__(kThreads) void x3_linear_kernel(const float *__restrict__ x, int64_t ldx, int64_t M,
                                                              const void *__restrict__ wp, float xscale, int npass,
-                                                             const float *__restrict__ xadd, int64_t xadd_rows, EpiArgs e) {
+                                                             const float *__restrict__ xadd, int64_t xadd_rows, EpiArgs e, RowMap rm) {
   extern __shared__ __attribute__((aligned(1024))) char lds[];
   constexpr int K = 256, KS = K / 16, NI = K / 32;
   const int wave = threadIdx.x >> 6, lane = threadIdx.x & 63, j = lane & 31, g = lane >> 5;
@@ -176,7 +192,13 @@
     const int64_t tok0 = tile * kTileTok + wave * 32;
     const int64_t row = tok0 + j < M ? tok0 + j : M - 1;
     h8 xh[KS], xl[KS];
-    load_x<KS>(x, ldx, row, g, xscale, xh, xl, xadd ? xadd + (row % xadd_rows) * K + 8 * g : nullptr);
+    if constexpr (BS) {
+      int64_t arow;
+      const float *xr = x3_row<true>(x, ldx, row, rm, 1, &arow);
+      load_x<KS>(xr, 0, 0, g, xscale, xh, xl, xadd ? xadd + arow * K + 8 * g : nullptr);
+    } else {
+      load_x<KS>(x, ldx, row, g, xscale, xh, xl, xadd ? xadd + (row % xadd_rows) * K + 8 * g : nullptr);
+    }
     for (int pass = 0; pass < npass; ++pass) {
       f16v acc[NB];
 #pragma unroll
@@ -196,10 +218,10 @@
 
 constexpr int x3_stream_layout_blocks(int nb) { return 4 * nb % 8 == 0 ? nb : nb + 1; }
 
-template <int NB, bool LN, bool EX = false, bool ADD = false>
+template <int NB, bool LN, bool EX = false, bool ADD = false, bool BS = false>
 __global__ __launch_bounds__(512) void x3_linear_stream_kernel(const float *__restrict__ x, int64_t ldx, int64_t M, int K,
                                                                const void *__restrict__ wp, float xscale, int npass,
-                                                               const float *__restrict__ xadd, int64_t xadd_rows, EpiArgs e) {
+                                                               const float *__restrict__ xadd, int64_t xadd_rows, EpiArgs e, RowMap rm) {
   extern __shared__ __attribute__((aligned(1024))) char lds[];
   constexpr int NBL = x3_stream_layout_blocks(NB);
   constexpr int NW = 8, PW = 4 * NBL / NW, kTile = NW * 32;
@@ -239,13 +261,14 @@
         rawp[2 * s] = *(const f4 *)(posp + 32 * it + 16 * s), rawp[2 * s + 1] = *(const f4 *)(posp + 32 * it + 16 * s + 4);
       }
     };
-    int64_t r0 = row_of(blockIdx.x);
-    const float *rowp = x + r0 * ldx + 8 * g, *posp = xadd + (r0 % xadd_rows) * K + 8 * g;
+    int64_t a0;
+    const float *rowp = x3_row<BS>(x, ldx, row_of(blockIdx.x), rm, xadd_rows, &a0) + 8 * g, *posp = xadd + a0 * K + 8 * g;
     load_raw(rowp, posp, 0);
     for (int64_t tile = blockIdx.x; tile < ntiles; tile += gridDim.x) {
       const int64_t tok0 = tile * kTile + wave * 32;
-      const int64_t rn = row_of(tile + gridDim.x < ntiles ? tile + gridDim.x : tile);
-      const float *nrowp = x + rn * ldx + 8 * g, *nposp = xadd + (rn % xadd_rows) * K + 8 * g;
+      int64_t an;
+      const float *nrowp = x3_row<BS>(x, ldx, row_of(tile + gridDim.x < ntiles ? tile + gridDim.x : tile), rm, xadd_rows, &an) + 8 * g;
+      const float *nposp = xadd + an * K + 8 * g;
       for (int pass = 0; pass < npass; ++pass) {
         f16v acc[NB];
 #pragma unroll
@@ -279,7 +302,10 @@
 #pragma unroll
     for (int s = 0; s < 4; ++s) raw[2 * s] = *(const f4 *)(rowp + 64 * kc + 16 * s), raw[2 * s + 1] = *(const f4 *)(rowp + 64 * kc + 16 * s + 4);
   };
-  auto row_ptr = [&](int64_t tile) { return x + row_of(tile) * ldx + 8 * g; };
+  auto row_ptr = [&](int64_t tile) {
+    int64_t unused;
+    return x3_row<BS>(x, ldx, row_of(tile), rm, 1, &unused) + 8 * g;
+  };
   const float *rowp = row_ptr(blockIdx.x);
   load_raw(rowp, 0);
   for (int64_t tile = blockIdx.x; tile < ntiles; tile += gridDim.x) {
@@ -433,6 +459,17 @@
   return DVIS_OK;
 }
 
+int x3_check_rows(int64_t batches, int64_t rpb, int64_t bstride, int64_t ldx, int K) {
+  DVIS_REQUIRE(batches > 0 && rpb > 0 && rpb < (int64_t)1 << 31 && batches * rpb < (int64_t)1 << 31,
+               "dvis_x3 rows: batches = %lld x rows_per_batch = %lld out of range", (long long)batches, (long long)rpb);
+  DVIS_REQUIRE(ldx >= K && bstride >= 0 && bstride % 4 == 0 && (batches == 1 || bstride >= (rpb - 1) * ldx + K),
+               "dvis_x3 rows: a row stride >= K and a batch stride %% 4 == 0 that keeps the entries apart are required");
+  const int64_t extent = (batches - 1) * bstride + (rpb - 1) * ldx + K;
+  DVIS_REQUIRE(extent * 4 < (int64_t)1 << 31, "dvis_x3 rows: the strided source spans %lld bytes: it must stay below 2 GiB (split the batch)",
+               (long long)(extent * 4));
+  return DVIS_OK;
+}
+
 }
 
 static int x3_passes(int N, int *nb) {
@@ -518,7 +555,7 @@
 
 static int x3_linear_impl(const float *x, int64_t ldx, int64_t M, int K, const void *wp, int N, int xexp, int wexp, const float *xadd,
                           int64_t xadd_rows, const float *bias, int relu, float *out, int64_t ldo, void *stream,
-                          const float *radd = nullptr, int64_t ldr = 0);
+                          const float *radd = nullptr, int64_t ldr = 0, const RowMap *rows = nullptr);
 
 DVIS_EXPORT int dvis_x3_linear(const float *x, int64_t ldx, int64_t M, int K, const void *wp, int N, int xexp, int wexp,
                                const float *bias, int relu, float *out, int64_t ldo, void *stream) {
@@ -541,9 +578,31 @@
   return x3_linear_impl(x, ldx, M, K, wp, N, xexp, wexp, nullptr, 0, bias, act, out, ldo, stream, res, ldres);
 }
 
+DVIS_EXPORT int dvis_x3_linear_rows(const float *x, int64_t batches, int64_t rows_per_batch, int64_t batch_stride, int64_t ldx, int K,
+                                    const void *wp, int N, int xexp, int wexp, const float *bias, int relu, float *out, int64_t ldo,
+                                    void *stream) {
+  DVIS_REQUIRE(N > 0 && N % 256 == 0, "dvis_x3_linear_rows: served for N %% 256 == 0 (N = %d)", N);
+  const int rc = x3_check_rows(batches, rows_per_batch, batch_stride, ldx, K);
+  if (rc != DVIS_OK) return rc;
+  const RowMap rm = {(unsigned)rows_per_batch, (unsigned)batch_stride};
+  return x3_linear_impl(x, ldx, batches * rows_per_batch, K, wp, N, xexp, wexp, nullptr, 0, bias, relu, out, ldo, stream, nullptr, 0, &rm);
+}
+
+DVIS_EXPORT int dvis_x3_linear_add_rows(const float *x, int64_t batches, int64_t rows_per_batch, int64_t batch_stride, int64_t ldx, int K,
+                                        const void *wp, int N, int xexp, int wexp, const float *xadd, const float *bias, int relu,
+                                        float *out, int64_t ldo, void *stream) {
+  DVIS_REQUIRE(xadd && (uintptr_t)xadd % 16 == 0, "dvis_x3_linear_add_rows: xadd (rows_per_batch x K, 16-byte aligned) is required");
+  DVIS_REQUIRE(K == 256 && N > 0 && N % 256 == 0, "dvis_x3_linear_add_rows: served for K = 256, N %% 256 == 0 (N %d, K %d)", N, K);
+  const int rc = x3_check_rows(batches, rows_per_batch, batch_stride, ldx, K);
+  if (rc != DVIS_OK) return rc;
+  const RowMap rm = {(unsigned)rows_per_batch, (unsigned)batch_stride};
+  return x3_linear_impl(x, ldx, batches * rows_per_batch, K, wp, N, xexp, wexp, xadd, rows_per_batch, bias, relu, out, ldo, stream, nullptr, 0,
+                        &rm);
+}
+
 static int x3_linear_impl(const float *x, int64_t ldx, int64_t M, int K, const void *wp, int N, int xexp, int wexp, const float *xadd,
                           int64_t xadd_rows, const float *bias, int relu, float *out, int64_t ldo, void *stream, const float *radd,
-                          int64_t ldr) {
+                          int64_t ldr, const RowMap *rows) {
   DVIS_REQUIRE(dvis_x3_linear_supported(N, K, 0), "dvis_x3_linear: (N, K) = (%d, %d) is not served (K %% 64 == 0; N in 128 / 192 / 256 or N %% 256 == 0; N = 288 at K = 256)", N, K);
   const int rc = x3_check_common(x, ldx, M, wp, out, ldo);
   if (rc != DVIS_OK) return rc;
@@ -557,25 +616,31 @@
   hipStream_t st = (hipStream_t)stream;
   int NB;
   const int npass = x3_passes(N, &NB);
-#define DVIS_X3_STREAM_FORM(NBV, LNV, EXV, ADDV, XADD, XROWS, WHAT, LDS_EXTRA)                                        \
+#define DVIS_X3_STREAM_FORM(NBV, LNV, EXV, ADDV, XADD, XROWS, WHAT, LDS_EXTRA) DVIS_X3_STREAM_ROWS(NBV, LNV, EXV, ADDV, false, XADD, XROWS, WHAT, LDS_EXTRA)
+#define DVIS_X3_STREAM_ROWS(NBV, LNV, EXV, ADDV, BSV, XADD, XROWS, WHAT, LDS_EXTRA)                                   \
   {                                                                                                                  \
     static DvisLdsOptIn opted;                                                                                       \
     typedef Ring<4 * x3_stream_layout_blocks(NBV) / 8, 8, 8> R;                                                      \
     const size_t lds_bytes = kStages * R::kItemBytes + 8 * kScratch + (LDS_EXTRA);                                   \
-    const int rc2 = dvis_lds_opt_in((const void *)x3_linear_stream_kernel<NBV, LNV, EXV, ADDV>, lds_bytes, &opted, WHAT);  \
+    const int rc2 = dvis_lds_opt_in((const void *)x3_linear_stream_kernel<NBV, LNV, EXV, ADDV, BSV>, lds_bytes, &opted, WHAT);  \
     if (rc2 != DVIS_OK) return rc2;                                                                                  \
     const int64_t ntiles = (M + 255) / 256;                                                                          \
-    hipLaunchKernelGGL((x3_linear_stream_kernel<NBV, LNV, EXV, ADDV>), dim3(x3_grid(ntiles)), dim3(512), lds_bytes, st, x, ldx, M, K, wp, \
-                       xs, npass, XADD, XROWS, e);                                                                   \
+    hipLaunchKernelGGL((x3_linear_stream_kernel<NBV, LNV, EXV, ADDV, BSV>), dim3(x3_grid(ntiles)), dim3(512), lds_bytes, st, x, ldx, M, K, wp, \
+                       xs, npass, XADD, XROWS, e, rm);                                                               \
     return dvis_check_launch(WHAT);                                                                                  \
   }
 #define DVIS_X3_STREAM_EX(NBV, LNV, EXV, WHAT, LDS_EXTRA) DVIS_X3_STREAM_FORM(NBV, LNV, EXV, false, (const float *)nullptr, (int64_t)0, WHAT, LDS_EXTRA)
 #define DVIS_X3_STREAM(NBV, LNV, WHAT, LDS_EXTRA) DVIS_X3_STREAM_EX(NBV, LNV, false, WHAT, LDS_EXTRA)
-#define DVIS_X3_RESIDENT(NBV)                                                                                        \
+#define DVIS_X3_RESIDENT(NBV, BSV)                                                                                   \
   {                                                                                                                  \
     static DvisLdsOptIn opted;                                                                                       \
-    return x3_launch(x3_linear_kernel<NBV>, &opted, kStages * Ring<NBV>::kItemBytes + kWaves * kScratch + (size_t)N * 4, \
-                     M, st, "dvis_x3_linear", x, ldx, M, wp, xs, npass, xadd, xadd_rows, e);                         \
+    return x3_launch(x3_linear_kernel<NBV, BSV>, &opted, kStages * Ring<NBV>::kItemBytes + kWaves * kScratch + (size_t)N * 4, \
+                     M, st, "dvis_x3_linear", x, ldx, M, wp, xs, npass, xadd, xadd_rows, e, rm);                     \
+  }
+  const RowMap rm = rows ? *rows : RowMap{0, 0};
+  if (rows) {
+    if (xadd) DVIS_X3_RESIDENT(8, true)
+    DVIS_X3_STREAM_ROWS(8, false, false, false, true, (const float *)nullptr, (int64_t)0, "dvis_x3_linear_rows", (size_t)N * 4)
   }
   if (relu == 2 || radd) {
     DVIS_REQUIRE(NB == 8 && !xadd, "dvis_x3_linear_res: the GELU / residual epilogue is served for N %% 256 == 0 (N = %d)", N);
@@ -583,9 +648,9 @@
   }
   if (xadd) {
     switch (NB) {
-      case 4: DVIS_X3_RESIDENT(4)
-      case 6: DVIS_X3_RESIDENT(6)
-      case 8: DVIS_X3_RESIDENT(8)
+      case 4: DVIS_X3_RESIDENT(4, false)
+      case 6: DVIS_X3_RESIDENT(6, false)
+      case 8: DVIS_X3_RESIDENT(8, false)
       default: DVIS_X3_STREAM_FORM(9, false, false, true, xadd, xadd_rows, "dvis_x3_linear_add", (size_t)N * 4)
     }
   }
@@ -617,11 +682,13 @@
   e.flag = gd.flag, e.tag = gd.tag;
   const float xs = x3_pow2(xexp);
   const int npass = 1;
+  const RowMap rm = {0, 0};
   hipStream_t st = (hipStream_t)stream;
   DVIS_X3_STREAM(8, true, "dvis_x3_linear_ln", (size_t)3 * 256 * 4)
 #undef DVIS_X3_STREAM
 #undef DVIS_X3_STREAM_EX
 #undef DVIS_X3_STREAM_FORM
+#undef DVIS_X3_STREAM_ROWS
 }
 
 DVIS_EXPORT int64_t dvis_x3_ffn_packed_bytes(int K, int H, int N) {
diff --git a/dvis_plus_amd/functions.py b/dvis_plus_amd/functions.py
--- a/dvis_plus_amd/functions.py
+++ b/dvis_plus_amd/functions.py
@@ -1669,8 +1669,52 @@
     return x2, ld
 
 
+X3_ROWS_IN_PLACE = os.environ.get("DVIS_X3_ROWS_IN_PLACE", "1") != "0"
+PD_TOP_TOKENS = os.environ.get("DVIS_PD_TOP_TOKENS", "1") != "0"
+
+
+def x3_rows_in_place(x, N, add=False):
+    if not X3_ROWS_IN_PLACE or x.dim() != 3 or N % 256 or x.is_contiguous() or (add and x.shape[2] != 256):
+        return None
+    (B, R, K), (sb, sr, sk) = x.shape, x.stride()
+    if B * R == 0 or sk != 1 or sr < K or sr % 4 or sb % 4 or x.data_ptr() % 16 or sb < (R - 1) * sr + K or B * R >= 2 ** 31:
+        return None
+    if ((R - 1) * sr + K) * 4 >= 2 ** 31:
+        return None
+    return B, R, sb, sr
+
+
+def _x3_linear_rows(x, rows, buf, wexp, N, bias, relu, xexp, xadd):
+    B, R, sb, sr = rows
+    K = x.shape[2]
+    out = torch.empty((B, R, N), dtype=torch.float32, device=x.device)
+    per = max(1, min(B, 1 + (2 ** 31 // 4 - 1 - ((R - 1) * sr + K)) // sb))
+    lib, st = native.lib(), native.stream_ptr(x.device)
+    bptr = None if bias is None else native.dev_ptr(bias.detach(), "bias")
+    with torch.cuda.device(x.device):
+        for i in range(0, B, per):
+            n = min(per, B - i)
+            xp, op = ctypes.c_void_p(x[i].data_ptr()), ctypes.c_void_p(out[i].data_ptr())
+            if xadd is None:
+                native.check(lib.dvis_x3_linear_rows(xp, n, R, sb, sr, K, ctypes.c_void_p(buf.data_ptr()), N, xexp, wexp, bptr, int(relu),
+                                                     op, N, st), "dvis_x3_linear_rows")
+            else:
+                native.check(lib.dvis_x3_linear_add_rows(xp, n, R, sb, sr, K, ctypes.c_void_p(buf.data_ptr()), N, xexp, wexp,
+                                                         ctypes.c_void_p(xadd.data_ptr()), bptr, int(relu), op, N, st),
+                             "dvis_x3_linear_add_rows")
+    return out
+
+
 def x3_linear(x, weight, bias, relu=False, xexp=None, xadd=None, act=None, residual=None):
     N, K = weight.shape
+    rows = x3_rows_in_place(x, N, add=xadd is not None) if act is None and residual is None else None
+    if rows is not None:
+        if xadd is not None:
+            if xadd.numel() != x.shape[1] * K or xadd.dtype != torch.float32 or not xadd.is_cuda:
+                raise RuntimeError("x3_linear: xadd must be a float32 GPU (S, K) embedding for x of shape (B, S, K)")
+            xadd = xadd.contiguous()
+        buf, wexp = x3_pack(weight)
+        return _x3_linear_rows(x, rows, buf, wexp, N, bias, relu, X3_XEXP if xexp is None else xexp, xadd)
     x2, ldx = _x3_rows(x, "x")
     buf, wexp = x3_pack(weight)
     out = torch.empty((*x.shape[:-1], N), dtype=torch.float32, device=x.device)
@@ -2042,11 +2086,29 @@
     return max(1, min(N, (2 ** 31 - 1) // per))
 
 
+class TokenLevel:
+
+    def __init__(self, tokens, row0, h, w):
+        self.tokens, self.row0, self.h, self.w = tokens, row0, h, w
+
+    def map(self):
+        return tokens_to_map(self.tokens, self.row0, self.h, self.w)
+
+
+def top_tokens_ok(tokens):
+    return (PD_TOP_TOKENS and tokens.is_cuda and tokens.dtype == torch.float32 and tokens.dim() == 3 and tokens.is_contiguous()
+            and tokens.shape[2] % 64 == 0 and tokens.data_ptr() % 16 == 0 and not torch.is_grad_enabled())
+
+
 def upsample_add_image(lateral, top, lat_affine=None, oexp=None):
     N, C, H, W = lateral.shape
     lib = native.lib()
     oe = X3_CONV_XEXP if oexp is None else oexp
-    top = top.contiguous()
+    tl = top if isinstance(top, TokenLevel) else None
+    if tl is not None and (tl.tokens.shape[0] != N or tl.tokens.shape[2] != C):
+        raise RuntimeError("upsample_add_image: the token level must have the lateral's batch and channels")
+    if tl is None:
+        top = top.contiguous()
     data = torch.empty(lib.dvis_conv_x3_image_bytes(N, C, H, W), dtype=torch.uint8, device=lateral.device)
     img = OperandImage(data, N, C, H, W, oe)
     step = _image_chunks(N, C, C, H, W, H, W)
@@ -2055,6 +2117,12 @@
             n = min(step, N - i)
             sc = None if lat_affine is None else native.dev_ptr(lat_affine[0].reshape(N, C)[i:i + n], "scale")
             sh = None if lat_affine is None else native.dev_ptr(lat_affine[1].reshape(N, C)[i:i + n], "shift")
+            if tl is not None:
+                native.check(lib.dvis_upsample_add_image_tokens(native.dev_ptr(lateral[i:i + n], "lateral"), sc, sh,
+                                                                ctypes.c_void_p(tl.tokens[i].data_ptr()), tl.tokens.shape[1], tl.row0,
+                                                                ctypes.c_void_p(img.images(i, n).data_ptr()), n, C, H, W, tl.h, tl.w, oe,
+                                                                native.stream_ptr(lateral.device)), "dvis_upsample_add_image_tokens")
+                continue
             native.check(lib.dvis_upsample_add_image(native.dev_ptr(lateral[i:i + n], "lateral"), sc, sh, native.dev_ptr(top[i:i + n], "top"),
                                                      ctypes.c_void_p(img.images(i, n).data_ptr()), n, C, H, W, top.shape[-2], top.shape[-1], oe,
                                                      native.stream_ptr(lateral.device)), "dvis_upsample_add_image")
diff --git a/dvis_plus_amd/native.py b/dvis_plus_amd/native.py
--- a/dvis_plus_amd/native.py
+++ b/dvis_plus_amd/native.py
@@ -114,6 +114,8 @@
     "dvis_x3_tile_linear": (_i, [_p, _i64, _i64, _i, _p, _i, _i, _i, _p, _i, _p, _i64, _p, _i64, _p]),
     "dvis_x3_linear_res": (_i, [_p, _i64, _i64, _i, _p, _i, _i, _i, _p, _i, _p, _i64, _p, _i64, _p]),
     "dvis_x3_linear_add": (_i, [_p, _i64, _i64, _i, _p, _i, _i, _i, _p, _i64, _p, _i, _p, _i64, _p]),
+    "dvis_x3_linear_rows": (_i, [_p, _i64, _i64, _i64, _i64, _i, _p, _i, _i, _i, _p, _i, _p, _i64, _p]),
+    "dvis_x3_linear_add_rows": (_i, [_p, _i64, _i64, _i64, _i64, _i, _p, _i, _i, _i, _p, _p, _i, _p, _i64, _p]),
     "dvis_x3_linear_ln": (_i, [_p, _i64, _i64, _i, _p, _i, _i, _i, _p, _p, _i64, _p, _p, _f, _p, _i64, _p, _p, _i64, _p]),
     "dvis_x3_ffn_packed_bytes": (_i64, [_i, _i, _i]),
     "dvis_x3_ffn_pack": (_i, [_p, _i64, _p, _i64, _i, _i, _i, _i, _i, _p, _p]),
@@ -137,6 +139,7 @@
     "dvis_conv_x3_pack_image": (_i, [_p, _i, _i, _i, _i, _p, _p]),
     "dvis_conv_x3_image": (_i, [_p, _p, _p, _p, _p, _p, _p, _i, _i, _i, _i, _i, _i, _i, _i, _i, _i, _i, _p, _p]),
     "dvis_upsample_add_image": (_i, [_p, _p, _p, _p, _p, _i, _i, _i, _i, _i, _i, _i, _p]),
+    "dvis_upsample_add_image_tokens": (_i, [_p, _p, _p, _p, _i64, _i64, _p, _i, _i, _i, _i, _i, _i, _i, _p]),
     "dvis_gemm_num_configs": (_i, []),
     "dvis_gemm_pick_config": (_i, [_i, _i, _i, _i]),
     "dvis_gemm_pick_config_nw": (_i, [_i, _i, _i, _i, _i]),
diff --git a/dvis_plus_amd/pixel_decoder.py b/dvis_plus_amd/pixel_decoder.py
--- a/dvis_plus_amd/pixel_decoder.py
+++ b/dvis_plus_amd/pixel_decoder.py
@@ -531,13 +531,12 @@
             with Fn.x3_stage("encoder"):
                 y, _, _, shapes_py = self.transformer(srcs, pos, affines)
             bs = y.shape[0]
-            out, tokens, start = [], [], 0
+            out, tokens, start, top_level = [], [], 0, None
             for li, (h, w) in enumerate(shapes_py):
                 tokens.append(y[:, start:start + h * w])
+                out.append(tokens[-1].transpose(1, 2).reshape(bs, -1, h, w))
                 if li + 1 == len(shapes_py) and self.num_fpn_levels > 0:
-                    out.append(Fn.tokens_to_map(y, start, h, w))
-                else:
-                    out.append(tokens[-1].transpose(1, 2).reshape(bs, -1, h, w))
+                    top_level = Fn.TokenLevel(y, start, h, w)
                 start += h * w
             with Fn.x3_stage("mask_path"):
                 deferred = None
@@ -545,15 +544,23 @@
                     x = features[f].float().contiguous()
                     cur_fpn, affine = self.lateral_convs[idx].conv_and_affine(x)
                     oc = self.output_convs[idx]
-                    if cur_fpn.is_cuda and cur_fpn.dtype == torch.float32 and cur_fpn.is_contiguous() and out[-1].dtype == torch.float32 \
-                            and oc.image_input_ok(*cur_fpn.shape, cur_fpn.device):
+                    image_ok = cur_fpn.is_cuda and cur_fpn.dtype == torch.float32 and cur_fpn.is_contiguous() and out[-1].dtype == torch.float32 \
+                        and oc.image_input_ok(*cur_fpn.shape, cur_fpn.device)
+                    top = out[-1]
+                    if top_level is not None:
+                        if image_ok and Fn.top_tokens_ok(y) and y.shape[2] == cur_fpn.shape[1]:
+                            top = top_level
+                        else:
+                            top = out[-1] = top_level.map()
+                        top_level = None
+                    if image_ok:
                         last = idx + 1 == self.num_fpn_levels and len(out) >= self.maskformer_num_feature_levels
-                        y = oc(Fn.upsample_add_image(cur_fpn, out[-1], affine), defer_to=self.mask_features if last else None)
-                        if isinstance(y, tuple):
-                            y, deferred = y
-                        out.append(y)
+                        o = oc(Fn.upsample_add_image(cur_fpn, top, affine), defer_to=self.mask_features if last else None)
+                        if isinstance(o, tuple):
+                            o, deferred = o
+                        out.append(o)
                     else:
-                        out.append(oc(Fn.upsample_add(cur_fpn, out[-1], affine)))
+                        out.append(oc(Fn.upsample_add(cur_fpn, top, affine)))
                 multi_scale_features = TokenMaps(out[:self.maskformer_num_feature_levels])
                 multi_scale_features.tokens = tokens[:self.maskformer_num_feature_levels]
                 return self.mask_features(out[-1], in_affine=deferred), out[0], multi_scale_features
diff --git a/dvis_plus_amd/transformer_decoder.py b/dvis_plus_amd/transformer_decoder.py
--- a/dvis_plus_amd/transformer_decoder.py
+++ b/dvis_plus_amd/transformer_decoder.py
@@ -261,7 +261,8 @@
                     tok = tokens[lvl]
                     pos_t = self.pe_layer.compute(h, w, tok.device).flatten(2).transpose(1, 2)
                     if Fn.x3_on() and Fn.x3_ok(tok, Wk.shape[0], Wk.shape[1], add=True):
-                        tok = tok.contiguous()
+                        if Fn.x3_rows_in_place(tok, Wk.shape[0], add=True) is None or Fn.x3_rows_in_place(tok, Wv.shape[0]) is None:
+                            tok = tok.contiguous()
                         kall = Fn.x3_linear(tok, Wk, bk, xadd=pos_t + le).transpose(0, 1)
                         vall = Fn.x3_linear(tok, Wv, bv_le).transpose(0, 1)
                     else:
diff --git a/include/dvis_hip.h b/include/dvis_hip.h
--- a/include/dvis_hip.h
+++ b/include/dvis_hip.h
@@ -227,6 +227,11 @@
                    const float *bias, int relu, float *out, int64_t ldo, void *stream);
 int dvis_x3_linear_add(const float *x, int64_t ldx, int64_t M, int K, const void *packed, int N, int xexp, int wexp,
                        const float *xadd, int64_t xadd_rows, const float *bias, int relu, float *out, int64_t ldo, void *stream);
+int dvis_x3_linear_rows(const float *x, int64_t batches, int64_t rows_per_batch, int64_t batch_stride, int64_t ldx, int K,
+                        const void *packed, int N, int xexp, int wexp, const float *bias, int relu, float *out, int64_t ldo, void *stream);
+int dvis_x3_linear_add_rows(const float *x, int64_t batches, int64_t rows_per_batch, int64_t batch_stride, int64_t ldx, int K,
+                            const void *packed, int N, int xexp, int wexp, const float *xadd, const float *bias, int relu, float *out,
+                            int64_t ldo, void *stream);
 int dvis_x3_linear_res(const float *x, int64_t ldx, int64_t M, int K, const void *wp, int N, int xexp, int wexp, const float *bias, int act,
                        const float *res, int64_t ldres, float *out, int64_t ldo, void *stream);
 
@@ -281,6 +286,8 @@
                        double *gn_part);
 int dvis_upsample_add_image(const float *lateral, const float *lat_scale, const float *lat_shift, const float *top, void *image, int N,
                             int C, int H, int W, int h, int w, int oexp, void *stream);
+int dvis_upsample_add_image_tokens(const float *lateral, const float *lat_scale, const float *lat_shift, const float *tok, int64_t S,
+                                   int64_t row0, void *image, int N, int C, int H, int W, int h, int w, int oexp, void *stream);
 int dvis_x3_ffn_pack(const float *W1, int64_t ldw1, const float *W2, int64_t ldw2, int K, int H, int N, int w1exp, int w2exp,
                      void *packed, void *stream);
 int dvis_x3_ffn_ln(const float *x, int64_t ldx, int64_t M, int K, int H, int N, const void *packed, int xexp, int w1exp,
```
